# PaulMayer123/IMS-Toucan-Prosody-Variance

Hardware: AMD Instinct MI355X
Metric: mel-frames/sec + vocoder RTF @24kHz, batch=32, 1/2/4/8 MI355X (higher is better)
Workload: dtype bf16

## Files before the change

### ims-toucan-prosody-variance_amd/build.py

```python
import os
import shutil
import subprocess

PKG = os.path.dirname(os.path.abspath(__file__))
CSRC = os.path.join(PKG, "csrc")
LIB = os.path.join(PKG, "libtoucan_hip.so")
SOURCES = ["conv1d.hip", "resblock.hip", "rowops.hip", "attention_mfma.hip", "sequence_ops.hip", "capi.hip", "pipeline.hip", "style.hip", "wavenet.hip", "ffn.hip", "align.hip", "score.hip", "gan.hip", "pitch.hip", "train.hip", "resample.hip", "glow_forward.hip"]


def _hipcc():
    return shutil.which("hipcc") or "/opt/rocm/bin/hipcc"


def needs_build():
    if not os.path.exists(LIB):
        return True
    t = os.path.getmtime(LIB)
    deps = [os.path.join(CSRC, f) for f in os.listdir(CSRC)] + [os.path.join(PKG, "..", "include", h) for h in ("toucan_tts.h", "toucan_align.h", "toucan_score.h", "toucan_gan.h", "toucan_pitch.h", "toucan_train.h", "toucan_resample.h")]
    return any(os.path.getmtime(d) > t for d in deps)


def build(force=False, verbose=False):
    if not force and not needs_build():
        return LIB
    objs = []
    bdir = os.path.join(PKG, "build")
    os.makedirs(bdir, exist_ok=True)
    procs = []
    for src in SOURCES:
        obj = os.path.join(bdir, src.replace(".hip", ".o"))
        objs.append(obj)
        cmd = [_hipcc(), "--offload-arch=gfx950", "-O3", "-std=c++17", "-fPIC", "-c", os.path.join(CSRC, src), "-o", obj]
        if verbose:
            print(" ".join(cmd))
        procs.append((src, subprocess.Popen(cmd, stdout=subprocess.PIPE, stderr=subprocess.STDOUT, text=True)))
    for src, p in procs:
        out, _ = p.communicate()
        if p.returncode != 0:
            raise RuntimeError(f"hipcc failed on {src}:\n{out}")
        if verbose and out.strip():
            print(out)
    cmd = [_hipcc(), "--offload-arch=gfx950", "-shared", "-fPIC", "-o", LIB] + objs
    r = subprocess.run(cmd, stdout=subprocess.PIPE, stderr=subprocess.STDOUT, text=True)
    if r.returncode != 0:
        raise RuntimeError(f"link failed:\n{r.stdout}")
    return LIB


if __name__ == "__main__":
    print(build(force=True, verbose=True))
```

### ims-toucan-prosody-variance_amd/capi.py

```python
import ctypes as C
import os

_PKG = os.path.dirname(os.path.abspath(__file__))
LIB_PATH = os.environ.get("TOUCAN_HIP_LIB") or os.path.join(_PKG, "libtoucan_hip.so")

MODE_LINEAR, MODE_GLU, MODE_GATED, MODE_COUPLING = 0, 1, 2, 3
ACT_NONE, ACT_RELU, ACT_TANH = 0, 1, 2
PRE_NONE, PRE_LRELU, PRE_SNAKE = 0, 1, 2
COMPUTE_F32, COMPUTE_BF16, COMPUTE_F16 = 0, 1, 2
COMPUTE_F32X3 = 3

_p = C.c_void_p
_i = C.c_int32
_f = C.c_float


class TtsTile(C.Structure):
    _fields_ = [("row0", _i), ("seq_begin", _i), ("seq_end", _i), ("seq_id", _i)]


class TtsConvDesc(C.Structure):
    _fields_ = [
        ("x", _p), ("ldx", _i), ("cin", _i),
        ("w", _p), ("cin_pad", _i), ("wn", _i), ("half_pad", _i),
        ("bias", _p),
        ("y", _p), ("ldy", _i), ("cout", _i),
        ("taps", _i), ("dil", _i), ("pad_left", _i),
        ("pre_act", _i), ("pre_slope", _f),
        ("snake_alpha", _p), ("snake_beta", _p), ("snake_filt", _p),
        ("mode", _i), ("act", _i), ("alpha", _f),
        ("seqvec", _p), ("ld_seqvec", _i),
        ("preadd", _p), ("ld_preadd", _i),
        ("res", _p), ("ld_res", _i), ("res_scale", _f),
        ("aux", _p), ("ld_aux", _i),
        ("accumulate", _i),
        ("compute", _i),
        ("io_flags", _i),
        ("tiles", _p), ("n_tiles", _i), ("tile_rows", _i),
    ]


class TtsResblockDesc(C.Structure):
    _fields_ = [
        ("x", _p), ("ldx", _i),
        ("y", _p), ("ldy", _i),
        ("c", _i), ("taps", _i), ("dil", _i),
        ("w1", _p), ("b1", _p),
        ("w2", _p), ("b2", _p),
        ("act", _i), ("slope", _f),
        ("alpha1", _p), ("beta1", _p), ("alpha2", _p), ("beta2", _p), ("filt", _p),
        ("alpha", _f), ("res_scale", _f), ("accumulate", _i),
        ("io_bf16", _i),
        ("tiles", _p), ("n_tiles", _i), ("tile_rows", _i),
        ("compute", _i),
        ("fir_tab", _p),
    ]


class TtsWavenetDesc(C.Structure):
    _fields_ = [
        ("hs_in", _p), ("ld_in", _i),
        ("hs_out", _p), ("ld_out", _i),
        ("cond", _p), ("ld_cond", _i),
        ("w1", _p), ("b1", _p),
        ("w2", _p), ("b2", _p),
        ("cout2", _i),
        ("compute", _i),
        ("tiles", _p), ("n_tiles", _i), ("tile_rows", _i),
    ]


class TtsFfnDesc(C.Structure):
    _fields_ = [
        ("x", _p), ("ldx", _i),
        ("y", _p), ("ldy", _i),
        ("rows", _i), ("channels", _i),
        ("ln_g", _p), ("ln_b", _p),
        ("w", _p), ("b2", _p),
        ("post_g", _p), ("post_b", _p),
        ("hidden", _i), ("compute", _i),
        ("alpha", _f), ("eps", _f),
    ]


class TtsConfig(C.Structure):
    _fields_ = [("multilingual", _i), ("multispeaker", _i), ("vocoder", _i), ("precision", _i), ("small_tile_blocks", _i), ("post_bias", _f)]


IO_X_BF16, IO_Y_BF16, IO_RES_BF16, IO_F16 = 1, 2, 4, 8
IO_SPLIT_K = 16
IO_SPLIT_K_ALWAYS = 32
ATT_KEY_SPLIT, ATT_KEY_SPLIT_ALWAYS = 1, 2

PROTOTYPES = {
    "tts_last_error": (C.c_char_p, []),
    "tts_abi_version": (C.c_int, []),
    "tts_diag_queue_nonzero": (C.c_int, []),
    "tts_diag_queue_slots_used": (C.c_int, []),
    "tts_conv1d_tile_rows": (C.c_int, [_i, _i]),
    "tts_conv1d_n_tile": (C.c_int, [_i, _i]),
    "tts_conv1d_small_tile_rows": (C.c_int, [_i, _i, _i]),
    "tts_conv1d": (C.c_int, [C.POINTER(TtsConvDesc), _p]),
    "tts_resblock_step": (C.c_int, [C.POINTER(TtsResblockDesc), _p]),
    "tts_resblock_tile_rows": (C.c_int, [_i]),
    "tts_snake_fir_table": (C.c_int, [_p, _p]),
    "tts_wavenet_layer": (C.c_int, [C.POINTER(TtsWavenetDesc), _p]),
    "tts_ffn_fused": (C.c_int, [C.POINTER(TtsFfnDesc), _p]),
    "tts_layernorm": (C.c_int, [_p, _i, _p, _i, _p, _p, _i, _i, _f, _p]),
    "tts_cond_layernorm": (C.c_int, [_p, _i, _p, _i, _p, _p, _i, _p, _i, _i, _p]),
    "tts_cln_mlp_weight_floats": (C.c_int64, [_i, _i]),
    "tts_cln_mlp": (C.c_int, [_p, _i, _i, _i, _p, _i, _p, _p]),
    "tts_l2_normalize": (C.c_int, [_p, _p, _i, _i, _p]),
    "tts_groupnorm": (C.c_int, [_p, _i, _p, _i, _p, _p, _i, _i, _f, _i, _p, _i, _p, _p, _i, _i, _p, _p]),
    "tts_groupnorm_workspace_floats": (C.c_int64, [_i, _i, _i]),
    "tts_relpos_attention": (C.c_int, [_p, _i, _p, _i, _p, _p, _p, _i, _i, _i, _p, _i, _i, _i, _p]),
    "tts_relpos_attention_f16": (C.c_int, [_p, _i, _p, _i, _p, _p, _p, _i, _i, _i, _p, _i, _i, _p]),
    "tts_dwconv_swish": (C.c_int, [_p, _i, _p, _i, _p, _p, _i, _i, _p, _i, _i, _p]),
    "tts_duration_from_log": (C.c_int, [_p, _p, _i, _p]),
    "tts_prosody_control": (C.c_int, [_p, _i, _p, _p, _p, _p, _p, _i, _f, _f, _f, _f, _p]),
    "tts_length_regulate": (C.c_int, [_p, _i, _p, _p, _p, _p, _p, _p, _p, _p, _p, _p, _i, _i, _i, _i, _p, _i, _p, _i, _f, _p]),
    "tts_glow_invconv_actnorm": (C.c_int, [_p, _i, _i, _i, _p, _p, _p, _p]),
    "tts_snake_aa": (C.c_int, [_p, _i, _p, _i, _p, _p, _p, _i, _p, _i, _i, _i, _p]),
    "tts_conv_post": (C.c_int, [_p, _i, _i, _p, _f, _i, _f, _p, _p, _i, _i, _i, _p]),
    "tts_conv_post_snake_tile_rows": (C.c_int, []),
    "tts_conv_post_snake": (C.c_int, [_p, _i, _i, _p, _f, _p, _p, _p, _p, _p, _i, _i, _i, _p]),
    "tts_gather_rows": (C.c_int, [_p, _i, _p, _p, _i, _i, _i, _p]),
    "tts_gru_layer": (C.c_int, [_p, _i, _i, _i, _i, _i, _p, _p, _p, _p, _p, _i, _p]),
    "tts_style_tokens": (C.c_int, [_p, _p, _p, _i, _i, _i, _i, _p, _p]),
    "tts_complex_magnitude": (C.c_int, [_p, _i, _p, _i, _i, _i, _p]),
    "tts_log10_floor": (C.c_int, [_p, _i, _p, _i, _i, _i, _f, _p]),
    "tts_create": (C.c_int, [C.POINTER(TtsConfig), C.POINTER(_p)]),
    "tts_destroy": (C.c_int, [_p]),
    "tts_load_weights": (C.c_int, [_p, C.c_char_p, _p, C.POINTER(C.c_int64), _i, _i]),
    "tts_workspace_bytes": (C.c_int64, [_p, _i, _i, _i]),
    "tts_workspace_claimed": (C.c_int64, [_p]),
    "tts_table_stats": (C.c_int, [_p, C.POINTER(C.c_int64), C.POINTER(C.c_int64)]),
    "tts_encoder": (C.c_int, [_p, _p, _p, _p, _p, _i, _p]),
    "tts_variance_predictors": (C.c_int, [_p, _p, _p, _p, _p]),
    "tts_control_and_regulate": (C.c_int, [_p, _f, _f, _f, _f, _p, _p]),
    "tts_decoder": (C.c_int, [_p, _p]),
    "tts_postnet": (C.c_int, [_p, _p]),
    "tts_postflow": (C.c_int, [_p, _p, _p]),
    "tts_mel": (C.c_int, [_p, C.POINTER(_p), C.POINTER(_i), _p, _p]),
    "tts_prosody": (C.c_int, [_p, C.POINTER(_p), C.POINTER(_p), C.POINTER(_p)]),
    "tts_copy_mel": (C.c_int, [_p, _p, _i, _p]),
    "tts_copy_prosody": (C.c_int, [_p, _p, _p, _p, _p]),
    "tts_profile": (C.c_int, [_p, _i, C.c_char_p]),
    "tts_profile_count": (_i, [_p]),
    "tts_profile_read": (C.c_int, [_p, _i, C.c_char_p, _i, C.POINTER(C.c_double), C.POINTER(C.c_double), C.POINTER(C.c_double), C.POINTER(C.c_double)]),
    "tts_vocoder_bigvgan": (C.c_int, [_p, _p, _i, _p, _p, _i, _p, _p]),
    "tts_vocoder_hifigan": (C.c_int, [_p, _p, _i, _p, _p, _i, _p, _p]),
    "tts_synthesize_batch": (C.c_int, [_p, _p, _p, _p, _p, _i, _p, _p, _p, _f, _f, _f, _f, _p, _p, _p, _p, C.c_int64, C.POINTER(C.c_int64), _p]),
}

ALIGN_PROTOTYPES = {
    "tts_relu_affine": (C.c_int, [_p, _i, _p, _i, _i, _i, _p, _p, _p]),
    "tts_lstm_recurrence": (C.c_int, [_p, _i, _p, _p, _p, _p, _p, _p, _i, _p, _p, _i, _i, _i, _p]),
    "tts_mas_durations": (C.c_int, [_p, _i, _p, _p, _p, _p, _p, _p, _p, _p, _p, _p, _i, _i, _i, _p, _p]),
    "tts_frame_energy": (C.c_int, [_p, _i, _i, _p, _i, _p]),
    "tts_token_average": (C.c_int, [_p, _p, _p, _p, _p, _p, _p, _i, _i, _i, _p, _p]),
}

SCORE_PROTOTYPES = {
    "tts_ctc_loss": (C.c_int, [_p, _i, _i, _p, _p, _p, _p, _p, _i, _i, _i, _p, _p]),
    "tts_score_losses": (C.c_int, [_p, _i, _p, _i, _p, _i, _p, _p, _p, _p, _p, _p, _p, _p, _p, _p, _i, _p, _p]),
    "tts_teacher_forced": (C.c_int, [_p, _p, _p, _p, _p, _p, _p, C.POINTER(_i), _p]),
    "tts_copy_decoder_mel": (C.c_int, [_p, _p, _i, _p]),
    "tts_glow_forward_rows": (C.c_int, [_p, _i, _i, _p, _i, _p, _p, _p, _p, _p]),
    "tts_glow_nll_reduce": (C.c_int, [_p, _i, _p, _p, _p, _p, _i, C.c_double, _p, _p, _p]),
    "tts_postflow_nll": (C.c_int, [_p, _p, _i, _p, _p, _p, _p]),
}
CTC_MAX_TARGETS = 2048
GLOW_FORWARD_BLOCK_ROWS, GLOW_FORWARD_GRID_ROWS = 12, 24576


class TtsGanConvDesc(C.Structure):
    _fields_ = [
        ("x", _p), ("w", _p), ("scale", _p), ("shift", _p), ("res", _p), ("y", _p),
        ("n", _i), ("h", _i), ("cin", _i), ("cout", _i), ("taps", _i),
        ("flags", _i),
        ("pre_slope", _f), ("res_ratio", _f), ("slope", _f),
    ]


GAN_PROTOTYPES = {
    "tts_gan_conv2d": (C.c_int, [C.POINTER(TtsGanConvDesc), _p]),
}
GAN_KC, GAN_NC = 16, 64
GAN_UPSAMPLE, GAN_PRE_LRELU, GAN_RESIDUAL, GAN_RES_UPSAMPLE, GAN_LRELU = 1, 2, 4, 8, 16

PITCH_PROTOTYPES = {
    "tts_wave_stats": (C.c_int, [_p, _p, _p, _i, _p, _p]),
    "tts_pitch_candidates": (C.c_int, [_p, _p, _p, _p, _p, _p, _i, _i, _p, _p, _p, _p, _p, _p, _p]),
    "tts_pitch_path": (C.c_int, [_p, _p, _p, _p, _p, _p, _p, _i, _i, _p, _p]),
}
PITCH_CANDIDATES, PITCH_LAGS, PITCH_WINDOW = 15, 600, 1198
PITCH_MIN_SAMPLES, PITCH_PATH_LDS_FRAMES = 1200, 2048

_l = C.c_int64
TRAIN_PROTOTYPES = {
    "tts_gemm_f32": (C.c_int, [_i, _p, _i, _p, _i, _p, _i, _p, _i, _i, _i, _i, _p]),
    "tts_bn_train_forward": (C.c_int, [_p, _i, _p, _p, _p, _p, _p, _p, _i, _p, _p, _i, _i, _f, _f, _p]),
    "tts_bn_train_backward": (C.c_int, [_p, _i, _p, _i, _p, _p, _p, _p, _p, _i, _p, _p, _i, _i, _p]),
    "tts_bn_eval_affine": (C.c_int, [_p, _p, _p, _p, _p, _p, _i, _f, _p]),
    "tts_lstm_train_step": (C.c_int, [_p, _i, _p, _p, _p, _p, _i, _p, _p, _i, _i, _i, _p]),
    "tts_lstm_backward_step": (C.c_int, [_p, _i, _p, _p, _p, _p, _p, _i, _i, _i, _p]),
    "tts_ctc_grad": (C.c_int, [_p, _i, _i, _i, _p, _i, _i, _p, _p, _p, _p, _i, _p]),
    "tts_col_sum": (C.c_int, [_p, _i, _i, _i, _p, _p, _p]),
    "tts_sumsq": (C.c_int, [_p, _l, _p, _p, _p]),
    "tts_sgd_clip_update": (C.c_int, [_p, _p, _l, _p, _f, _f, _p]),
}
GEMM_NN, GEMM_NT, GEMM_TN = 0, 1, 2
CTC_GRAD_MAX_TARGETS, SUMSQ_PARTIALS = 768, 256


class TtsResampleSpan(C.Structure):
    _fields_ = [("in_begin", _l), ("n_held", _l), ("pos0", _l), ("out_first", _l), ("out_count", _l), ("out_begin", _l)]


RESAMPLE_PROTOTYPES = {
    "tts_resample_tile_outputs": (C.c_int, []),
    "tts_resample": (C.c_int, [_p, _p, _p, _i, _l, _i, _i, _i, _i, _p, _p]),
}
RESAMPLE_MAX_FACTOR, RESAMPLE_LDS_TABLE_BYTES = 1024, 65536

_LIB = None
ABI_VERSION = 15


class ToucanHipError(RuntimeError):
    pass


def lib():
    global _LIB
    if _LIB is not None:
        return _LIB
    if not os.path.exists(LIB_PATH):
        raise ToucanHipError(
            f"{LIB_PATH} not found: the HIP extension is mandatory (no CPU fallback). "
            f"Build it with `python -c 'import __graft_entry__ as g; g.build()'`.")
    import torch
    handle = C.CDLL(LIB_PATH)
    _assert_single_hip_runtime()
    for name, (res, args) in list(PROTOTYPES.items()) + list(ALIGN_PROTOTYPES.items()) + list(SCORE_PROTOTYPES.items()) + \
            list(GAN_PROTOTYPES.items()) + list(PITCH_PROTOTYPES.items()) + list(TRAIN_PROTOTYPES.items()) + list(RESAMPLE_PROTOTYPES.items()):
        try:
            fn = getattr(handle, name)
        except AttributeError as e:
            raise ToucanHipError(f"{LIB_PATH} does not export {name}") from e
        fn.restype = res
        fn.argtypes = args
    got = handle.tts_abi_version()
    if got != ABI_VERSION:
        raise ToucanHipError(f"{LIB_PATH} reports ABI version {got}, this binding was written for {ABI_VERSION}: rebuild the "
                             f"library (python -c 'import __graft_entry__ as g; g.build()')")
    _LIB = handle
    return handle


def _assert_single_hip_runtime():
    try:
        with open("/proc/self/maps") as f:
            paths = {line.split()[-1] for line in f if "libamdhip64" in line}
    except OSError:
        return
    if len(paths) > 1:
        raise ToucanHipError(f"two HIP runtimes are mapped ({sorted(paths)}); import torch before loading libtoucan_hip.so")


CALLS = 0


def check(rc, what=""):
    global CALLS
    CALLS += 1
    if rc != 0:
        msg = lib().tts_last_error().decode("utf-8", "replace")
        raise ToucanHipError(f"{what} failed with code {rc}: {msg}")
```

### ims-toucan-prosody-variance_amd/csrc/conv1d.hip

```cpp
#include <cstdlib>
#include <type_traits>

#include "common.h"
#include "snake.h"

namespace tts {

template <int TM, int TN, int WAVES_M, int WAVES_N, bool DUAL>
struct ConvCfg {
  static constexpr int BM = TM * WAVES_M * 32;
  static constexpr int BN = TN * WAVES_N * 32;
};

__device__ __forceinline__ float pre_activation(float v, int pre_act, float slope) {
  if (pre_act == TTS_PRE_LRELU) return v > 0.0f ? v : v * slope;
  return v;
}

__device__ __forceinline__ unsigned short f2bf(float f) { return f32_to_bf16(f); }

template <bool BF16, bool F16, class T>
__device__ __forceinline__ void store_group(T* dst, float a, float b, float c, float e) {
  if constexpr (BF16) {
    *reinterpret_cast<uint2*>(dst) = make_uint2(pack16<F16>(a, b), pack16<F16>(c, e));
  } else {
    dst[0] = a;
    dst[1] = b;
    dst[2] = c;
    dst[3] = e;
  }
}

__device__ __forceinline__ void split3(float v, float& hi, float& lo) {
  hi = (float)(_Float16)v;
  lo = (v - hi) * 2048.0f;
}
__device__ __forceinline__ void store_group_x3(unsigned short* dst, size_t plane_elems, float a, float b, float c, float e) {
  float h[4], l[4];
  split3(a, h[0], l[0]);
  split3(b, h[1], l[1]);
  split3(c, h[2], l[2]);
  split3(e, h[3], l[3]);
  *reinterpret_cast<uint2*>(dst) = make_uint2(pack16<true>(h[0], h[1]), pack16<true>(h[2], h[3]));
  *reinterpret_cast<uint2*>(dst + plane_elems) = make_uint2(pack16<true>(l[0], l[1]), pack16<true>(l[2], l[3]));
}

template <bool BF16, bool F16>
struct Elem {
  using T = unsigned short;
  static __device__ __forceinline__ unsigned short cvt(float v) { return to16<F16>(v); }
};
template <bool F16>
struct Elem<false, F16> {
  using T = float;
  static __device__ __forceinline__ float cvt(float v) { return v; }
};

template <int K, int N, class F>
__device__ __forceinline__ void static_for(F&& f) {
  if constexpr (K < N) {
    f(std::integral_constant<int, K>{});
    static_for<K + 1, N>(f);
  }
}

template <bool DUAL>
__device__ __forceinline__ float epilogue_value(const TtsConvDesc& d, float a, float g, float ba, float bg, float sv, float pa, float pg, float ax,
                                                float rv) {
  float v = a + ba + sv;
  if (d.preadd) v += pa;
  if (DUAL) {
    g += bg;
    if (d.preadd) g += pg;
    if (d.mode == TTS_MODE_GLU) {
      v = v * (1.0f / (1.0f + expf(-g)));
    } else if (d.mode == TTS_MODE_GATED) {
      v = tanhf(v) * (1.0f / (1.0f + expf(-g)));
    } else {
      v = (ax - v) * expf(-g);
    }
  } else {
    if (d.act == TTS_ACT_RELU) v = fmaxf(v, 0.0f);
    else if (d.act == TTS_ACT_TANH) v = tanhf(v);
  }
  v *= d.alpha;
  if (d.res) v += d.res_scale * rv;
  return v;
}

template <bool DUAL>
__device__ __forceinline__ void epilogue_element(const TtsConvDesc& d, int row, int n, float a, float g, float ba, float bg, float sv, bool io_f16) {
  const float pa = d.preadd ? d.preadd[(size_t)row * d.ld_preadd + n] : 0.0f;
  const float pg = (DUAL && d.preadd) ? d.preadd[(size_t)row * d.ld_preadd + d.cout + n] : 0.0f;
  const float ax = (DUAL && d.mode == TTS_MODE_COUPLING) ? d.aux[(size_t)row * d.ld_aux + n] : 0.0f;
  float rv = 0.0f;
  if (d.res)
    rv = (d.io_flags & TTS_IO_RES_BF16) ? load16(reinterpret_cast<const unsigned short*>(d.res)[(size_t)row * d.ld_res + n], io_f16)
                                        : d.res[(size_t)row * d.ld_res + n];
  float v = epilogue_value<DUAL>(d, a, g, ba, bg, sv, pa, pg, ax, rv);
  if (d.io_flags & TTS_IO_Y_BF16) {
    unsigned short* yp = reinterpret_cast<unsigned short*>(d.y) + (size_t)row * d.ldy + n;
    if (d.accumulate) v += load16(*yp, io_f16);
    *yp = store16(v, io_f16);
  } else {
    float* yp = d.y + (size_t)row * d.ldy + n;
    if (d.accumulate) v += *yp;
    *yp = v;
  }
}

__device__ __forceinline__ bool epilogue_vec_ok(const TtsConvDesc& d) {
  auto al = [](const void* p, unsigned m) { return (reinterpret_cast<uintptr_t>(p) & (m - 1)) == 0; };
  bool ok = (d.cout & 3) == 0 && (d.ldy & 3) == 0 && al(d.y, (d.io_flags & TTS_IO_Y_BF16) ? 8 : 16);
  if (d.bias) ok = ok && al(d.bias, 16);
  if (d.seqvec) ok = ok && (d.ld_seqvec & 3) == 0 && al(d.seqvec, 16);
  if (d.preadd) ok = ok && (d.ld_preadd & 3) == 0 && al(d.preadd, 16);
  if (d.res) ok = ok && (d.ld_res & 3) == 0 && al(d.res, (d.io_flags & TTS_IO_RES_BF16) ? 8 : 16);
  if (d.mode == TTS_MODE_COUPLING) ok = ok && (d.ld_aux & 3) == 0 && al(d.aux, 16);
  return ok;
}

template <int TM, int TN, int NH, bool DUAL>
__device__ __forceinline__ void conv_epilogue_t(const TtsConvDesc& d, const TtsTile& tile, int n0, int wm, int wn, int lrow, int lk,
                                                const f32x16 (&acc)[NH][TM][TN], const float* eb = nullptr, int eb_n = 0) {
  const bool io_f16 = d.io_flags & TTS_IO_F16;
  const bool vec = epilogue_vec_ok(d);
  const bool y16 = d.io_flags & TTS_IO_Y_BF16, r16 = d.io_flags & TTS_IO_RES_BF16;
  if constexpr (!DUAL) {
    if (vec && !d.preadd && eb) {
      auto col_of = [&](int j, int rq) { return n0 + (wn * TN + j) * 32 + 8 * rq + 4 * lk; };
#pragma unroll
      for (int i = 0; i < TM; ++i) {
        const int row = tile.row0 + (wm * TM + i) * 32 + lrow;
        const int rowc = row < tile.seq_end ? row : tile.seq_end - 1;
        constexpr int NG = TN * 4, CH = 8;
#pragma unroll
        for (int g0 = 0; g0 < NG; g0 += CH) {
        uint4 rv[CH], yv[CH];
#pragma unroll
          for (int g = 0; g < CH; ++g) {
            if (g0 + g >= NG) continue;
            const int j = (g0 + g) >> 2, rq = (g0 + g) & 3;
            int n = col_of(j, rq);
            n = n < d.cout ? n : d.cout - 4;
            rv[g] = make_uint4(0, 0, 0, 0);
            yv[g] = make_uint4(0, 0, 0, 0);
            if (d.res) {
              if (r16) {
                const uint2 u = *reinterpret_cast<const uint2*>(reinterpret_cast<const unsigned short*>(d.res) + (size_t)rowc * d.ld_res + n);
                rv[g].x = u.x; rv[g].y = u.y;
              } else {
                rv[g] = *reinterpret_cast<const uint4*>(d.res + (size_t)rowc * d.ld_res + n);
              }
            }
            if (d.accumulate) {
              if (y16) {
                const uint2 u = *reinterpret_cast<const uint2*>(reinterpret_cast<const unsigned short*>(d.y) + (size_t)rowc * d.ldy + n);
                yv[g].x = u.x; yv[g].y = u.y;
              } else {
                yv[g] = *reinterpret_cast<const uint4*>(d.y + (size_t)rowc * d.ldy + n);
              }
            }
          }
        __builtin_amdgcn_sched_barrier(0);
        if (row < tile.seq_end) {
#pragma unroll
          for (int g = 0; g < CH; ++g) {
            if (g0 + g >= NG) continue;
            const int j = (g0 + g) >> 2, rq = (g0 + g) & 3;
            const int n = col_of(j, rq);
            if (n >= d.cout) continue;
            const float4 ba = *reinterpret_cast<const float4*>(eb + (n - n0));
            const float4 sv = *reinterpret_cast<const float4*>(eb + eb_n + (n - n0));
            const uint4 ru = rv[g], yu = yv[g];
            float4 r4, y4;
            if (r16) r4 = make_float4(load16(ru.x & 0xFFFF, io_f16), load16(ru.x >> 16, io_f16), load16(ru.y & 0xFFFF, io_f16), load16(ru.y >> 16, io_f16));
            else r4 = make_float4(__builtin_bit_cast(float, ru.x), __builtin_bit_cast(float, ru.y), __builtin_bit_cast(float, ru.z), __builtin_bit_cast(float, ru.w));
            if (y16) y4 = make_float4(load16(yu.x & 0xFFFF, io_f16), load16(yu.x >> 16, io_f16), load16(yu.y & 0xFFFF, io_f16), load16(yu.y >> 16, io_f16));
            else y4 = make_float4(__builtin_bit_cast(float, yu.x), __builtin_bit_cast(float, yu.y), __builtin_bit_cast(float, yu.z), __builtin_bit_cast(float, yu.w));
            float v0 = epilogue_value<false>(d, acc[0][i][j][4 * rq + 0], 0.f, ba.x, 0.f, sv.x, 0.f, 0.f, 0.f, r4.x);
            float v1 = epilogue_value<false>(d, acc[0][i][j][4 * rq + 1], 0.f, ba.y, 0.f, sv.y, 0.f, 0.f, 0.f, r4.y);
            float v2 = epilogue_value<false>(d, acc[0][i][j][4 * rq + 2], 0.f, ba.z, 0.f, sv.z, 0.f, 0.f, 0.f, r4.z);
            float v3 = epilogue_value<false>(d, acc[0][i][j][4 * rq + 3], 0.f, ba.w, 0.f, sv.w, 0.f, 0.f, 0.f, r4.w);
            if (d.accumulate) { v0 += y4.x; v1 += y4.y; v2 += y4.z; v3 += y4.w; }
            if (y16) {
              uint2* yp = reinterpret_cast<uint2*>(reinterpret_cast<unsigned short*>(d.y) + (size_t)row * d.ldy + n);
              *yp = make_uint2((unsigned int)store16(v0, io_f16) | ((unsigned int)store16(v1, io_f16) << 16),
                               (unsigned int)store16(v2, io_f16) | ((unsigned int)store16(v3, io_f16) << 16));
            } else {
              *reinterpret_cast<float4*>(d.y + (size_t)row * d.ldy + n) = make_float4(v0, v1, v2, v3);
            }
          }
        }
        __builtin_amdgcn_sched_barrier(0);
        }
      }
      return;
    }
  }
#pragma unroll
  for (int i = 0; i < TM; ++i) {
    const int row = tile.row0 + (wm * TM + i) * 32 + lrow;
    if (row >= tile.seq_end) continue;
#pragma unroll
    for (int j = 0; j < TN; ++j) {
#pragma unroll
      for (int rq = 0; rq < 4; ++rq) {
        const int n = n0 + (wn * TN + j) * 32 + 8 * rq + 4 * lk;
        if (n >= d.cout) continue;
        if (!vec) {
          for (int q = 0; q < 4 && n + q < d.cout; ++q) {
            const float ba = d.bias ? d.bias[n + q] : 0.0f;
            const float bg = (DUAL && d.bias) ? d.bias[d.cout + n + q] : 0.0f;
            const float sv = d.seqvec ? d.seqvec[(size_t)tile.seq_id * d.ld_seqvec + n + q] : 0.0f;
            epilogue_element<DUAL>(d, row, n + q, acc[0][i][j][4 * rq + q], acc[NH - 1][i][j][4 * rq + q], ba, bg, sv, io_f16);
          }
          continue;
        }
        const float4 z4 = make_float4(0.f, 0.f, 0.f, 0.f);
        auto ld4 = [](const float* p) { return *reinterpret_cast<const float4*>(p); };
        const float4 ba = d.bias ? ld4(d.bias + n) : z4;
        const float4 bg = (DUAL && d.bias) ? ld4(d.bias + d.cout + n) : z4;
        const float4 sv = d.seqvec ? ld4(d.seqvec + (size_t)tile.seq_id * d.ld_seqvec + n) : z4;
        const float4 pa = d.preadd ? ld4(d.preadd + (size_t)row * d.ld_preadd + n) : z4;
        const float4 pg = (DUAL && d.preadd) ? ld4(d.preadd + (size_t)row * d.ld_preadd + d.cout + n) : z4;
        const float4 ax = (DUAL && d.mode == TTS_MODE_COUPLING) ? ld4(d.aux + (size_t)row * d.ld_aux + n) : z4;
        float4 rv = z4;
        if (d.res) {
          if (r16) {
            const uint2 u = *reinterpret_cast<const uint2*>(reinterpret_cast<const unsigned short*>(d.res) + (size_t)row * d.ld_res + n);
            rv = make_float4(load16(u.x & 0xFFFF, io_f16), load16(u.x >> 16, io_f16), load16(u.y & 0xFFFF, io_f16), load16(u.y >> 16, io_f16));
          } else {
            rv = ld4(d.res + (size_t)row * d.ld_res + n);
          }
        }
        float v[4];
        v[0] = epilogue_value<DUAL>(d, acc[0][i][j][4 * rq + 0], acc[NH - 1][i][j][4 * rq + 0], ba.x, bg.x, sv.x, pa.x, pg.x, ax.x, rv.x);
        v[1] = epilogue_value<DUAL>(d, acc[0][i][j][4 * rq + 1], acc[NH - 1][i][j][4 * rq + 1], ba.y, bg.y, sv.y, pa.y, pg.y, ax.y, rv.y);
        v[2] = epilogue_value<DUAL>(d, acc[0][i][j][4 * rq + 2], acc[NH - 1][i][j][4 * rq + 2], ba.z, bg.z, sv.z, pa.z, pg.z, ax.z, rv.z);
        v[3] = epilogue_value<DUAL>(d, acc[0][i][j][4 * rq + 3], acc[NH - 1][i][j][4 * rq + 3], ba.w, bg.w, sv.w, pa.w, pg.w, ax.w, rv.w);
        if (y16) {
          uint2* yp = reinterpret_cast<uint2*>(reinterpret_cast<unsigned short*>(d.y) + (size_t)row * d.ldy + n);
          if (d.accumulate) {
            const uint2 u = *yp;
            v[0] += load16(u.x & 0xFFFF, io_f16); v[1] += load16(u.x >> 16, io_f16);
            v[2] += load16(u.y & 0xFFFF, io_f16); v[3] += load16(u.y >> 16, io_f16);
          }
          *yp = make_uint2((unsigned int)store16(v[0], io_f16) | ((unsigned int)store16(v[1], io_f16) << 16),
                           (unsigned int)store16(v[2], io_f16) | ((unsigned int)store16(v[3], io_f16) << 16));
        } else {
          float4* yp = reinterpret_cast<float4*>(d.y + (size_t)row * d.ldy + n);
          if (d.accumulate) {
            const float4 u = *yp;
            v[0] += u.x; v[1] += u.y; v[2] += u.z; v[3] += u.w;
          }
          *yp = make_float4(v[0], v[1], v[2], v[3]);
        }
      }
    }
  }
}

template <int NH, bool DUAL>
__device__ __forceinline__ void conv_epilogue16_t(const TtsConvDesc& d, const TtsTile& tile, int n0, int row_base, int lane, const f32x4 (&acc)[NH]) {
  const bool io_f16 = d.io_flags & TTS_IO_F16;
  const int row = row_base + (lane & 15), n = n0 + 4 * (lane >> 4);
  if (row >= tile.seq_end || n >= d.cout) return;
  if (!epilogue_vec_ok(d)) {
    for (int q = 0; q < 4 && n + q < d.cout; ++q) {
      const float ba = d.bias ? d.bias[n + q] : 0.0f;
      const float bg = (DUAL && d.bias) ? d.bias[d.cout + n + q] : 0.0f;
      const float sv = d.seqvec ? d.seqvec[(size_t)tile.seq_id * d.ld_seqvec + n + q] : 0.0f;
      epilogue_element<DUAL>(d, row, n + q, acc[0][q], acc[NH - 1][q], ba, bg, sv, io_f16);
    }
    return;
  }
  const bool y16 = d.io_flags & TTS_IO_Y_BF16, r16 = d.io_flags & TTS_IO_RES_BF16;
  auto ld4 = [](const float* p) { return *reinterpret_cast<const float4*>(p); };
  auto ld16 = [&](const float* base, size_t off) {
    const uint2 u = *reinterpret_cast<const uint2*>(reinterpret_cast<const unsigned short*>(base) + off);
    return make_float4(load16(u.x & 0xFFFF, io_f16), load16(u.x >> 16, io_f16), load16(u.y & 0xFFFF, io_f16), load16(u.y >> 16, io_f16));
  };
  const float4 z4 = make_float4(0.f, 0.f, 0.f, 0.f);
  float4 ba = z4, bg = z4, sv = z4, pa = z4, pg = z4, ax = z4, rv = z4, yv = z4;
  if (d.bias) ba = ld4(d.bias + n);
  if (DUAL && d.bias) bg = ld4(d.bias + d.cout + n);
  if (d.seqvec) sv = ld4(d.seqvec + (size_t)tile.seq_id * d.ld_seqvec + n);
  if (d.preadd) pa = ld4(d.preadd + (size_t)row * d.ld_preadd + n);
  if (DUAL && d.preadd) pg = ld4(d.preadd + (size_t)row * d.ld_preadd + d.cout + n);
  if (DUAL && d.mode == TTS_MODE_COUPLING) ax = ld4(d.aux + (size_t)row * d.ld_aux + n);
  if (d.res) {
    if (r16) rv = ld16(d.res, (size_t)row * d.ld_res + n);
    else rv = ld4(d.res + (size_t)row * d.ld_res + n);
  }
  if (d.accumulate) {
    if (y16) yv = ld16(d.y, (size_t)row * d.ldy + n);
    else yv = ld4(d.y + (size_t)row * d.ldy + n);
  }
  float v0 = epilogue_value<DUAL>(d, acc[0][0], acc[NH - 1][0], ba.x, bg.x, sv.x, pa.x, pg.x, ax.x, rv.x);
  float v1 = epilogue_value<DUAL>(d, acc[0][1], acc[NH - 1][1], ba.y, bg.y, sv.y, pa.y, pg.y, ax.y, rv.y);
  float v2 = epilogue_value<DUAL>(d, acc[0][2], acc[NH - 1][2], ba.z, bg.z, sv.z, pa.z, pg.z, ax.z, rv.z);
  float v3 = epilogue_value<DUAL>(d, acc[0][3], acc[NH - 1][3], ba.w, bg.w, sv.w, pa.w, pg.w, ax.w, rv.w);
  if (d.accumulate) { v0 += yv.x; v1 += yv.y; v2 += yv.z; v3 += yv.w; }
  if (y16) {
    *reinterpret_cast<uint2*>(reinterpret_cast<unsigned short*>(d.y) + (size_t)row * d.ldy + n) =
        make_uint2((unsigned int)store16(v0, io_f16) | ((unsigned int)store16(v1, io_f16) << 16),
                   (unsigned int)store16(v2, io_f16) | ((unsigned int)store16(v3, io_f16) << 16));
  } else {
    *reinterpret_cast<float4*>(d.y + (size_t)row * d.ldy + n) = make_float4(v0, v1, v2, v3);
  }
}

constexpr int conv_min_waves(int tm, int tn, bool dual, bool bf16, bool snake, bool x3) {
  return (((tm == 2 && tn == 2) || (tm == 1 && tn == 3)) && !dual && !snake && !x3) ? 3 : 1;
}

template <int TM, int TN, int WAVES_M, int WAVES_N, bool DUAL, bool BF16, bool SNAKE, bool F16, bool X3 = false>
__global__ __launch_bounds__(256) __attribute__((amdgpu_waves_per_eu(conv_min_waves(TM, TN, DUAL, BF16, SNAKE, X3))))
void conv1d_kernel(const TtsConvDesc d) {
  static_assert(BF16 || !F16, "F16 selects the element format of the 16-bit MFMA path");
  static_assert(!X3 || (BF16 && F16 && !SNAKE), "the split fp32 product runs on the fp16 path");
  using C = ConvCfg<TM, TN, WAVES_M, WAVES_N, DUAL>;
  using ET = typename Elem<BF16, F16>::T;
  constexpr int BM = C::BM, BN = C::BN;
  constexpr int NH = DUAL ? 2 : 1;
  constexpr int BK = BF16 ? 64 : 32;
  const int XP = BF16 ? (d.cin_pad <= 32 ? 40 : BK + 8) : BK + 1;
  constexpr int EPU = BF16 ? 8 : 4;
  constexpr int UNITS = BK * BN / EPU;
  constexpr int UPT = UNITS / 256;
  static_assert(UNITS % 256 == 0, "slab must split evenly over the workgroup");
  extern __shared__ __attribute__((aligned(16))) unsigned char lds_raw[];

  const TtsTile tile = d.tiles[blockIdx.x];
  const int n0 = blockIdx.y * BN;
  const int halo = (d.taps - 1) * d.dil;
  const int win_rows = BM + halo;
  constexpr bool WIN2 = BM == 64 && !SNAKE && !X3;
  constexpr int NP = X3 ? 2 : 1;
  constexpr int GPR = BK / 4;
  constexpr int PF = BF16 ? 5 : 3;
  const size_t xs_elems = ((size_t)win_rows * XP + 7) & ~(size_t)7;
  ET* xs0 = reinterpret_cast<ET*>(lds_raw);
  ET* ws = xs0 + ((WIN2 || X3) ? 2 : 1) * xs_elems;
  constexpr int WBUF = NH * NP * BK * BN;
  float* eb = DUAL ? nullptr : reinterpret_cast<float*>(ws + (size_t)2 * WBUF);

  const int tid = threadIdx.x;
  const int lane = tid & 63;
  const int wave = tid >> 6;
  const int wm = wave / WAVES_N;
  const int wn = wave % WAVES_N;
  const int lrow = lane & 31;
  const int lk = lane >> 5;

  f32x16 acc[NH][TM][TN];
  f32x16 accx[X3 ? NH : 1][X3 ? TM : 1][X3 ? TN : 1];
#pragma unroll
  for (int h = 0; h < NH; ++h)
#pragma unroll
    for (int i = 0; i < TM; ++i)
#pragma unroll
      for (int j = 0; j < TN; ++j)
#pragma unroll
        for (int r = 0; r < 16; ++r) {
          acc[h][i][j][r] = 0.0f;
          if constexpr (X3) accx[h][i][j][r] = 0.0f;
        }

  if constexpr (!DUAL) {
    if (threadIdx.x < BN) {
      const int n = n0 + threadIdx.x;
      eb[threadIdx.x] = (d.bias && n < d.cout) ? d.bias[n] : 0.0f;
      eb[BN + threadIdx.x] = (d.seqvec && n < d.cout) ? d.seqvec[(size_t)tile.seq_id * d.ld_seqvec + n] : 0.0f;
    }
  }
  const int row_first = tile.row0 - d.pad_left;
  const bool x_bf16 = d.io_flags & TTS_IO_X_BF16;
  const bool x_f16 = BF16 ? F16 : (d.io_flags & TTS_IO_F16) != 0;
  const unsigned short* __restrict__ xh = reinterpret_cast<const unsigned short*>(d.x);
  const bool vec_ok = ((d.ldx & 3) == 0) && ((d.cin & 3) == 0) && ((reinterpret_cast<uintptr_t>(d.x) & (x_bf16 ? 7 : 15)) == 0);
  const bool win2 = WIN2 && vec_ok && win_rows * GPR <= PF * 256;
  const ET* __restrict__ W = reinterpret_cast<const ET*>(d.w);
  const int n_chunks = (d.cin_pad + BK - 1) / BK;
  const int total_steps = n_chunks * d.taps;

  uint4 wreg[NH][NP][UPT];
  const size_t w_plane = (size_t)d.taps * d.cin_pad * d.wn;
  auto load_slab = [&](int c0, int tap, int kchunk) __attribute__((always_inline)) {
#pragma unroll
    for (int h = 0; h < NH; ++h)
#pragma unroll
      for (int q = 0; q < UPT; ++q) {
        const int u = tid + q * 256;
        size_t goff;
        bool ok;
        if constexpr (BF16) {
          int kb = u / BN;
          const int n = u % BN;
          ok = kb * 8 < kchunk;
          kb = ok ? kb : 0;
          goff = (((size_t)tap * (d.cin_pad / 8) + c0 / 8 + kb) * d.wn + n0 + h * d.half_pad + n) * 8;
        } else {
          int k = u / (BN / 4);
          const int c4 = (u % (BN / 4)) * 4;
          ok = k < kchunk;
          k = ok ? k : 0;
          goff = ((size_t)tap * d.cin_pad + c0 + k) * d.wn + n0 + h * d.half_pad + c4;
        }
#pragma unroll
        for (int pl = 0; pl < NP; ++pl) {
          const uint4 v = *reinterpret_cast<const uint4*>(W + goff + pl * w_plane);
          wreg[h][pl][q] = ok ? v : make_uint4(0, 0, 0, 0);
        }
      }
  };
  auto store_slab = [&](int buf) __attribute__((always_inline)) {
#pragma unroll
    for (int h = 0; h < NH; ++h)
#pragma unroll
      for (int q = 0; q < UPT; ++q) {
        const int u = tid + q * 256;
#pragma unroll
        for (int pl = 0; pl < NP; ++pl)
          *reinterpret_cast<uint4*>(ws + (size_t)buf * WBUF + (h * NP + pl) * BK * BN + u * EPU) = wreg[h][pl][q];
      }
  };

  uint4 pre[WIN2 ? PF : 1];
  auto win_decode = [&](int e, int c0, int& wr, int& c4, bool& ok, size_t& goff) __attribute__((always_inline)) {
    wr = e / GPR;
    c4 = (e % GPR) * 4;
    const int gr = row_first + wr;
    ok = gr >= tile.seq_begin && gr < tile.seq_end && (c0 + c4) < d.cin;
    const int grc = gr < tile.seq_begin ? tile.seq_begin : (gr >= tile.seq_end ? tile.seq_end - 1 : gr);
    const int cc = (c0 + c4) < d.cin ? (c0 + c4) : d.cin - 4;
    goff = (size_t)grc * d.ldx + cc;
  };
  auto win_request = [&](int c0) __attribute__((always_inline)) {
    if constexpr (WIN2) {
      const int total = win_rows * GPR;
      size_t goff[PF];
#pragma unroll
      for (int q = 0; q < PF; ++q) {
        int e = tid + q * 256;
        e = e < total ? e : total - 1;
        int wr, c4;
        bool ok;
        win_decode(e, c0, wr, c4, ok, goff[q]);
      }
      if (x_bf16) {
#pragma unroll
        for (int q = 0; q < PF; ++q) {
          const uint2 raw = *reinterpret_cast<const uint2*>(xh + goff[q]);
          pre[q].x = raw.x;
          pre[q].y = raw.y;
        }
      } else {
#pragma unroll
        for (int q = 0; q < PF; ++q) pre[q] = *reinterpret_cast<const uint4*>(d.x + goff[q]);
      }
    }
  };
  auto win_commit = [&](int c0, ET* xs) __attribute__((always_inline)) {
    if constexpr (WIN2) {
      const int total = win_rows * GPR;
#pragma unroll
      for (int q = 0; q < PF; ++q) {
        const int e = tid + q * 256;
        if (e < total) {
          int wr, c4;
          bool ok;
          size_t goff;
          win_decode(e, c0, wr, c4, ok, goff);
          float4 v;
          if (x_bf16)
            v = make_float4(load16(pre[q].x & 0xFFFF, x_f16), load16(pre[q].x >> 16, x_f16), load16(pre[q].y & 0xFFFF, x_f16), load16(pre[q].y >> 16, x_f16));
          else
            v = make_float4(__builtin_bit_cast(float, pre[q].x), __builtin_bit_cast(float, pre[q].y), __builtin_bit_cast(float, pre[q].z),
                            __builtin_bit_cast(float, pre[q].w));
          if (!ok) v = make_float4(0.f, 0.f, 0.f, 0.f);
          ET* dst = xs + wr * XP + c4;
          store_group<BF16, F16>(dst, pre_activation(v.x, d.pre_act, d.pre_slope), pre_activation(v.y, d.pre_act, d.pre_slope),
                            pre_activation(v.z, d.pre_act, d.pre_slope), pre_activation(v.w, d.pre_act, d.pre_slope));
        }
      }
    }
  };
  if (win2) {
    win_request(0);
    win_commit(0, xs0);
  }

  {
    const int k0 = d.cin_pad < BK ? d.cin_pad : BK;
    load_slab(0, 0, k0);
    store_slab(0);
  }

  int step = 0;
  for (int ch = 0; ch < n_chunks; ++ch) {
    const int c0 = ch * BK;
    const int kchunk = (d.cin_pad - c0) < BK ? (d.cin_pad - c0) : BK;
    ET* xs = xs0 + ((win2 && (ch & 1)) ? xs_elems : 0);
    if (!win2 && ch > 0) __syncthreads();
    if (win2) {
      if (ch + 1 < n_chunks) win_request(c0 + BK);
    } else if (SNAKE) {
      float f[12];
#pragma unroll
      for (int k = 0; k < 12; ++k) f[k] = d.snake_filt[k];
      const int T = tile.seq_end - tile.seq_begin;
      const int items = ((win_rows + 7) >> 3) * kchunk;
      for (int it = tid; it < items; it += 256) {
        const int chl = it % kchunk, wr0 = (it / kchunk) * 8;
        const int cg = c0 + chl;
        const int t0 = row_first + wr0 - tile.seq_begin;
        float o[8];
        const bool live = cg < d.cin && t0 + 7 >= 0 && t0 < T;
        if constexpr (SNAKE)
          if (live) {
            const float ea = expf(d.snake_alpha[cg]), ib = 1.0f / (expf(d.snake_beta[cg]) + 1e-9f);
            if (x_bf16)
              snake_rows_fn<8>([&](int q) { return load16(xh[(size_t)(tile.seq_begin + q) * d.ldx + cg], x_f16); }, T, t0, f, ea, ib, o);
            else
              snake_rows<8>(d.x, d.ldx, cg, tile.seq_begin, T, t0, f, ea, ib, o);
          }
#pragma unroll
        for (int i = 0; i < 8; ++i)
          if (wr0 + i < win_rows) xs[(wr0 + i) * XP + chl] = Elem<BF16, F16>::cvt((live && t0 + i >= 0 && t0 + i < T) ? o[i] : 0.0f);
      }
    } else if (BF16 && BM != 64 && vec_ok && x_bf16 && (d.cin & 7) == 0 && (d.ldx & 7) == 0 && (reinterpret_cast<uintptr_t>(d.x) & 15) == 0) {
      if constexpr (BF16 && BM != 64) {
        constexpr int PER8 = 6;
        const int q8 = kchunk >> 3;
        const int total = win_rows * q8;
        for (int base = tid; base < total; base += 256 * PER8) {
          uint4 raw[PER8];
#pragma unroll
          for (int p = 0; p < PER8; ++p) {
            int e = base + p * 256;
            e = e < total ? e : total - 1;
            const int wr = e / q8, c8 = (e % q8) * 8;
            const int gr = row_first + wr;
            const int grc = gr < tile.seq_begin ? tile.seq_begin : (gr >= tile.seq_end ? tile.seq_end - 1 : gr);
            const int cc = (c0 + c8) < d.cin ? (c0 + c8) : d.cin - 8;
            raw[p] = *reinterpret_cast<const uint4*>(xh + (size_t)grc * d.ldx + cc);
          }
#pragma unroll
          for (int p = 0; p < PER8; ++p) {
            const int e = base + p * 256;
            if (e >= total) continue;
            const int wr = e / q8, c8 = (e % q8) * 8;
            const int gr = row_first + wr;
            const bool ok = gr >= tile.seq_begin && gr < tile.seq_end && (c0 + c8) < d.cin;
            uint4 o = raw[p];
            if (d.pre_act != TTS_PRE_NONE) {
              const unsigned int w4[4] = {o.x, o.y, o.z, o.w};
              unsigned int r4[4];
#pragma unroll
              for (int q = 0; q < 4; ++q)
                r4[q] = pack16<F16>(pre_activation(from16<F16>(w4[q] & 0xFFFF), d.pre_act, d.pre_slope),
// ... 248 lines not shown
#pragma unroll
        for (int j = 0; j < 4; ++j) TTS_GLOAD32(b[h][slot][j], wp + ((size_t)g * 8 + j) * wrow + h * whalf);
    };
    auto arrive = [&](int slot) __attribute__((always_inline)) {
      TTS_WAIT_VM((DEPTH - 1) * L);
      TTS_PIN(a[slot]);
#pragma unroll
      for (int h = 0; h < NH; ++h)
#pragma unroll
        for (int j = 0; j < 4; ++j) TTS_PIN(b[h][slot][j]);
    };
#pragma unroll
    for (int u = 0; u < DEPTH; ++u) request(u, u);
    for (int base = 0; base < n_groups; base += DEPTH) {
#pragma unroll
      for (int u = 0; u < DEPTH; ++u) {
        arrive(u);
        float av[4], bv[NH][4];
#pragma unroll
        for (int j = 0; j < 4; ++j) {
          av[j] = pre_activation(u2f(a[u][j]), d.pre_act, d.pre_slope);
#pragma unroll
          for (int h = 0; h < NH; ++h) bv[h][j] = u2f(b[h][u][j]);
        }
#pragma unroll
        for (int j = 0; j < 4; ++j)
#pragma unroll
          for (int h = 0; h < NH; ++h) acc[h][0][0] = __builtin_amdgcn_mfma_f32_32x32x2f32(bv[h][j], av[j], acc[h][0][0], 0, 0, 0);
        int nxt = base + u + DEPTH;
        nxt = nxt < n_groups ? nxt : n_groups - 1;
        request(u, nxt);
      }
    }
    TTS_WAIT_VM(0);
#pragma unroll
    for (int u = 0; u < DEPTH; ++u) {
      TTS_PIN(a[u]);
#pragma unroll
      for (int h = 0; h < NH; ++h)
#pragma unroll
        for (int j = 0; j < 4; ++j) TTS_PIN(b[h][u][j]);
    }
  }
  conv_epilogue_t<1, 1, NH, DUAL>(d, tile, n0, wm, wn, lrow, lk, acc);
}

template <bool DUAL, bool T16>
__global__ __launch_bounds__(256) void conv_splitk_f32_kernel(const TtsConvDesc d) {
  constexpr int NH = DUAL ? 2 : 1;
  constexpr int T = T16 ? 16 : 32;
  constexpr int GC = 16;
  constexpr int NA = T16 ? 1 : 2;
  constexpr int NB = 4 * NA;
  constexpr int AR = T16 ? 4 : 16;
  constexpr int DEPTH = T16 ? 4 : 2;
  constexpr int L = NA + NB * NH;
  static_assert((DEPTH - 1) * L <= 63, "vmcnt is a 6-bit count");
  using Acc = typename std::conditional<T16, f32x4, f32x16>::type;
  __shared__ float part[3][NH][AR][64];
  const int subs = d.tile_rows / T;
  const TtsTile tile = d.tiles[blockIdx.x / subs];
  const int sub = blockIdx.x % subs;
  if (tile.row0 + sub * T >= tile.seq_end) return;
  const int n0 = blockIdx.y * T;
  const int tid = threadIdx.x, lane = tid & 63, lrow = lane & (T - 1), kq = lane / T;
  const int wave = __builtin_amdgcn_readfirstlane(tid >> 6);
  const int orow = tile.row0 + sub * T + lrow;
  const int col = n0 + lrow;

  Acc acc[NH];
#pragma unroll
  for (int h = 0; h < NH; ++h)
#pragma unroll
    for (int r = 0; r < AR; ++r) acc[h][r] = 0.0f;

  typedef unsigned int u32x4 __attribute__((ext_vector_type(4)));
  auto u2f = [](unsigned int bits) __attribute__((always_inline)) { return __builtin_bit_cast(float, bits); };
  const int G = d.cin / GC;
  const int S = d.taps * G;
  const int n_w = S > wave ? (S - wave + 3) >> 2 : 0;
  int tap_r = wave / G, g_r = wave % G;
  const size_t wrow = (size_t)d.wn * 4, whalf = (size_t)d.half_pad * 4;
  u32x4 a[DEPTH][NA];
  unsigned int b[NH][DEPTH][NB];
  bool inside[DEPTH];
  auto request = [&](int slot) __attribute__((always_inline)) {
    const bool live = tap_r < d.taps;
    const int tp = live ? tap_r : d.taps - 1, gg = live ? g_r : G - 1;
    int r = orow + tp * d.dil - d.pad_left;
    inside[slot] = live && r >= tile.seq_begin && r < tile.seq_end;
    r = r < tile.seq_begin ? tile.seq_begin : (r >= tile.seq_end ? tile.seq_end - 1 : r);
    const char* xp = reinterpret_cast<const char*>(d.x) + ((size_t)r * d.ldx + gg * GC + kq * 4) * 4;
    const char* wp = reinterpret_cast<const char*>(d.w) + (((size_t)tp * d.cin_pad + gg * GC + kq * 4) * d.wn + col) * 4;
#pragma unroll
    for (int q = 0; q < NA; ++q) TTS_GLOAD128(a[slot][q], xp + q * 32);
#pragma unroll
    for (int h = 0; h < NH; ++h)
#pragma unroll
      for (int q = 0; q < NA; ++q)
#pragma unroll
        for (int j = 0; j < 4; ++j) TTS_GLOAD32(b[h][slot][4 * q + j], wp + (8 * q + j) * wrow + h * whalf);
    if (live) {
      g_r += 4;
      while (g_r >= G) { g_r -= G; ++tap_r; }
    }
  };
  auto arrive = [&](int slot) __attribute__((always_inline)) {
    TTS_WAIT_VM((DEPTH - 1) * L);
#pragma unroll
    for (int q = 0; q < NA; ++q) TTS_PIN(a[slot][q]);
#pragma unroll
    for (int h = 0; h < NH; ++h)
#pragma unroll
      for (int j = 0; j < NB; ++j) TTS_PIN(b[h][slot][j]);
  };
#pragma unroll
  for (int u = 0; u < DEPTH; ++u) request(u);
  for (int base = 0; base < n_w; base += DEPTH) {
#pragma unroll
    for (int u = 0; u < DEPTH; ++u) {
      arrive(u);
      float av[NA][4], bv[NH][NB];
#pragma unroll
      for (int q = 0; q < NA; ++q)
#pragma unroll
        for (int j = 0; j < 4; ++j) av[q][j] = inside[u] ? pre_activation(u2f(a[u][q][j]), d.pre_act, d.pre_slope) : 0.0f;
#pragma unroll
      for (int h = 0; h < NH; ++h)
#pragma unroll
        for (int j = 0; j < NB; ++j) bv[h][j] = u2f(b[h][u][j]);
#pragma unroll
      for (int j = 0; j < 4; ++j)
#pragma unroll
        for (int q = 0; q < NA; ++q)
#pragma unroll
          for (int h = 0; h < NH; ++h) {
            if constexpr (T16) acc[h] = __builtin_amdgcn_mfma_f32_16x16x4f32(bv[h][4 * q + j], av[q][j], acc[h], 0, 0, 0);
            else acc[h] = __builtin_amdgcn_mfma_f32_32x32x2f32(bv[h][4 * q + j], av[q][j], acc[h], 0, 0, 0);
          }
      request(u);
    }
  }
  TTS_WAIT_VM(0);
#pragma unroll
  for (int u = 0; u < DEPTH; ++u) {
#pragma unroll
    for (int q = 0; q < NA; ++q) TTS_PIN(a[u][q]);
#pragma unroll
    for (int h = 0; h < NH; ++h)
#pragma unroll
      for (int j = 0; j < NB; ++j) TTS_PIN(b[h][u][j]);
  }
  if (wave != 0) {
#pragma unroll
    for (int h = 0; h < NH; ++h)
#pragma unroll
      for (int r = 0; r < AR; ++r) part[wave - 1][h][r][lane] = acc[h][r];
  }
  __syncthreads();
  if (wave != 0) return;
#pragma unroll
  for (int h = 0; h < NH; ++h)
#pragma unroll
    for (int r = 0; r < AR; ++r) acc[h][r] = ((acc[h][r] + part[0][h][r][lane]) + part[1][h][r][lane]) + part[2][h][r][lane];
  if constexpr (T16) {
    conv_epilogue16_t<NH, DUAL>(d, tile, n0, tile.row0 + sub * 16, lane, acc);
  } else {
    f32x16 acc32[NH][1][1];
#pragma unroll
    for (int h = 0; h < NH; ++h) acc32[h][0][0] = acc[h];
    conv_epilogue_t<1, 1, NH, DUAL>(d, tile, n0, sub, 0, lrow, kq, acc32);
  }
}

enum ConvShape { S_128x128, S_128x96, S_128x64, S_256x32, S_D128x96, S_64x64, S_D64x64, S_64x128 };

static ConvShape pick_shape(int cout, int mode) {
  if (mode != TTS_MODE_LINEAR) return S_D128x96;
  if (cout <= 32) return S_256x32;
  if (cout <= 64) return S_128x64;
  const int pad96 = (cout + 95) / 96 * 96, pad128 = (cout + 127) / 128 * 128;
  return (pad96 < pad128) ? S_128x96 : S_128x128;
}

static void shape_dims(ConvShape s, int& bm, int& bn) {
  switch (s) {
    case S_128x128: bm = 128; bn = 128; break;
    case S_128x96: bm = 128; bn = 96; break;
    case S_128x64: bm = 128; bn = 64; break;
    case S_256x32: bm = 256; bn = 32; break;
    case S_D128x96: bm = 128; bn = 96; break;
    case S_64x64: bm = 64; bn = 64; break;
    case S_D64x64: bm = 64; bn = 64; break;
    case S_64x128: bm = 64; bn = 128; break;
  }
}

static bool small_form_ok(int cout, int mode, int cols) {
  if (cols % 64 != 0) return false;
  return mode != TTS_MODE_LINEAR || cout > 64;
}

template <int TM, int TN, int WAVES_M, int WAVES_N, bool DUAL, bool BF16, bool SNAKE, bool F16 = false, bool X3 = false>
static int launch_one(const TtsConvDesc& d, hipStream_t st) {
  using C = ConvCfg<TM, TN, WAVES_M, WAVES_N, DUAL>;
  constexpr int BK = BF16 ? 64 : 32, ESZ = BF16 ? 2 : 4, NH = DUAL ? 2 : 1;
  const int XP = BF16 ? (d.cin_pad <= 32 ? 40 : BK + 8) : BK + 1;
  const int halo = (d.taps - 1) * d.dil;
  const int win_rows = C::BM + halo;
  const int n_tiles_n = ((DUAL ? d.half_pad : d.wn) + C::BN - 1) / C::BN;
  dim3 grid(d.n_tiles, n_tiles_n), block(256);
  const size_t xs_elems = ((size_t)win_rows * XP + 7) & ~(size_t)7;
  const size_t lds = (((C::BM == 64 && !SNAKE) || X3 ? 2 : 1) * xs_elems + (size_t)2 * NH * (X3 ? 2 : 1) * BK * C::BN) * ESZ +
                     (DUAL ? 0 : 2 * C::BN * sizeof(float));
  TTS_CHECK_ARG(lds <= 160 * 1024, "conv1d: LDS %zu B exceeds 160 KiB (taps %d dil %d)", lds, d.taps, d.dil);
  auto k = conv1d_kernel<TM, TN, WAVES_M, WAVES_N, DUAL, BF16, SNAKE, F16, X3>;
  static unsigned long long lds_raised = 0;
  if (lds > 64 * 1024) {
    const hipError_t e = raise_lds_limit(reinterpret_cast<const void*>(k), lds_raised);
    if (e != hipSuccess) {
      set_error("conv1d: raising the dynamic LDS limit failed: %s", hipGetErrorString(e));
      return TTS_E_LAUNCH;
    }
  }
  hipLaunchKernelGGL(k, grid, block, lds, st, d);
  return launch_status("conv1d");
}

template <int TM, int TN, int WAVES_M, int WAVES_N, bool DUAL>
static int launch_cfg(const TtsConvDesc& d, hipStream_t st) {
  if constexpr (!DUAL) {
    TTS_CHECK_ARG(!(d.pre_act == TTS_PRE_SNAKE && d.compute == 3), "conv1d: the snake prologue is not available with the split fp32 product");
    if (d.pre_act == TTS_PRE_SNAKE) {
      if (d.compute == 0) return launch_one<TM, TN, WAVES_M, WAVES_N, DUAL, false, true>(d, st);
      if (d.compute == 2) return launch_one<TM, TN, WAVES_M, WAVES_N, DUAL, true, true, true>(d, st);
      return launch_one<TM, TN, WAVES_M, WAVES_N, DUAL, true, true>(d, st);
    }
  }
  TTS_CHECK_ARG(d.pre_act != TTS_PRE_SNAKE, "conv1d: the snake prologue is not available in the dual modes");
  if (d.compute == 3) return launch_one<TM, TN, WAVES_M, WAVES_N, DUAL, true, false, true, true>(d, st);
  if (d.compute == 0) return launch_one<TM, TN, WAVES_M, WAVES_N, DUAL, false, false>(d, st);
  if (d.compute == 2) return launch_one<TM, TN, WAVES_M, WAVES_N, DUAL, true, false, true>(d, st);
  return launch_one<TM, TN, WAVES_M, WAVES_N, DUAL, true, false>(d, st);
}

static bool gemm_rows_ok(const TtsConvDesc& d) {
  if (d.compute == 3) return false;
  if (d.taps != 1 || d.pad_left != 0 || d.pre_act == TTS_PRE_SNAKE || d.cin != d.cin_pad) return false;
  const bool xb = d.io_flags & TTS_IO_X_BF16;
  if (xb && d.compute == 0) return false;
  if (d.cin % (d.compute ? 64 : 32) != 0) return false;
  if (d.compute != 0 && std::getenv("TOUCAN_GEMM_ROWS_BF16") == nullptr) {
    const int cols = d.mode != TTS_MODE_LINEAR ? d.half_pad : d.wn;
    if ((long long)d.n_tiles * (cols / 64) > 256) return false;
  }
  if ((d.ldx & (xb ? 7 : 3)) != 0 || (reinterpret_cast<uintptr_t>(d.x) & 15) != 0) return false;
  return true;
}

static bool splitk_ok(const TtsConvDesc& d, int cols) {
  if (d.compute != 0 || !(d.io_flags & (TTS_IO_SPLIT_K | TTS_IO_SPLIT_K_ALWAYS)) || (d.io_flags & TTS_IO_X_BF16) || d.pre_act == TTS_PRE_SNAKE) return false;
  if ((d.cin & 15) != 0 || d.cin < 32 || (d.ldx & 3) != 0 || (reinterpret_cast<uintptr_t>(d.x) & 15) != 0 || (cols & 31) != 0) return false;
  constexpr int min_depth = 64, max_grid = 128;
  if ((long long)d.taps * d.cin < min_depth) return false;
  if (!(d.io_flags & TTS_IO_SPLIT_K_ALWAYS) && (long long)d.n_tiles * (d.tile_rows / 64) * ((cols + 63) / 64) > max_grid) return false;
  return std::getenv("TOUCAN_NO_SPLIT_K") == nullptr;
}

static int launch_splitk(const TtsConvDesc& d, int cols, hipStream_t st) {
  const bool dual = d.mode != TTS_MODE_LINEAR;
  if (d.cin >= 64 && (long long)d.n_tiles * (d.tile_rows / 32) * (cols / 32) <= 128 && std::getenv("TOUCAN_NO_SPLIT_K16") == nullptr) {
    dim3 grid(d.n_tiles * (d.tile_rows / 16), cols / 16), block(256);
    if (dual) hipLaunchKernelGGL((conv_splitk_f32_kernel<true, true>), grid, block, 0, st, d);
    else hipLaunchKernelGGL((conv_splitk_f32_kernel<false, true>), grid, block, 0, st, d);
    return launch_status("conv1d (split-K, 16 x 16)");
  }
  dim3 grid(d.n_tiles * (d.tile_rows / 32), cols / 32), block(256);
  if (dual) hipLaunchKernelGGL((conv_splitk_f32_kernel<true, false>), grid, block, 0, st, d);
  else hipLaunchKernelGGL((conv_splitk_f32_kernel<false, false>), grid, block, 0, st, d);
  return launch_status("conv1d (split-K)");
}

static int launch_gemm_rows(const TtsConvDesc& d, hipStream_t st) {
  const bool dual = d.mode != TTS_MODE_LINEAR, xb = d.io_flags & TTS_IO_X_BF16;
  const int cols = dual ? d.half_pad : d.wn;
  dim3 grid(d.n_tiles, cols / 64), block(256);
#define TTS_GEMM_ROWS(DUAL_, BF16_, XB_, F16_) hipLaunchKernelGGL((gemm_rows_kernel<DUAL_, BF16_, XB_, F16_>), grid, block, 0, st, d)
#define TTS_GEMM_ROWS2(DUAL_, XB_) do { if (d.compute == 2) TTS_GEMM_ROWS(DUAL_, true, XB_, true); else TTS_GEMM_ROWS(DUAL_, true, XB_, false); } while (0)
  if (d.compute == 0) {
    if (dual) TTS_GEMM_ROWS(true, false, false, false);
    else TTS_GEMM_ROWS(false, false, false, false);
  } else if (xb) {
    if (dual) TTS_GEMM_ROWS2(true, true);
    else TTS_GEMM_ROWS2(false, true);
  } else {
    if (dual) TTS_GEMM_ROWS2(true, false);
    else TTS_GEMM_ROWS2(false, false);
  }
#undef TTS_GEMM_ROWS2
#undef TTS_GEMM_ROWS
  return launch_status("conv1d (1-tap rows)");
}

int conv1d_dispatch(const TtsConvDesc& d, hipStream_t st) {
  TTS_CHECK_ARG(d.x && d.w && d.y && d.tiles, "conv1d: null pointer");
  TTS_CHECK_ARG(d.cin > 0 && d.cout > 0 && d.taps > 0 && d.dil > 0, "conv1d: bad dims");
  TTS_CHECK_ARG(d.cin_pad % 32 == 0 && d.cin_pad >= d.cin, "conv1d: cin_pad %d must be a multiple of 32 >= cin %d", d.cin_pad, d.cin);
  TTS_CHECK_ARG(d.mode >= 0 && d.mode <= 3, "conv1d: bad mode %d", d.mode);
  TTS_CHECK_ARG(d.compute >= 0 && d.compute <= 3, "conv1d: bad compute %d (0 fp32, 1 bf16, 2 fp16, 3 split fp32)", d.compute);
  TTS_CHECK_ARG(d.compute == 0 || d.compute == 3 || ((d.io_flags & TTS_IO_F16) != 0) == (d.compute == 2) || !(d.io_flags & 7),
                "conv1d: the 16-bit tensors of a bf16 / fp16 call must be in the call's own format");
  TTS_CHECK_ARG(d.compute != 3 || !(d.io_flags & 7), "conv1d: the split fp32 product takes and returns fp32 tensors");
  TTS_CHECK_ARG(d.mode != TTS_MODE_COUPLING || d.aux, "conv1d: coupling mode needs aux");
  TTS_CHECK_ARG(d.pre_act != TTS_PRE_SNAKE || (d.snake_alpha && d.snake_beta && d.snake_filt), "conv1d: PRE_SNAKE needs alpha/beta/filter");
  if (d.n_tiles == 0) return TTS_OK;
  const int cols = d.mode == TTS_MODE_LINEAR ? d.wn : d.half_pad;
  ConvShape s = pick_shape(d.cout, d.mode);
  if (d.tile_rows == 64 && small_form_ok(d.cout, d.mode, cols)) s = d.mode == TTS_MODE_LINEAR ? S_64x64 : S_D64x64;
  int bm, bn;
  shape_dims(s, bm, bn);
  TTS_CHECK_ARG(d.tile_rows == bm, "conv1d: tile table built for %d rows, kernel needs %d", d.tile_rows, bm);
  TTS_CHECK_ARG(cols % bn == 0 && cols >= d.cout, "conv1d: packed width %d not a multiple of the N tile %d (cout %d)", cols, bn, d.cout);
  TTS_CHECK_ARG(d.mode == TTS_MODE_LINEAR || d.wn == 2 * d.half_pad, "conv1d: dual mode needs wn == 2*half_pad");
  if (splitk_ok(d, cols)) return launch_splitk(d, cols, st);
  if ((s == S_64x64 || s == S_D64x64) && gemm_rows_ok(d)) return launch_gemm_rows(d, st);
  if (s == S_64x64 && cols % 128 == 0 && cols >= 256 && (long long)d.n_tiles * (cols / 64) >= 512) {
    s = S_64x128;
    bn = 128;
  }
  switch (s) {
    case S_128x128: return launch_cfg<2, 2, 2, 2, false>(d, st);
    case S_128x96: return launch_cfg<1, 3, 4, 1, false>(d, st);
    case S_128x64: return launch_cfg<2, 1, 2, 2, false>(d, st);
    case S_256x32: return launch_cfg<2, 1, 4, 1, false>(d, st);
    case S_D128x96: return launch_cfg<1, 3, 4, 1, true>(d, st);
    case S_64x64: return launch_cfg<1, 1, 2, 2, false>(d, st);
    case S_D64x64: return launch_cfg<1, 1, 2, 2, true>(d, st);
    case S_64x128: return launch_cfg<2, 1, 1, 4, false>(d, st);
  }
  return TTS_E_ARG;
}

int conv1d_tile_rows(int cout, int mode) {
  int bm, bn;
  shape_dims(pick_shape(cout, mode), bm, bn);
  return bm;
}

int conv1d_small_tile_rows(int cout, int mode, int packed_cols) { return small_form_ok(cout, mode, packed_cols) ? 64 : 0; }

int conv1d_n_tile(int cout, int mode) {
  int bm, bn;
  shape_dims(pick_shape(cout, mode), bm, bn);
  return bn;
}

}
```

### ims-toucan-prosody-variance_amd/csrc/pipeline.hip

```cpp
#include <algorithm>
#include <cmath>
#include <cstdlib>
#include <cstring>
#include <string>
#include <unordered_map>
#include <utility>
#include <vector>

#include "common.h"
#include "../../include/toucan_score.h"

namespace tts {

namespace {

constexpr int ATT = 192, HEADS = 4, DK = 48;

struct Dev {
  void* p = nullptr;
  int64_t shape[4] = {0, 0, 0, 0};
  int ndim = 0, dtype = 0;
  size_t bytes = 0;
};

struct ConvW {
  const float* w = nullptr;
  const void* w16 = nullptr;
  const float* bias = nullptr;
  int mode = 0, taps = 1, dil = 1, pad_left = 0, cin = 0, cin_pad = 0, cout = 0, wn = 0, half_pad = 0, tile_rows = 0, small_tile_rows = 0,
      small_only = 0, n_tile = 0, compute16 = 0, algo_taps = 1;
};

struct Block {
  const float *ln_g[5], *ln_b[5];
  ConvW ffm1, ffm2, qkv, out, pos, pw1, pw2, ff1, ff2;
  const float *u, *v, *dw_w, *dw_b;
  const Dev *ffm_fused = nullptr, *ff_fused = nullptr;
};

struct Predictor {
  int layers = 0, first_cln = 0;
  ConvW conv[7], lin;
  const float *g[7], *b[7];
};

struct Acoustic {
  bool resolved = false;
  ConvW embed0, embed2;
  const float* lang_table = nullptr;
  Block enc[6], dec[6];
  const float *out_norm_g, *out_norm_b;
  ConvW hs_h, hs_e;
  const float* cln_weights = nullptr;
  int n_mlp = 0;
  Predictor pitch, energy, duration;
  const float *pitch_w, *pitch_b, *energy_w, *energy_b;
  ConvW feat_out, g_proj;
  struct { ConvW conv; const float *g, *b; } postnet[5];
  struct { ConvW start, end, cond; const float *winv, *an_bias, *an_logs; } flow[18];
  bool scoring = false;
  struct { const float* wfwd; ConvW end_ml; } flow_fwd[18];
  double flow_logdet = 0.0;
  struct { ConvW inl[4], res_skip[4]; } flowgrp[5];
};

struct Vocoder {
  bool resolved = false;
  ConvW pre, ups[4];
  struct { ConvW c1, c2; const float *a1 = nullptr, *b1 = nullptr, *a2 = nullptr, *b2 = nullptr; } blk[4][3][3];
  const float *post_w, *post_a = nullptr, *post_b = nullptr, *filt = nullptr;
  const void* fir_tab = nullptr;
};

struct Layout {
  std::vector<int> begins, lengths;
  int total = 0, max_len = 0;
  static Layout make(const int* len, int n, int align) {
    Layout l;
    int off = 0;
    for (int i = 0; i < n; ++i) {
      l.begins.push_back(off);
      l.lengths.push_back(len[i]);
      off += (len[i] + align - 1) / align * align;
      l.max_len = std::max(l.max_len, len[i]);
    }
    l.total = off;
    return l;
  }
  Layout scaled(int f) const {
    Layout l;
    for (size_t i = 0; i < begins.size(); ++i) {
      l.begins.push_back(begins[i] * f);
      l.lengths.push_back(lengths[i] * f);
    }
    l.total = total * f;
    l.max_len = max_len * f;
    return l;
  }
  Layout halved() const {
    Layout l;
    for (size_t i = 0; i < begins.size(); ++i) {
      l.begins.push_back(begins[i] / 2);
      l.lengths.push_back(lengths[i] / 2);
      l.max_len = std::max(l.max_len, lengths[i] / 2);
    }
    l.total = total / 2;
    return l;
  }
  int n() const { return (int)lengths.size(); }
};

struct Arena {
  char* base = nullptr;
  size_t cap = 0, off = 0;
  void reset() { off = 0; }
};

struct TileTab {
  TtsTile* dev = nullptr;
  int n = 0;
};

constexpr size_t TABLE_FIRST_CHUNK = 64 << 10;
constexpr size_t TABLE_BUDGET = 16 << 20;

struct TableChunk {
  char* dev = nullptr;
  char* host = nullptr;
  size_t cap = 0, off = 0;
};

struct TableStore {
  std::vector<TableChunk> chunks;
  std::unordered_map<std::string, std::pair<void*, int>> index;
  hipEvent_t last_use = nullptr;
};

struct ProfRec {
  std::string name;
  double flops = 0, bytes = 0, elems = 0;
  hipEvent_t e0 = nullptr, e1 = nullptr;
};

}

struct Handle {
  TtsConfig cfg;
  std::unordered_map<std::string, Dev> weights;
  Acoustic acoustic;
  Vocoder vocoder;
  Arena phone, frame, voc[2];
  Arena nll;
  TableStore tabs[2][2];
  int tab_gen[2] = {0, 0};
  int tab_which = 0;
  long long n_tables_built = 0;
  int small_tile_blocks = 1536;
  int split_mode = 0;
  float* ptab[2] = {nullptr, nullptr};
  int pmax = 0;
  Layout lp, lf;
  int B = 0;
  const float* text = nullptr;
  float *e_norm = nullptr, *enc = nullptr, *pitch = nullptr, *energy = nullptr, *cln = nullptr;
  int* dur = nullptr;
  float *cat = nullptr, *dec = nullptr, *mel0 = nullptr, *mel = nullptr;
  std::vector<int> frames;
  bool have_flow = false;
  bool prof_on = false, prof_detail = false;
  std::string prof_select;
  std::vector<ProfRec> prof;
  std::vector<hipEvent_t> event_pool;
};

namespace {

#define TTS_TRY(expr)            \
  do {                           \
    const int rc_ = (expr);      \
    if (rc_ != TTS_OK) return rc_; \
  } while (0)

bool is16(const Handle* h);

#define TTS_CHECK_RESOLVED(h, entry) TTS_CHECK_ARG((h)->acoustic.resolved, entry ": weights were loaded since tts_encoder: run it again")

int hip_ok(hipError_t e, const char* what) {
  if (e == hipSuccess) return TTS_OK;
  set_error("%s: %s", what, hipGetErrorString(e));
  return TTS_E_LAUNCH;
}

int arena_reserve(Arena& a, size_t bytes, hipStream_t st) {
  a.reset();
  if (a.cap >= bytes) return TTS_OK;
  if (a.base) {
    TTS_TRY(hip_ok(hipStreamSynchronize(st), "workspace: stream sync before regrowth"));
    (void)hipFree(a.base);
    a.base = nullptr;
    a.cap = 0;
  }
  const size_t want = bytes + bytes / 8 + (1 << 20);
  TTS_TRY(hip_ok(hipMalloc(reinterpret_cast<void**>(&a.base), want), "workspace: hipMalloc"));
  a.cap = want;
  return TTS_OK;
}

template <class T>
T* arena_alloc(Arena& a, size_t count) {
  const size_t bytes = (count * sizeof(T) + 255) & ~(size_t)255;
  if (a.off + bytes > a.cap) return nullptr;
  T* p = reinterpret_cast<T*>(a.base + a.off);
  a.off += bytes;
  return p;
}

#define TTS_ALLOC(var, arena, T, count)                                                        \
  T* var = arena_alloc<T>(arena, (size_t)(count));                                             \
  if (!var) {                                                                                  \
    set_error("%s: workspace exhausted (%zu of %zu bytes used)", __func__, (arena).off, (arena).cap); \
    return TTS_E_ARG;                                                                          \
  }

std::string layout_key(const Layout& l, int tile_rows) {
  std::string k(reinterpret_cast<const char*>(l.begins.data()), l.begins.size() * sizeof(int));
  k.append(reinterpret_cast<const char*>(l.lengths.data()), l.lengths.size() * sizeof(int));
  k.append(reinterpret_cast<const char*>(&tile_rows), sizeof(int));
  return k;
}

int tables_begin(Handle* h, int which, hipStream_t st) {
  h->tab_which = which;
  h->tab_gen[which] ^= 1;
  TableStore& s = h->tabs[which][h->tab_gen[which]];
  if (!s.last_use) return TTS_OK;
  size_t held = 0;
  for (const TableChunk& c : s.chunks) held += c.off;
  if (held > TABLE_BUDGET) {
    TTS_TRY(hip_ok(hipEventSynchronize(s.last_use), "tile tables: last use before rewinding"));
    s.index.clear();
    for (TableChunk& c : s.chunks) c.off = 0;
    return TTS_OK;
  }
  const hipError_t q = hipEventQuery(s.last_use);
  if (q == hipSuccess) return TTS_OK;
  if (q != hipErrorNotReady) return hip_ok(q, "tile tables: last use");
  (void)hipGetLastError();
  return hip_ok(hipStreamWaitEvent(st, s.last_use, 0), "tile tables: wait for last use");
}

template <class Build>
int table_of(Handle* h, const std::string& key, hipStream_t st, Build build, void** dev, int* n) {
  TableStore& s = h->tabs[h->tab_which][h->tab_gen[h->tab_which]];
  auto it = s.index.find(key);
  if (it == s.index.end()) {
    auto host = build();
    const int count = (int)host.size();
    if (host.empty()) host.resize(1);
    const size_t bytes = host.size() * sizeof(host[0]), need = (bytes + 255) & ~(size_t)255;
    TableChunk* c = nullptr;
    for (TableChunk& k : s.chunks)
      if (k.off + need <= k.cap) {
        c = &k;
        break;
      }
    if (!c) {
      TableChunk k;
      k.cap = std::max(s.chunks.empty() ? TABLE_FIRST_CHUNK : 2 * s.chunks.back().cap, need);
      TTS_TRY(hip_ok(hipMalloc(reinterpret_cast<void**>(&k.dev), k.cap), "tile tables: hipMalloc"));
      const hipError_t e = hipHostMalloc(reinterpret_cast<void**>(&k.host), k.cap, hipHostMallocDefault);
      if (e != hipSuccess) (void)hipFree(k.dev);
      TTS_TRY(hip_ok(e, "tile tables: hipHostMalloc"));
      s.chunks.push_back(k);
      c = &s.chunks.back();
    }
    memcpy(c->host + c->off, host.data(), bytes);
    TTS_TRY(hip_ok(hipMemcpyAsync(c->dev + c->off, c->host + c->off, bytes, hipMemcpyHostToDevice, st), "tile tables: upload"));
    it = s.index.emplace(key, std::make_pair(static_cast<void*>(c->dev + c->off), count)).first;
    c->off += need;
    ++h->n_tables_built;
  }
  *dev = it->second.first;
  if (n) *n = it->second.second;
  return TTS_OK;
}

int tiles_of(Handle* h, const Layout& l, int tile_rows, hipStream_t st, TileTab* out) {
  void* dev;
  TTS_TRY(table_of(h, layout_key(l, tile_rows), st, [&] {
    std::vector<TtsTile> host;
    for (int u = 0; u < l.n(); ++u)
      for (int r = 0; r < l.lengths[u]; r += tile_rows) host.push_back(TtsTile{l.begins[u] + r, l.begins[u], l.begins[u] + l.lengths[u], u});
    return host;
  }, &dev, &out->n));
  out->dev = static_cast<TtsTile*>(dev);
  return TTS_OK;
}

int bounds_of(Handle* h, const Layout& l, hipStream_t st, const int** sb, const int** se) {
  void* dev;
  TTS_TRY(table_of(h, layout_key(l, -1), st, [&] {
    std::vector<int> host(2 * std::max(1, l.n()));
    for (int u = 0; u < l.n(); ++u) {
      host[u] = l.begins[u];
      host[l.n() + u] = l.begins[u] + l.lengths[u];
    }
    return host;
  }, &dev, nullptr));
  *sb = static_cast<const int*>(dev);
  *se = *sb + l.n();
  return TTS_OK;
}

const Dev* find(const Handle* h, const std::string& name) {
  auto it = h->weights.find(name);
  return it == h->weights.end() ? nullptr : &it->second;
}

int need(const Handle* h, const std::string& name, const Dev** out) {
  *out = find(h, name);
  if (!*out) {
    set_error("weight '%s' was not loaded (tts_load_weights)", name.c_str());
    return TTS_E_ARG;
  }
  return TTS_OK;
}

int fvec(const Handle* h, const std::string& name, const float** out) {
  const Dev* d;
  TTS_TRY(need(h, name, &d));
  *out = static_cast<const float*>(d->p);
  return TTS_OK;
}

int conv_of(const Handle* h, const std::string& name, ConvW* c) {
  const Dev *w, *m;
  TTS_TRY(need(h, name + ".w", &w));
  TTS_TRY(need(h, name + ".meta", &m));
  const int* mm = static_cast<const int*>(m->p);
  c->w = static_cast<const float*>(w->p);
  const Dev* w16 = find(h, name + ".w16");
  c->w16 = w16 ? w16->p : nullptr;
  const Dev* b = find(h, name + ".bias");
  c->bias = b ? static_cast<const float*>(b->p) : nullptr;
  c->mode = mm[0]; c->taps = mm[1]; c->dil = mm[2]; c->pad_left = mm[3]; c->cin = mm[4]; c->cin_pad = mm[5]; c->cout = mm[6];
  c->wn = mm[7]; c->half_pad = mm[8]; c->tile_rows = mm[9]; c->small_tile_rows = mm[10]; c->small_only = mm[11]; c->n_tile = mm[12];
  c->compute16 = mm[13];
  c->algo_taps = mm[14] > 0 ? mm[14] : c->taps;
  return TTS_OK;
}

hipEvent_t prof_event(Handle* h) {
  if (!h->event_pool.empty()) {
    hipEvent_t e = h->event_pool.back();
    h->event_pool.pop_back();
    return e;
  }
  hipEvent_t e = nullptr;
  (void)hipEventCreate(&e);
  return e;
}

template <class Launch>
int prof_launch(Handle* h, const char* name, double flops, double bytes, double elems, hipStream_t st, Launch launch) {
  if (!h->prof_on || !(h->prof_select.empty() || h->prof_select == name)) return launch();
  h->prof.emplace_back();
  ProfRec* r = &h->prof.back();
  r->name = name; r->flops = flops; r->bytes = bytes; r->elems = elems;
  r->e0 = prof_event(h);
  r->e1 = prof_event(h);
  (void)hipEventRecord(r->e0, st);
  const int rc = launch();
  (void)hipEventRecord(r->e1, st);
  return rc;
}

struct T2 {
  void* p;
  int ld;
  int bits;
  T2() : p(nullptr), ld(0), bits(32) {}
  T2(void* p_, int ld_, int bits_ = 32) : p(p_), ld(ld_), bits(bits_) {}
};

struct ConvOpt {
  int pre = TTS_PRE_NONE;
  float pre_slope = 0.f;
  int act = TTS_ACT_NONE;
  float alpha = 1.f;
  const float* seqvec = nullptr; int ld_seqvec = 0;
  const float* preadd = nullptr; int ld_preadd = 0;
  T2 res; float res_scale = 1.f;
  const float* aux = nullptr; int ld_aux = 0;
  bool accumulate = false;
  bool fp32_only = false;
  bool no_split_k = false;
  const float *snake_alpha = nullptr, *snake_beta = nullptr, *snake_filt = nullptr;
};

int conv(Handle* h, const ConvW& cw, T2 x, T2 y, const Layout& l, hipStream_t st, const ConvOpt& o = ConvOpt()) {
  int tile_rows = cw.tile_rows;
  if (h->small_tile_blocks && cw.small_tile_rows && !cw.small_only) {
    const int cols = cw.mode == TTS_MODE_LINEAR ? cw.wn : cw.half_pad;
    const long long grid = (long long)((l.total + cw.tile_rows - 1) / cw.tile_rows) * (cols / cw.n_tile);
    if (grid < h->small_tile_blocks) tile_rows = cw.small_tile_rows;
  }
  TileTab tt;
  TTS_TRY(tiles_of(h, l, tile_rows, st, &tt));
  TtsConvDesc d;
  memset(&d, 0, sizeof(d));
  bool use16 = !o.fp32_only && h->cfg.precision != TTS_COMPUTE_F32 && cw.w16 != nullptr;
  if (use16 && cw.compute16 == TTS_COMPUTE_F32X3) {
    const int cols = cw.mode == TTS_MODE_LINEAR ? cw.wn : cw.half_pad;
    const bool small = (long long)tt.n * (tile_rows / 64) * ((cols + 63) / 64) <= 128;
    if (h->split_mode == 2 || (h->split_mode == 1 && small)) use16 = false;
  }
  d.x = static_cast<const float*>(x.p); d.ldx = x.ld; d.cin = cw.cin;
  d.w = use16 ? cw.w16 : cw.w; d.cin_pad = cw.cin_pad; d.wn = cw.wn; d.half_pad = cw.half_pad;
  d.bias = cw.bias;
  d.y = static_cast<float*>(y.p); d.ldy = y.ld; d.cout = cw.cout;
  d.taps = cw.taps; d.dil = cw.dil; d.pad_left = cw.pad_left;
  d.pre_act = o.pre; d.pre_slope = o.pre_slope;
  d.snake_alpha = o.snake_alpha; d.snake_beta = o.snake_beta; d.snake_filt = o.snake_filt;
  d.mode = cw.mode; d.act = o.act; d.alpha = o.alpha;
  d.seqvec = o.seqvec; d.ld_seqvec = o.ld_seqvec;
  d.preadd = o.preadd; d.ld_preadd = o.ld_preadd;
  d.res = static_cast<const float*>(o.res.p); d.ld_res = o.res.ld; d.res_scale = o.res_scale;
  d.aux = o.aux; d.ld_aux = o.ld_aux;
  d.accumulate = o.accumulate ? 1 : 0;
  d.compute = use16 ? cw.compute16 : TTS_COMPUTE_F32;
  const bool any16 = x.bits == 16 || y.bits == 16 || (o.res.p && o.res.bits == 16);
  d.io_flags = (x.bits == 16 ? TTS_IO_X_BF16 : 0) | (y.bits == 16 ? TTS_IO_Y_BF16 : 0) | ((o.res.p && o.res.bits == 16) ? TTS_IO_RES_BF16 : 0) |
               ((any16 && h->cfg.precision == TTS_COMPUTE_F16) ? TTS_IO_F16 : 0);
  if (h->split_mode && !o.no_split_k && !is16(h) && d.compute == TTS_COMPUTE_F32)
    d.io_flags |= h->split_mode == 2 ? TTS_IO_SPLIT_K_ALWAYS : TTS_IO_SPLIT_K;
  d.tiles = tt.dev; d.n_tiles = tt.n; d.tile_rows = tile_rows;
  if (h->prof_on) {
    const bool dual = cw.mode != TTS_MODE_LINEAR;
    const int bm = tile_rows != cw.tile_rows ? tile_rows : cw.tile_rows, bn = tile_rows != cw.tile_rows ? 64 : cw.n_tile;
    char name[96];
    int nlen = snprintf(name, sizeof(name), "conv1d_%s<%dx%d%s>", d.compute == TTS_COMPUTE_F32 ? "f32" : (d.compute == TTS_COMPUTE_BF16 ? "bf16" : (d.compute == TTS_COMPUTE_F16 ? "f16" : "f32x3")),
                        bm, bn, dual ? ",dual" : "");
    if (h->prof_detail)
      snprintf(name + nlen, sizeof(name) - nlen, "[%dx%d k%d r%d]", cw.cin, cw.cout * (dual ? 2 : 1), cw.taps, l.total);
    double rows = 0;
    for (int n : l.lengths) rows += n;
    const double ctot = (double)cw.cout * (dual ? 2 : 1);
    return prof_launch(h, name, 2.0 * rows * cw.cin * ctot * cw.algo_taps,
                       rows * (cw.cin * (x.bits / 8.0) + cw.cout * (y.bits / 8.0)) + cw.taps * cw.cin * ctot * (d.compute == TTS_COMPUTE_F32 ? 4 : 2),
                       rows * cw.cout, st, [&] { return tts_conv1d(&d, st); });
  }
  return tts_conv1d(&d, st);
}

int block_of(const Handle* h, const std::string& p, Block* b) {
  static const char* ln[5] = {"norm_ff_macaron", "norm_mha", "norm_conv", "norm_ff", "norm_final"};
  for (int i = 0; i < 5; ++i) {
    TTS_TRY(fvec(h, p + ln[i] + ".g", &b->ln_g[i]));
    TTS_TRY(fvec(h, p + ln[i] + ".b", &b->ln_b[i]));
  }
  TTS_TRY(conv_of(h, p + "ffm.w1", &b->ffm1));
  TTS_TRY(conv_of(h, p + "ffm.w2", &b->ffm2));
  TTS_TRY(conv_of(h, p + "ff.w1", &b->ff1));
  TTS_TRY(conv_of(h, p + "ff.w2", &b->ff2));
  b->ffm_fused = find(h, p + "ffm.fused");
  b->ff_fused = find(h, p + "ff.fused");
  TTS_TRY(conv_of(h, p + "qkv", &b->qkv));
  TTS_TRY(conv_of(h, p + "out", &b->out));
  TTS_TRY(conv_of(h, p + "pos", &b->pos));
  TTS_TRY(conv_of(h, p + "pw1", &b->pw1));
  TTS_TRY(conv_of(h, p + "pw2", &b->pw2));
  TTS_TRY(fvec(h, p + "u", &b->u));
  TTS_TRY(fvec(h, p + "v", &b->v));
  TTS_TRY(fvec(h, p + "dw_w", &b->dw_w));
  TTS_TRY(fvec(h, p + "dw_b", &b->dw_b));
  return TTS_OK;
}

int predictor_of(const Handle* h, const std::string& p, int layers, int first_cln, Predictor* out) {
  out->layers = layers;
  out->first_cln = first_cln;
  for (int i = 0; i < layers; ++i) {
    TTS_TRY(conv_of(h, p + ".conv." + std::to_string(i), &out->conv[i]));
    if (h->cfg.multispeaker) continue;
    TTS_TRY(fvec(h, p + ".norm." + std::to_string(i) + ".g", &out->g[i]));
    TTS_TRY(fvec(h, p + ".norm." + std::to_string(i) + ".b", &out->b[i]));
  }
  return conv_of(h, p + ".lin", &out->lin);
}

int resolve_acoustic(Handle* h) {
  Acoustic& m = h->acoustic;
  if (m.resolved) return TTS_OK;
  TTS_TRY(conv_of(h, "embed0", &m.embed0));
  TTS_TRY(conv_of(h, "embed2", &m.embed2));
  const Dev* lang = find(h, "lang_table");
  m.lang_table = lang ? static_cast<const float*>(lang->p) : nullptr;
  for (int b = 0; b < 6; ++b) {
    TTS_TRY(block_of(h, "enc." + std::to_string(b) + ".", &m.enc[b]));
    TTS_TRY(block_of(h, "dec." + std::to_string(b) + ".", &m.dec[b]));
  }
  TTS_TRY(fvec(h, "out_norm.g", &m.out_norm_g));
  TTS_TRY(fvec(h, "out_norm.b", &m.out_norm_b));
  if (h->cfg.multispeaker) {
    TTS_TRY(conv_of(h, "hs_h", &m.hs_h));
    TTS_TRY(conv_of(h, "hs_e", &m.hs_e));
    const Dev* w;
    TTS_TRY(need(h, "cln_weights", &w));
    m.cln_weights = static_cast<const float*>(w->p);
    m.n_mlp = (int)(w->bytes / 4 / tts_cln_mlp_weight_floats(64, 256));
  }
  TTS_TRY(predictor_of(h, "pitch", 7, 0, &m.pitch));
  TTS_TRY(predictor_of(h, "energy", 2, 7, &m.energy));
  TTS_TRY(predictor_of(h, "duration", 3, 9, &m.duration));
  TTS_TRY(fvec(h, "pitch_w", &m.pitch_w));
  TTS_TRY(fvec(h, "pitch_b", &m.pitch_b));
  TTS_TRY(fvec(h, "energy_w", &m.energy_w));
  TTS_TRY(fvec(h, "energy_b", &m.energy_b));
  TTS_TRY(conv_of(h, "feat_out", &m.feat_out));
  for (int i = 0; i < 5; ++i) {
    const std::string p = "postnet." + std::to_string(i);
    TTS_TRY(conv_of(h, p + ".conv", &m.postnet[i].conv));
    TTS_TRY(fvec(h, p + ".g", &m.postnet[i].g));
    TTS_TRY(fvec(h, p + ".b", &m.postnet[i].b));
  }
  TTS_TRY(conv_of(h, "g_proj", &m.g_proj));
  for (int b = 0; b < 18; ++b) {
    const std::string p = "flow." + std::to_string(b) + ".";
    TTS_TRY(conv_of(h, p + "start", &m.flow[b].start));
    TTS_TRY(conv_of(h, p + "end", &m.flow[b].end));
    TTS_TRY(conv_of(h, p + "cond", &m.flow[b].cond));
    TTS_TRY(fvec(h, p + "winv", &m.flow[b].winv));
    TTS_TRY(fvec(h, p + "an_bias", &m.flow[b].an_bias));
    TTS_TRY(fvec(h, p + "an_logs", &m.flow[b].an_logs));
  }
  for (int g = 0; g < 5; ++g)
    for (int i = 0; i < 4; ++i) {
      const std::string p = "flowgrp." + std::to_string(g) + ".";
      TTS_TRY(conv_of(h, p + "inl." + std::to_string(i), &m.flowgrp[g].inl[i]));
      TTS_TRY(conv_of(h, p + "res_skip." + std::to_string(i), &m.flowgrp[g].res_skip[i]));
    }
  const Dev* logdet = find(h, "flow.logdet");
  m.scoring = logdet != nullptr;
  if (m.scoring) {
    TTS_CHECK_ARG(logdet->dtype == 3 && logdet->bytes == sizeof(double), "weight 'flow.logdet' is not one float64 as two int32 words of host metadata");
    memcpy(&m.flow_logdet, logdet->p, sizeof(double));
    for (int b = 0; b < 18; ++b) {
      const std::string p = "flow." + std::to_string(b) + ".";
      TTS_TRY(fvec(h, p + "wfwd", &m.flow_fwd[b].wfwd));
      TTS_TRY(conv_of(h, p + "end_ml", &m.flow_fwd[b].end_ml));
      const ConvW& e = m.flow_fwd[b].end_ml;
      TTS_CHECK_ARG(e.mode == TTS_MODE_LINEAR && e.cin == ATT && e.cout == 160 && e.taps == 1, "weight '%send_ml' is not a plain 1-tap 192 -> 160 conv", p.c_str());
    }
  }
  m.resolved = true;
  return TTS_OK;
}

int resolve_vocoder(Handle* h) {
  Vocoder& m = h->vocoder;
  if (m.resolved) return TTS_OK;
  const bool big = h->cfg.vocoder == 2;
  TTS_TRY(conv_of(h, "voc.pre", &m.pre));
  for (int i = 0; i < 4; ++i) {
    TTS_TRY(conv_of(h, "voc.ups." + std::to_string(i), &m.ups[i]));
    for (int j = 0; j < 3; ++j)
      for (int dd = 0; dd < 3; ++dd) {
        const std::string p = "voc.blk." + std::to_string(i) + "." + std::to_string(j) + "." + std::to_string(dd);
        auto& k = m.blk[i][j][dd];
        TTS_TRY(conv_of(h, p + ".c1", &k.c1));
        TTS_TRY(conv_of(h, p + ".c2", &k.c2));
        if (!big) continue;
        TTS_TRY(fvec(h, p + ".a1", &k.a1));
        TTS_TRY(fvec(h, p + ".b1", &k.b1));
        TTS_TRY(fvec(h, p + ".a2", &k.a2));
        TTS_TRY(fvec(h, p + ".b2", &k.b2));
      }
  }
  TTS_TRY(fvec(h, "voc.post_w", &m.post_w));
  if (big) {
    TTS_TRY(fvec(h, "voc.post_a", &m.post_a));
    TTS_TRY(fvec(h, "voc.post_b", &m.post_b));
    TTS_TRY(fvec(h, "voc.filt", &m.filt));
    const Dev* ft;
    TTS_TRY(need(h, "voc.fir_tab", &ft));
    m.fir_tab = ft->p;
  }
  m.resolved = true;
  return TTS_OK;
}

bool is16(const Handle* h) { return h->cfg.precision == TTS_COMPUTE_BF16 || h->cfg.precision == TTS_COMPUTE_F16; }
int bits16(const Handle* h) { return is16(h) ? 16 : 32; }
bool postflow_cond_buffer(const Handle* h) { return !is16(h); }

int ensure_ptabs(Handle* h, hipStream_t st) {
  const Dev* pe;
  TTS_TRY(need(h, "pe", &pe));
  const int rows = (int)pe->shape[0], pmax = (rows + 1) / 2;
  if (h->pmax == pmax && h->ptab[0]) return TTS_OK;
  TTS_TRY(hip_ok(hipStreamSynchronize(st), "position tables: sync"));
  for (int s = 0; s < 2; ++s) {
    if (h->ptab[s]) (void)hipFree(h->ptab[s]);
    TTS_TRY(hip_ok(hipMalloc(reinterpret_cast<void**>(&h->ptab[s]), (size_t)6 * rows * ATT * sizeof(float)), "position tables: hipMalloc"));
  }
  int one = rows;
  const Layout l = Layout::make(&one, 1, 1);
  for (int s = 0; s < 2; ++s)
    for (int b = 0; b < 6; ++b) {
      ConvOpt o;
      o.fp32_only = true;
      o.no_split_k = true;
      TTS_TRY(conv(h, (s ? h->acoustic.dec : h->acoustic.enc)[b].pos, T2(pe->p, ATT), T2(h->ptab[s] + (size_t)b * rows * ATT, ATT), l, st, o));
    }
  h->pmax = pmax;
  return TTS_OK;
}

int ffn_fused(Handle* h, const Dev* fused, const ConvW& w1, const ConvW& w2, const float* g, const float* b, const float* post_g, const float* post_b,
              float* x, int R, hipStream_t st) {
  TtsFfnDesc d;
  memset(&d, 0, sizeof(d));
  d.x = x; d.ldx = ATT; d.y = x; d.ldy = ATT; d.rows = R; d.channels = ATT;
  d.ln_g = g; d.ln_b = b;
  d.w = fused->p; d.b2 = w2.bias;
  d.post_g = post_g; d.post_b = post_b;
  d.hidden = (int)(fused->bytes / (28 * 1024)) * 32;
  d.compute = w1.compute16; d.alpha = 0.5f; d.eps = 1e-12f;
  return prof_launch(h, d.compute == TTS_COMPUTE_F16 ? "ffn_fused_f16" : "ffn_fused_bf16", 4.0 * R * ATT * d.hidden,
                     (double)R * ATT * 8 + (double)fused->bytes, (double)R * ATT, st, [&] { return tts_ffn_fused(&d, st); });
}

int conformer(Handle* h, int stack, float* x, const Layout& l, Arena& a, hipStream_t st) {
  const int R = l.total, kernel = stack ? 31 : 7;
  if (l.max_len > h->pmax) {
    set_error("conformer: %d positions exceed the uploaded position table (pmax %d): upload a larger 'pe'", l.max_len, h->pmax);
    return TTS_E_ARG;
  }
  const int b16 = bits16(h);
  TTS_ALLOC(ln, a, float, (size_t)R * ATT);
  TTS_ALLOC(hid, a, char, (size_t)R * 1536 * (b16 / 8));
  TTS_ALLOC(qkv, a, float, (size_t)R * 3 * ATT);
  TTS_ALLOC(ctx, a, float, (size_t)R * ATT);
  TTS_ALLOC(glu, a, float, (size_t)R * ATT);
  TTS_ALLOC(dwo, a, float, (size_t)R * ATT);
  TileTab t128, t64;
  TTS_TRY(tiles_of(h, l, 128, st, &t128));
  TTS_TRY(tiles_of(h, l, 64, st, &t64));
  const size_t prow = (size_t)(2 * h->pmax - 1) * ATT;
  for (int bi = 0; bi < 6; ++bi) {
    const Block& b = (stack ? h->acoustic.dec : h->acoustic.enc)[bi];
    ConvOpt relu, half, res1;
    relu.act = TTS_ACT_RELU;
    half.alpha = 0.5f; half.res = T2(x, ATT);
    res1.res = T2(x, ATT);
    const bool fuse_ffn = b16 == 16;
    if (fuse_ffn && b.ffm_fused) {
      TTS_TRY(ffn_fused(h, b.ffm_fused, b.ffm1, b.ffm2, b.ln_g[0], b.ln_b[0], nullptr, nullptr, x, R, st));
    } else {
      TTS_TRY(tts_layernorm(x, ATT, ln, ATT, b.ln_g[0], b.ln_b[0], R, ATT, 1e-12f, st));
      TTS_TRY(conv(h, b.ffm1, T2(ln, ATT), T2(hid, 1536, b16), l, st, relu));
      TTS_TRY(conv(h, b.ffm2, T2(hid, 1536, b16), T2(x, ATT), l, st, half));
    }
    TTS_TRY(tts_layernorm(x, ATT, ln, ATT, b.ln_g[1], b.ln_b[1], R, ATT, 1e-12f, st));
    TTS_TRY(conv(h, b.qkv, T2(ln, ATT), T2(qkv, 3 * ATT), l, st));
    if (b16 == 16)
      TTS_TRY(tts_relpos_attention_f16(qkv, 3 * ATT, h->ptab[stack] + bi * prow, h->pmax, b.u, b.v, ctx, ATT, HEADS, DK, t128.dev, t128.n, 128, st));
    else
      TTS_TRY(tts_relpos_attention(qkv, 3 * ATT, h->ptab[stack] + bi * prow, h->pmax, b.u, b.v, ctx, ATT, HEADS, DK, t128.dev, t128.n, 128,
                                   h->split_mode == 2 ? TTS_ATT_KEY_SPLIT_ALWAYS : (h->split_mode == 1 ? TTS_ATT_KEY_SPLIT : 0), st));
    TTS_TRY(conv(h, b.out, T2(ctx, ATT), T2(x, ATT), l, st, res1));
    TTS_TRY(tts_layernorm(x, ATT, ln, ATT, b.ln_g[2], b.ln_b[2], R, ATT, 1e-12f, st));
    TTS_TRY(conv(h, b.pw1, T2(ln, ATT), T2(glu, ATT), l, st));
    TTS_TRY(tts_dwconv_swish(glu, ATT, dwo, ATT, b.dw_w, b.dw_b, ATT, kernel, t64.dev, t64.n, 64, st));
    TTS_TRY(conv(h, b.pw2, T2(dwo, ATT), T2(x, ATT), l, st, res1));
    if (fuse_ffn && b.ff_fused) {
      TTS_TRY(ffn_fused(h, b.ff_fused, b.ff1, b.ff2, b.ln_g[3], b.ln_b[3], b.ln_g[4], b.ln_b[4], x, R, st));
    } else {
      TTS_TRY(tts_layernorm(x, ATT, ln, ATT, b.ln_g[3], b.ln_b[3], R, ATT, 1e-12f, st));
      TTS_TRY(conv(h, b.ff1, T2(ln, ATT), T2(hid, 1536, b16), l, st, relu));
      TTS_TRY(conv(h, b.ff2, T2(hid, 1536, b16), T2(x, ATT), l, st, half));
      TTS_TRY(tts_layernorm(x, ATT, x, ATT, b.ln_g[4], b.ln_b[4], R, ATT, 1e-12f, st));
    }
  }
  return TTS_OK;
}

size_t conformer_bytes(size_t R) { return R * (ATT * 4 * 4 + 1536 * 4 + 3 * ATT * 4) + 8 * 256; }

size_t phone_arena_bytes(size_t R, size_t B) {
  return conformer_bytes(R) + R * (100 + 3 * ATT + 6 * 256 + 16) * 4 + B * (64 + 2 * ATT + 24 * 256 + 8) * 4 + (1 << 16);
}
size_t frame_arena_bytes(size_t RF, bool cond_buffer) {
  return conformer_bytes(RF) + RF * ((80 + ATT) + 2 * ATT + 3 * 80 + 2 * 256 + ATT + 160 + 4 * ATT + ATT + (cond_buffer ? 8 * ATT : 0) + 64) * 4 + (64 << 20);
}
size_t vocoder_stage_bytes(size_t R, int stage, bool fused_mode, bool big) {
  static const int UPS[4] = {8, 48, 192, 384};
  const size_t ch = 256 >> stage, rows = R * UPS[stage], se = fused_mode ? 2 : 4;
  const bool fused = fused_mode && ch <= 128;
  const size_t tensors = 4 + (fused ? 0 : (big ? 3 : 1));
  return tensors * (((rows * ch * se) + 255) & ~(size_t)255) + (1 << 20);
}
size_t vocoder_arena_bytes(size_t R, int arena, bool fused_mode, bool big) {
  size_t m = arena == 1 ? R * 512 * 4 + (1 << 20) : 0;
  for (int i = arena; i < 4; i += 2) m = std::max(m, vocoder_stage_bytes(R, i, fused_mode, big));
  return m;
}
size_t with_growth_slack(size_t bytes) { return bytes + bytes / 8 + (1 << 20); }

int predictor(Handle* h, const Predictor& p, float* out, hipStream_t st) {
  const Layout& l = h->lp;
  const int R = l.total;
  TTS_ALLOC(a, h->phone, float, (size_t)R * 256);
  TTS_ALLOC(bb, h->phone, float, (size_t)R * 256);
  TileTab t64;
  TTS_TRY(tiles_of(h, l, 64, st, &t64));
  const float* cur = h->enc;
  int ld = ATT;
  for (int i = 0; i < p.layers; ++i) {
    ConvOpt o;
    o.act = TTS_ACT_RELU;
    o.fp32_only = true;
    TTS_TRY(conv(h, p.conv[i], T2(const_cast<float*>(cur), ld), T2(a, 256), l, st, o));
    if (h->cfg.multispeaker) {
      const float* sc = h->cln + (size_t)(2 * (p.first_cln + i)) * h->B * 256;
      TTS_TRY(tts_cond_layernorm(a, 256, bb, 256, sc, sc + (size_t)h->B * 256, 256, t64.dev, t64.n, 64, st));
    } else {
      TTS_TRY(tts_layernorm(a, 256, bb, 256, p.g[i], p.b[i], R, 256, 1e-12f, st));
    }
    cur = bb;
    ld = 256;
  }
  ConvOpt o;
  o.fp32_only = true;
  return conv(h, p.lin, T2(const_cast<float*>(cur), ld), T2(out, 1), l, st, o);
}

}

int pipeline_create(const TtsConfig* cfg, Handle** out) {
  TTS_CHECK_ARG(cfg && out, "tts_create: null pointer");
  TTS_CHECK_ARG(cfg->precision >= 0 && cfg->precision <= 3, "tts_create: precision %d (0 fp32, 1 bf16, 2 fp16, 3 split fp32)", cfg->precision);
// ... 790 lines not shown
```

### ims-toucan-prosody-variance_amd/engine.py

```python
import ctypes as C
import math

import numpy as np
import torch

from . import capi, packing
from .capi import (ACT_NONE, ACT_RELU, ACT_TANH, COMPUTE_BF16, COMPUTE_F16, COMPUTE_F32, COMPUTE_F32X3, MODE_COUPLING, MODE_GATED, MODE_GLU,
                   MODE_LINEAR, PRE_LRELU, PRE_NONE, PRE_SNAKE)
from .ragged import Ragged

ATT, HEADS, DK = 192, 4, 48


def _ptr(t):
    return 0 if t is None else t.data_ptr()


def _is_bf16(t):
    return t is not None and t.dtype in (torch.bfloat16, torch.float16)


def _f16_flag(*ts):
    return capi.IO_F16 if any(t is not None and t.dtype == torch.float16 for t in ts) else 0


def precision_of(bf16, precision):
    name = precision if precision is not None else ("bf16" if bf16 else "f32")
    if name in ("fp32", "f32"):
        return "f32", False, COMPUTE_F32, torch.float32
    if name in ("f32x3", "fp32x3"):
        return "f32x3", "x3", COMPUTE_F32X3, torch.float32
    if name == "bf16":
        return "bf16", "bf16", COMPUTE_BF16, torch.bfloat16
    if name in ("fp16", "f16"):
        return "f16", "f16", COMPUTE_F16, torch.float16
    raise ValueError(f"precision {name!r}: expected f32, bf16 or f16")


def _ld(t):
    if t is None:
        return 0
    if t.dim() == 1:
        return 1
    assert t.stride(-1) == 1, "kernels need unit channel stride"
    return t.stride(0)


class Ops:

    def __init__(self, device, lib=None):
        self.lib = capi.lib() if lib is None else lib
        self.device = torch.device(device)
        if self.device.type == "cuda" and self.device.index is None:
            self.device = torch.device("cuda", torch.cuda.current_device())
        if isinstance(self.lib, C.CDLL) and self.device.type != "cuda":
            raise capi.ToucanHipError(f"device {str(self.device)!r}: libtoucan_hip.so has no CPU path - construct the engines / the "
                                      f"interface with device='cuda' (the reference's default 'cpu' cannot be served)")
        self.timer = None
        self.split_k = 0
        self.small_tile_blocks = 1536
        self._fir_tabs = {}
        self.default_compute = COMPUTE_F32

    def stream(self):
        if self.device.type == "cuda":
            return torch.cuda.current_stream(self.device).cuda_stream
        return 0

    def empty(self, *shape, dtype=torch.float32):
        return torch.empty(*shape, dtype=dtype, device=self.device)

    def conv(self, cw, x, y, rag, pre=PRE_NONE, pre_slope=0.0, act=ACT_NONE, alpha=1.0, seqvec=None, preadd=None, res=None,
             res_scale=1.0, aux=None, accumulate=False, compute=None, snake=None, split_k=True):
        if compute is None:
            compute = self.default_compute
        tile_rows = cw.tile_rows
        if self.small_tile_blocks and cw.small_tile_rows and not cw.small_only:
            cols = cw.wn if cw.mode == MODE_LINEAR else cw.half_pad
            if -(-rag.total_rows // cw.tile_rows) * (cols // cw.n_tile) < self.small_tile_blocks:
                tile_rows = cw.small_tile_rows
        tiles, n_tiles = rag.tiles(tile_rows)
        d = capi.TtsConvDesc()
        d.x, d.ldx, d.cin = x.data_ptr(), _ld(x), cw.cin
        use_bf16 = compute != COMPUTE_F32 and cw.w16 is not None
        if use_bf16 and cw.compute16 == COMPUTE_F32X3:
            cols = cw.wn if cw.mode == MODE_LINEAR else cw.half_pad
            small = n_tiles * (tile_rows // 64) * (-(-cols // 64)) <= 128
            if self.split_k == 2 or (self.split_k == 1 and small):
                use_bf16 = False
        d.w = cw.w16.data_ptr() if use_bf16 else cw.w.data_ptr()
        d.cin_pad, d.wn, d.half_pad = cw.cin_pad, cw.wn, cw.half_pad
        d.bias = _ptr(cw.bias)
        d.y, d.ldy, d.cout = y.data_ptr(), _ld(y), cw.cout
        d.taps, d.dil, d.pad_left = cw.taps, cw.dil, cw.pad_left
        d.pre_act, d.pre_slope = pre, pre_slope
        if snake is not None:
            d.snake_alpha, d.snake_beta, d.snake_filt = snake[0].data_ptr(), snake[1].data_ptr(), snake[2].data_ptr()
        d.mode, d.act, d.alpha = cw.mode, act, alpha
        d.seqvec, d.ld_seqvec = _ptr(seqvec), _ld(seqvec)
        d.preadd, d.ld_preadd = _ptr(preadd), _ld(preadd)
        d.res, d.ld_res, d.res_scale = _ptr(res), _ld(res), res_scale
        d.aux, d.ld_aux = _ptr(aux), _ld(aux)
        d.accumulate = 1 if accumulate else 0
        d.compute = cw.compute16 if use_bf16 else COMPUTE_F32
        d.io_flags = (capi.IO_X_BF16 if _is_bf16(x) else 0) | (capi.IO_Y_BF16 if _is_bf16(y) else 0) | (capi.IO_RES_BF16 if _is_bf16(res) else 0) \
            | _f16_flag(x, y, res)
        if split_k and self.split_k and self.default_compute in (COMPUTE_F32, COMPUTE_F32X3) and d.compute == COMPUTE_F32:
            d.io_flags |= capi.IO_SPLIT_K_ALWAYS if self.split_k == 2 else capi.IO_SPLIT_K
        d.tiles, d.n_tiles, d.tile_rows = tiles.data_ptr(), n_tiles, tile_rows
        tm = self.timer
        if tm is not None and tm.wants(cw, d.compute, tile_rows):
            ev0, ev1 = tm.events()
            ev0.record()
            capi.check(self.lib.tts_conv1d(C.byref(d), self.stream()), "tts_conv1d")
            ev1.record()
            tm.add(cw, d.compute, sum(rag.lengths), ev0, ev1, tile_rows, x.element_size(), y.element_size())
        else:
            capi.check(self.lib.tts_conv1d(C.byref(d), self.stream()), "tts_conv1d")
        return y

    def resblock_step(self, c1, c2, x, y, rag, act, slope=0.1, snake1=None, snake2=None, filt=None, alpha=1.0, res_scale=1.0,
                      accumulate=False, fir_tab=None):
        tile_rows = self.lib.tts_resblock_tile_rows(c1.cin)
        tiles, n_tiles = rag.tiles(tile_rows)
        d = capi.TtsResblockDesc()
        d.x, d.ldx, d.y, d.ldy = x.data_ptr(), _ld(x), y.data_ptr(), _ld(y)
        d.c, d.taps, d.dil = c1.cin, c1.taps, c1.dil
        d.w1, d.b1, d.w2, d.b2 = c1.w16.data_ptr(), c1.bias.data_ptr(), c2.w16.data_ptr(), c2.bias.data_ptr()
        assert c1.compute16 == c2.compute16 != COMPUTE_F32
        d.compute = c1.compute16
        d.act, d.slope = act, slope
        if snake1 is not None:
            d.alpha1, d.beta1 = snake1[0].data_ptr(), snake1[1].data_ptr()
            d.alpha2, d.beta2 = snake2[0].data_ptr(), snake2[1].data_ptr()
            d.filt = filt.data_ptr()
            if fir_tab is None:
                key = (filt.data_ptr(), str(filt.device))
                if key not in self._fir_tabs:
                    self._fir_tabs[key] = (packing.snake_fir_table(filt.detach().cpu().numpy(), filt.device), filt)
                fir_tab = self._fir_tabs[key][0]
            d.fir_tab = fir_tab.data_ptr()
        d.alpha, d.res_scale, d.accumulate = alpha, res_scale, 1 if accumulate else 0
        assert x.dtype == y.dtype and (not _is_bf16(x) or (x.dtype == torch.float16) == (c1.compute16 == COMPUTE_F16))
        d.io_bf16 = 1 if _is_bf16(x) else 0
        d.tiles, d.n_tiles, d.tile_rows = tiles.data_ptr(), n_tiles, tile_rows
        tm = self.timer
        if tm is not None and tm.wants_name("resblock_step<%d>" % c1.cin):
            ev0, ev1 = tm.events()
            ev0.record()
            capi.check(self.lib.tts_resblock_step(C.byref(d), self.stream()), "tts_resblock_step")
            ev1.record()
            rows = sum(rag.lengths)
            nbytes = 2.0 * rows * c1.cin * x.element_size() + 2.0 * c1.taps * c1.cin * c1.cin * 2
            tm.add_named("resblock_step<%d>" % c1.cin, 2.0 * rows * c1.cin * c1.cin * c1.taps * 2, ev0, ev1, nbytes, float(rows) * c1.cin)
        else:
            capi.check(self.lib.tts_resblock_step(C.byref(d), self.stream()), "tts_resblock_step")
        return y

    def wavenet_layer(self, inl, res_skip, hs_in, hs_out, cond, rag):
        tiles, n = rag.tiles(64)
        d = capi.TtsWavenetDesc()
        d.hs_in, d.ld_in, d.hs_out, d.ld_out = hs_in.data_ptr(), _ld(hs_in), hs_out.data_ptr(), _ld(hs_out)
        d.cond, d.ld_cond = cond.data_ptr(), _ld(cond)
        d.w1, d.b1, d.w2, d.b2 = inl.w16.data_ptr(), inl.bias.data_ptr(), res_skip.w16.data_ptr(), res_skip.bias.data_ptr()
        assert inl.compute16 == res_skip.compute16 != COMPUTE_F32 and inl.wn == 384 and inl.taps == 5 and res_skip.wn == res_skip.cout
        d.cout2, d.compute = res_skip.cout, inl.compute16
        d.tiles, d.n_tiles, d.tile_rows = tiles.data_ptr(), n, 64
        capi.check(self.lib.tts_wavenet_layer(C.byref(d), self.stream()), "tts_wavenet_layer")
        return hs_out

    def ffn_fused(self, x, y, norm, fused, b2, rows, compute, post=None, alpha=0.5, eps=1e-12):
        d = capi.TtsFfnDesc()
        d.x, d.ldx, d.y, d.ldy, d.rows, d.channels = x.data_ptr(), _ld(x), y.data_ptr(), _ld(y), rows, x.shape[1]
        d.ln_g, d.ln_b = norm[0].data_ptr(), norm[1].data_ptr()
        d.w, d.b2 = fused.data_ptr(), b2.data_ptr()
        d.post_g, d.post_b = (post[0].data_ptr(), post[1].data_ptr()) if post is not None else (None, None)
        d.hidden, d.compute, d.alpha, d.eps = 32 * (fused.numel() // (14 * 1024)), compute, alpha, eps
        capi.check(self.lib.tts_ffn_fused(C.byref(d), self.stream()), "tts_ffn_fused")
        return y

    def layernorm(self, x, y, gamma, beta, rows, c, eps=1e-12):
        capi.check(self.lib.tts_layernorm(x.data_ptr(), _ld(x), y.data_ptr(), _ld(y), gamma.data_ptr(), beta.data_ptr(), rows, c, eps,
                                          self.stream()), "tts_layernorm")
        return y

    def cond_layernorm(self, x, y, scale, shift, c, rag):
        tiles, n = rag.tiles(64)
        capi.check(self.lib.tts_cond_layernorm(x.data_ptr(), _ld(x), y.data_ptr(), _ld(y), scale.data_ptr(), shift.data_ptr(), c,
                                               tiles.data_ptr(), n, 64, self.stream()), "tts_cond_layernorm")
        return y

    def cln_mlp(self, e_norm, weights, n_mlp, d_in, d_out):
        out = self.empty(n_mlp, e_norm.shape[0], d_out)
        capi.check(self.lib.tts_cln_mlp(e_norm.data_ptr(), e_norm.shape[0], d_in, d_out, weights.data_ptr(), n_mlp, out.data_ptr(),
                                        self.stream()), "tts_cln_mlp")
        return out

    def l2_normalize(self, x, y):
        capi.check(self.lib.tts_l2_normalize(x.data_ptr(), y.data_ptr(), x.shape[0], x.shape[1], self.stream()), "tts_l2_normalize")
        return y

    def groupnorm(self, x, y, gamma, beta, c, groups, rag, tanh, res=None, eps=1e-5):
        sb, se = rag.bounds()
        ws = self.empty(max(1, int(self.lib.tts_groupnorm_workspace_floats(rag.n_seq, rag.max_len, groups))))
        capi.check(self.lib.tts_groupnorm(x.data_ptr(), _ld(x), y.data_ptr(), _ld(y), gamma.data_ptr(), beta.data_ptr(), c, groups, eps,
                                          1 if tanh else 0, _ptr(res), _ld(res), sb.data_ptr(), se.data_ptr(), rag.n_seq, rag.max_len,
                                          ws.data_ptr(), self.stream()), "tts_groupnorm")
        return y

    def attention(self, qkv, ptab, pmax, bias_u, bias_v, ctx, rag, tile_rows=128, f16=False, flags=None):
        tiles, n = rag.tiles(tile_rows)
        args = (qkv.data_ptr(), _ld(qkv), ptab.data_ptr(), pmax, bias_u.data_ptr(), bias_v.data_ptr(), ctx.data_ptr(), _ld(ctx), HEADS, DK,
                tiles.data_ptr(), n, tile_rows)
        if f16:
            capi.check(self.lib.tts_relpos_attention_f16(*args, self.stream()), "tts_relpos_attention_f16")
            return ctx
        if flags is None:
            flags = 0 if self.default_compute not in (COMPUTE_F32, COMPUTE_F32X3) else {0: 0, 1: capi.ATT_KEY_SPLIT, 2: capi.ATT_KEY_SPLIT_ALWAYS}[self.split_k]
        capi.check(self.lib.tts_relpos_attention(*args, flags, self.stream()), "tts_relpos_attention")
        return ctx

    def dwconv_swish(self, x, y, w, b, c, k, rag):
        tiles, n = rag.tiles(64)
        capi.check(self.lib.tts_dwconv_swish(x.data_ptr(), _ld(x), y.data_ptr(), _ld(y), w.data_ptr(), b.data_ptr(), c, k,
                                             tiles.data_ptr(), n, 64, self.stream()), "tts_dwconv_swish")
        return y

    def duration_from_log(self, logd, dur):
        capi.check(self.lib.tts_duration_from_log(logd.data_ptr(), dur.data_ptr(), logd.numel(), self.stream()), "tts_duration_from_log")

    def prosody_control(self, text, pitch, energy, dur, rag, duration_scale, pitch_scale, energy_scale, pause_scale):
        sb, se = rag.bounds()
        capi.check(self.lib.tts_prosody_control(text.data_ptr(), _ld(text), pitch.data_ptr(), energy.data_ptr(), dur.data_ptr(),
                                                sb.data_ptr(), se.data_ptr(), rag.n_seq, duration_scale, pitch_scale, energy_scale,
                                                pause_scale, self.stream()), "tts_prosody_control")

    def length_regulate(self, enc, pitch, energy, wp, bp, we, be, dur, rag_phone, rag_frame, up, dec_in, dec_scale):
        pb, pe = rag_phone.bounds()
        fb, _ = rag_frame.bounds()
        capi.check(self.lib.tts_length_regulate(enc.data_ptr(), _ld(enc), pitch.data_ptr(), energy.data_ptr(), wp.data_ptr(),
                                                bp.data_ptr(), we.data_ptr(), be.data_ptr(), dur.data_ptr(), pb.data_ptr(), pe.data_ptr(),
                                                fb.data_ptr(), rag_phone.n_seq, rag_frame.max_len, rag_phone.max_len, enc.shape[1],
                                                up.data_ptr(), _ld(up), _ptr(dec_in), _ld(dec_in), dec_scale, self.stream()),
                   "tts_length_regulate")

    def glow_invconv_actnorm(self, x, rows, c, winv, an_bias, an_logs):
        capi.check(self.lib.tts_glow_invconv_actnorm(x.data_ptr(), _ld(x), rows, c, winv.data_ptr(), an_bias.data_ptr(), an_logs.data_ptr(),
                                                     self.stream()), "tts_glow_invconv_actnorm")

    def snake_aa(self, x, y, alpha, beta, filt, c, rag):
        tiles, n = rag.tiles(256)
        flags = (capi.IO_X_BF16 if _is_bf16(x) else 0) | (capi.IO_Y_BF16 if _is_bf16(y) else 0) | _f16_flag(x, y)
        capi.check(self.lib.tts_snake_aa(x.data_ptr(), _ld(x), y.data_ptr(), _ld(y), alpha.data_ptr(), beta.data_ptr(), filt.data_ptr(), c,
                                         tiles.data_ptr(), n, 256, flags, self.stream()), "tts_snake_aa")
        return y

    def conv_post(self, x, cin, w, bias, pre, slope, wav, rag):
        tiles, n = rag.tiles(256)
        capi.check(self.lib.tts_conv_post(x.data_ptr(), _ld(x), cin, w.data_ptr(), bias, pre, slope, wav.data_ptr(), tiles.data_ptr(), n,
                                          256, (capi.IO_X_BF16 if _is_bf16(x) else 0) | _f16_flag(x), self.stream()), "tts_conv_post")
        return wav

    def conv_post_snake(self, x, cin, w, bias, alpha, beta, filt, wav, rag):
        tr = self.lib.tts_conv_post_snake_tile_rows()
        tiles, n = rag.tiles(tr)
        capi.check(self.lib.tts_conv_post_snake(x.data_ptr(), _ld(x), cin, w.data_ptr(), bias, alpha.data_ptr(), beta.data_ptr(), filt.data_ptr(),
                                                wav.data_ptr(), tiles.data_ptr(), n, tr, (capi.IO_X_BF16 if _is_bf16(x) else 0) | _f16_flag(x), self.stream()),
                   "tts_conv_post_snake")
        return wav

    def gather_rows(self, src, idx, dst):
        capi.check(self.lib.tts_gather_rows(src.data_ptr(), _ld(src), idx.data_ptr(), dst.data_ptr(), _ld(dst), idx.numel(), src.shape[1],
                                            self.stream()), "tts_gather_rows")
        return dst


def _dev(a, device):
    return torch.from_numpy(np.ascontiguousarray(a, dtype=np.float32)).to(device)


class GraphCache:

    def __init__(self, device, max_entries=16):
        self.device = torch.device(device)
        self.entries = {}
        self.max_entries = max_entries

    def run(self, key, inputs, fn):
        entry = self.entries.get(key)
        if entry is None:
            if len(self.entries) >= self.max_entries:
                self.entries.clear()
            static = {k: (None if v is None else v.clone()) for k, v in inputs.items()}
            side = torch.cuda.Stream(self.device)
            side.wait_stream(torch.cuda.current_stream(self.device))
            with torch.cuda.stream(side):
                fn(**static)
            torch.cuda.current_stream(self.device).wait_stream(side)
            torch.cuda.synchronize(self.device)
            graph = torch.cuda.CUDAGraph()
            with torch.cuda.graph(graph):
                outs = fn(**static)
            entry = self.entries[key] = (graph, static, outs, fn)
            graph.replay()
            return outs
        graph, static, outs, _keep = entry
        for k, v in inputs.items():
            if v is not None:
                static[k].copy_(v)
        graph.replay()
        return outs


class ConformerWeights:

    def __init__(self, sd, prefix, kernel, device, bf16=False):
        self.kernel = kernel
        self.blocks = []
        pack = lambda *a, **k: packing.pack_conv(*a, bf16=bf16, **k)
        for b in range(6):
            p = f"{prefix}.encoders.{b}."
            blk = {}
            for ln in ("norm_ff_macaron", "norm_mha", "norm_conv", "norm_ff", "norm_final"):
                blk[ln] = (_dev(sd[p + ln + ".weight"], device), _dev(sd[p + ln + ".bias"], device))
            for ff in ("feed_forward_macaron", "feed_forward"):
                blk[ff + ".w1"] = pack(sd[p + ff + ".w_1.weight"], sd[p + ff + ".w_1.bias"], device)
                blk[ff + ".w2"] = pack(sd[p + ff + ".w_2.weight"], sd[p + ff + ".w_2.bias"], device)
                w1 = np.asarray(sd[p + ff + ".w_1.weight"])
                if bf16 in ("bf16", "f16", True) and (w1.ndim == 2 or w1.shape[2] == 1) and w1.shape[1] == ATT and w1.shape[0] % 32 == 0:
                    blk[ff + ".fused"] = packing.pack_ffn(w1, sd[p + ff + ".w_1.bias"], sd[p + ff + ".w_2.weight"], device, "f16" if bf16 == "f16" else "bf16")
            a = p + "self_attn."
            wqkv = np.concatenate([sd[a + f"linear_{n}.weight"] for n in "qkv"], axis=0)
            bqkv = np.concatenate([sd[a + f"linear_{n}.bias"] for n in "qkv"], axis=0)
            blk["qkv"] = pack(wqkv, bqkv, device)
            blk["out"] = pack(sd[a + "linear_out.weight"], sd[a + "linear_out.bias"], device)
            blk["pos"] = packing.pack_conv(sd[a + "linear_pos.weight"], None, device)
            blk["u"] = _dev(sd[a + "pos_bias_u"].reshape(-1), device)
            blk["v"] = _dev(sd[a + "pos_bias_v"].reshape(-1), device)
            c = p + "conv_module."
            blk["pw1"] = pack(sd[c + "pointwise_conv1.weight"], sd[c + "pointwise_conv1.bias"], device, mode=MODE_GLU)
            g = sd[c + "norm.weight"].astype(np.float64) / np.sqrt(sd[c + "norm.running_var"].astype(np.float64) + 1e-5)
            dw = sd[c + "depthwise_conv.weight"][:, 0, :].astype(np.float64) * g[:, None]
            db = (sd[c + "depthwise_conv.bias"].astype(np.float64) - sd[c + "norm.running_mean"].astype(np.float64)) * g \
                + sd[c + "norm.bias"].astype(np.float64)
            blk["dw_w"] = _dev(dw.T, device)
            blk["dw_b"] = _dev(db, device)
            blk["pw2"] = pack(sd[c + "pointwise_conv2.weight"], sd[c + "pointwise_conv2.bias"], device)
            self.blocks.append(blk)
        self.pmax = 0
        self.ptabs = None


class AcousticEngine:

    def __init__(self, state_dict, device, bf16=False, use_graphs=False, precision=None, pack_only=False):
        self.ops = None if pack_only else Ops(device)
        self.device = torch.device(device) if pack_only else self.ops.device
        self.precision, bf16, compute16, self.dt16 = precision_of(bf16, precision)
        self.bf16 = bf16 in ("bf16", "f16", True)
        self.use_graphs = use_graphs
        self._graphs = GraphCache(self.device)
        if bf16 and self.ops is not None:
            self.ops.default_compute = compute16
        dev = self.device
        sd = packing.fold_weight_norm(state_dict)
        self.multilingual = "encoder.language_embedding.weight" in sd
        self.multispeaker = "encoder.hs_emb_projection.weight" in sd
        pc = packing.pack_conv
        pcb = lambda *a, **k: packing.pack_conv(*a, bf16=bf16, **k)
        self.embed0 = pc(sd["encoder.embed.0.weight"], sd["encoder.embed.0.bias"], dev)
        self.embed2 = pc(sd["encoder.embed.2.weight"], sd["encoder.embed.2.bias"], dev)
        self.lang_table = _dev(sd["encoder.language_embedding.weight"], dev) if self.multilingual else None
        self.enc = ConformerWeights(sd, "encoder", 7, dev, bf16)
        self.dec = ConformerWeights(sd, "decoder", 31, dev, bf16)
        self.out_norm = (_dev(sd["encoder.output_norm.weight"], dev), _dev(sd["encoder.output_norm.bias"], dev))
        if self.multispeaker:
            hs = sd["encoder.hs_emb_projection.weight"]
            self.hs_h = pcb(hs[:, :ATT], None, dev)
            self.hs_e = pc(hs[:, ATT:], sd["encoder.hs_emb_projection.bias"], dev)
        self.pred = {}
        cln_blocks = []
        for name, layers, k in (("pitch_predictor", 7, 5), ("energy_predictor", 2, 3), ("duration_predictor", 3, 3)):
            convs = [pc(sd[f"{name}.conv.{i}.0.weight"], sd[f"{name}.conv.{i}.0.bias"], dev) for i in range(layers)]
            first = len(cln_blocks) // 2
            if not self.multispeaker:
                norms = [(_dev(sd[f"{name}.norms.{i}.weight"], dev), _dev(sd[f"{name}.norms.{i}.bias"], dev)) for i in range(layers)]
                self.pred[name] = (convs, norms, pc(sd[name + ".linear.weight"], sd[name + ".linear.bias"], dev))
                continue
            for i in range(layers):
                for which in ("W_scale", "W_bias"):
                    q = f"{name}.norms.{i}.{which}."
                    parts = []
                    for j in (0, 2, 4):
                        parts += [np.ascontiguousarray(np.asarray(sd[q + f"{j}.weight"], dtype=np.float32).T).reshape(-1),
                                  np.asarray(sd[q + f"{j}.bias"], dtype=np.float32).reshape(-1)]
                    cln_blocks.append(np.concatenate(parts))
            lin = pc(sd[name + ".linear.weight"], sd[name + ".linear.bias"], dev)
            self.pred[name] = (convs, first, lin)
        self.n_cln_mlp = len(cln_blocks)
        if cln_blocks:
            self.cln_weights = _dev(np.concatenate(cln_blocks), dev)
            assert cln_blocks[0].size == capi.lib().tts_cln_mlp_weight_floats(64, 256)
        self.pitch_w = _dev(sd["pitch_embed.0.weight"].reshape(-1), dev)
        self.pitch_b = _dev(sd["pitch_embed.0.bias"], dev)
        self.energy_w = _dev(sd["energy_embed.0.weight"].reshape(-1), dev)
        self.energy_b = _dev(sd["energy_embed.0.bias"], dev)
        self.feat_out = pcb(sd["feat_out.weight"], sd["feat_out.bias"], dev)
        self.postnet = [(pcb(sd[f"conv_postnet.postnet.{i}.0.weight"], None, dev), _dev(sd[f"conv_postnet.postnet.{i}.1.weight"], dev),
                         _dev(sd[f"conv_postnet.postnet.{i}.1.bias"], dev)) for i in range(5)]
        self.g_proj = pcb(sd["post_flow.g_proj.weight"], sd["post_flow.g_proj.bias"], dev)
        self.flow = []
# ... 409 lines not shown
```

### ims-toucan-prosody-variance_amd/profiling.py

```python
import torch

from . import capi


def kernel_class(cw, compute, tile_rows=None):
    dual = cw.mode != capi.MODE_LINEAR
    bm, bn = cw.tile_rows, cw.n_tile
    if tile_rows is not None and tile_rows != cw.tile_rows:
        bm, bn = tile_rows, 64
    prec = {capi.COMPUTE_F32: "f32", capi.COMPUTE_BF16: "bf16", capi.COMPUTE_F16: "f16", capi.COMPUTE_F32X3: "f32x3"}[compute]
    return "conv1d_%s<%dx%d%s>" % (prec, bm, bn, ",dual" if dual else "")


class ConvTimer:
    def __init__(self, select=None):
        self.select = select
        self.records = []
        self.enabled = True

    def wants(self, cw, compute, tile_rows=None):
        return self.enabled and (self.select is None or kernel_class(cw, compute, tile_rows) in self.select)

    def wants_name(self, name):
        return self.enabled and (self.select is None or name in self.select)

    def add_named(self, name, flops, ev0, ev1, nbytes=0.0, elems=0.0):
        self.records.append((name, flops, ev0, ev1, nbytes, elems))

    def events(self):
        return torch.cuda.Event(enable_timing=True), torch.cuda.Event(enable_timing=True)

    def add(self, cw, compute, rows, ev0, ev1, tile_rows=None, x_bytes=4, y_bytes=4):
        ctot = cw.cout * (2 if cw.mode != capi.MODE_LINEAR else 1)
        flops = 2.0 * rows * cw.cin * ctot * cw.algo_taps
        wbytes = cw.taps * cw.cin * ctot * (4 if compute == capi.COMPUTE_F32 else 2)
        nbytes = float(rows) * (cw.cin * x_bytes + cw.cout * y_bytes) + wbytes
        self.records.append((kernel_class(cw, compute, tile_rows), flops, ev0, ev1, nbytes, float(rows) * cw.cout))

    def summary(self):
        out = {}
        for name, flops, e0, e1, nbytes, elems in self.records:
            ms = e0.elapsed_time(e1)
            s = out.setdefault(name, dict(launches=0, total_ms=0.0, flops=0.0, bytes=0.0, elems=0.0))
            s["launches"] += 1
            s["total_ms"] += ms
            s["flops"] += flops
            s["bytes"] += nbytes
            s["elems"] += elems
        for s in out.values():
            s["avg_us"] = 1e3 * s["total_ms"] / s["launches"]
            s["flops_per_launch"] = s["flops"] / s["launches"]
            s["bytes_per_launch"] = s["bytes"] / s["launches"]
            s["elems_per_launch"] = s["elems"] / s["launches"]
            s["tflops"] = s["flops"] / (s["total_ms"] * 1e-3) / 1e12 if s["total_ms"] > 0 else 0.0
        return out

    def reset(self):
        self.records = []
```

### include/toucan_tts.h

```cpp
#ifndef TOUCAN_TTS_H
#define TOUCAN_TTS_H

#include <stdint.h>

#ifdef __cplusplus
extern "C" {
#endif

typedef void* tts_stream_t;

#define TTS_OK 0
#define TTS_E_ARG (-1)
#define TTS_E_LAUNCH (-2)

typedef struct {
  int32_t row0;
  int32_t seq_begin;
  int32_t seq_end;
  int32_t seq_id;
} TtsTile;

#define TTS_MODE_LINEAR 0
#define TTS_MODE_GLU 1
#define TTS_MODE_GATED 2
#define TTS_MODE_COUPLING 3
#define TTS_ACT_NONE 0
#define TTS_ACT_RELU 1
#define TTS_ACT_TANH 2
#define TTS_IO_X_BF16 1
#define TTS_IO_Y_BF16 2
#define TTS_IO_RES_BF16 4
#define TTS_IO_F16 8
#define TTS_IO_SPLIT_K 16
#define TTS_IO_SPLIT_K_ALWAYS 32
#define TTS_ATT_KEY_SPLIT 1
#define TTS_ATT_KEY_SPLIT_ALWAYS 2
#define TTS_COMPUTE_F32 0
#define TTS_COMPUTE_BF16 1
#define TTS_COMPUTE_F16 2
#define TTS_COMPUTE_F32X3 3
#define TTS_PRE_NONE 0
#define TTS_PRE_LRELU 1
#define TTS_PRE_SNAKE 2

typedef struct {
  const float* x;      int32_t ldx;  int32_t cin;
  const void*  w;      int32_t cin_pad; int32_t wn; int32_t half_pad;
  const float* bias;
  float* y;            int32_t ldy;  int32_t cout;
  int32_t taps, dil, pad_left;
  int32_t pre_act;     float pre_slope;
  const float* snake_alpha; const float* snake_beta; const float* snake_filt;
  int32_t mode, act;   float alpha;
  const float* seqvec; int32_t ld_seqvec;
  const float* preadd; int32_t ld_preadd;
  const float* res;    int32_t ld_res; float res_scale;
  const float* aux;    int32_t ld_aux;
  int32_t accumulate;
  int32_t compute;
  int32_t io_flags;
  const TtsTile* tiles; int32_t n_tiles; int32_t tile_rows;
} TtsConvDesc;

int tts_conv1d_tile_rows(int32_t cout, int32_t mode);
int tts_conv1d_n_tile(int32_t cout, int32_t mode);
int tts_conv1d_small_tile_rows(int32_t cout, int32_t mode, int32_t packed_cols);
int tts_conv1d(const TtsConvDesc* d, tts_stream_t stream);

typedef struct {
  const float* x; int32_t ldx;
  float* y;       int32_t ldy;
  int32_t c, taps, dil;
  const void* w1; const float* b1;
  const void* w2; const float* b2;
  int32_t act; float slope;
  const float* alpha1; const float* beta1; const float* alpha2; const float* beta2; const float* filt;
  float alpha, res_scale; int32_t accumulate;
  int32_t io_bf16;
  const TtsTile* tiles; int32_t n_tiles; int32_t tile_rows;
  int32_t compute;
  const void* fir_tab;
} TtsResblockDesc;

#define TTS_SNAKE_FIR_TABLE_BYTES 4096
int tts_snake_fir_table(const float* filt , void* table );

int tts_resblock_tile_rows(int32_t c);
int tts_resblock_step(const TtsResblockDesc* d, tts_stream_t stream);

typedef struct {
  const float* hs_in;  int32_t ld_in;
  float* hs_out;       int32_t ld_out;
  const float* cond;   int32_t ld_cond;
  const void* w1;      const float* b1;
  const void* w2;      const float* b2;
  int32_t cout2;
  int32_t compute;
  const TtsTile* tiles; int32_t n_tiles; int32_t tile_rows;
} TtsWavenetDesc;
int tts_wavenet_layer(const TtsWavenetDesc* d, tts_stream_t stream);

typedef struct {
  const float* x;      int32_t ldx;
  float* y;            int32_t ldy;
  int32_t rows;        int32_t channels;
  const float* ln_g;   const float* ln_b;
  const void* w;       const float* b2;
  const float* post_g; const float* post_b;
  int32_t hidden;      int32_t compute;
  float alpha;         float eps;
} TtsFfnDesc;
int tts_ffn_fused(const TtsFfnDesc* d, tts_stream_t stream);

int tts_layernorm(const float* x, int32_t ldx, float* y, int32_t ldy, const float* gamma, const float* beta,
                  int32_t rows, int32_t c, float eps, tts_stream_t stream);

int tts_cond_layernorm(const float* x, int32_t ldx, float* y, int32_t ldy, const float* scale, const float* shift,
                       int32_t c, const TtsTile* tiles, int32_t n_tiles, int32_t tile_rows, tts_stream_t stream);

int64_t tts_cln_mlp_weight_floats(int32_t d_in, int32_t d_out);
int tts_cln_mlp(const float* e, int32_t n_seq, int32_t d_in, int32_t d_out, const float* weights, int32_t n_mlp, float* out,
                tts_stream_t stream);

int tts_l2_normalize(const float* x, float* y, int32_t rows, int32_t c, tts_stream_t stream);

int tts_groupnorm(const float* x, int32_t ldx, float* y, int32_t ldy, const float* gamma, const float* beta,
                  int32_t c, int32_t groups, float eps, int32_t apply_tanh, const float* res, int32_t ld_res,
                  const int32_t* seq_begin, const int32_t* seq_end, int32_t n_seq, int32_t max_len, float* workspace,
                  tts_stream_t stream);
int64_t tts_groupnorm_workspace_floats(int32_t n_seq, int32_t max_len, int32_t groups);

int tts_relpos_attention(const float* qkv, int32_t ld_qkv, const float* ptab, int32_t pmax, const float* bias_u,
                         const float* bias_v, float* ctx, int32_t ld_ctx, int32_t heads, int32_t dk,
                         const TtsTile* tiles, int32_t n_tiles, int32_t tile_rows, int32_t flags, tts_stream_t stream);
int tts_relpos_attention_f16(const float* qkv, int32_t ld_qkv, const float* ptab, int32_t pmax, const float* bias_u,
                             const float* bias_v, float* ctx, int32_t ld_ctx, int32_t heads, int32_t dk,
                             const TtsTile* tiles, int32_t n_tiles, int32_t tile_rows, tts_stream_t stream);

int tts_dwconv_swish(const float* x, int32_t ldx, float* y, int32_t ldy, const float* w, const float* b, int32_t c,
                     int32_t k, const TtsTile* tiles, int32_t n_tiles, int32_t tile_rows, tts_stream_t stream);

int tts_duration_from_log(const float* logd, int32_t* dur, int32_t n, tts_stream_t stream);

int tts_prosody_control(const float* text, int32_t ld_text, float* pitch, float* energy, int32_t* dur,
                        const int32_t* seq_begin, const int32_t* seq_end, int32_t n_seq, float duration_scale,
                        float pitch_scale, float energy_scale, float pause_scale, tts_stream_t stream);

int tts_length_regulate(const float* enc, int32_t ld_enc, const float* pitch, const float* energy,
                        const float* wp, const float* bp, const float* we, const float* be, const int32_t* dur,
                        const int32_t* phone_begin, const int32_t* phone_end, const int32_t* frame_begin,
                        int32_t n_seq, int32_t max_frames, int32_t max_phones, int32_t c, float* up, int32_t ld_up,
                        float* dec_in, int32_t ld_dec, float dec_scale, tts_stream_t stream);

int tts_glow_invconv_actnorm(float* x, int32_t ldx, int32_t rows, int32_t c, const float* winv ,
                             const float* an_bias, const float* an_logs, tts_stream_t stream);

int tts_snake_aa(const float* x, int32_t ldx, float* y, int32_t ldy, const float* alpha, const float* beta,
                 const float* filt , int32_t c, const TtsTile* tiles, int32_t n_tiles, int32_t tile_rows,
                 int32_t io_flags , tts_stream_t stream);

int tts_conv_post(const float* x, int32_t ldx, int32_t cin, const float* w , float bias, int32_t pre_act,
                  float pre_slope, float* wav, const TtsTile* tiles, int32_t n_tiles, int32_t tile_rows,
                  int32_t io_flags , tts_stream_t stream);

int tts_conv_post_snake_tile_rows(void);
int tts_conv_post_snake(const float* x, int32_t ldx, int32_t cin, const float* w , float bias, const float* alpha,
                        const float* beta, const float* filt , float* wav, const TtsTile* tiles, int32_t n_tiles,
                        int32_t tile_rows, int32_t io_flags , tts_stream_t stream);

int tts_gather_rows(const float* src, int32_t ld_src, const int32_t* idx, float* dst, int32_t ld_dst, int32_t n,
                    int32_t c, tts_stream_t stream);


int tts_gru_layer(const float* x, int32_t ldx, int32_t batch, int32_t steps, int32_t in_dim, int32_t hidden, const float* w_ih_t,
                  const float* w_hh_t, const float* b_ih, const float* b_hh, float* y, int32_t ldy, tts_stream_t stream);
int tts_style_tokens(const float* q, const float* k, const float* v, int32_t batch, int32_t n_tokens, int32_t heads, int32_t dk, float* ctx,
                     tts_stream_t stream);
int tts_complex_magnitude(const float* x, int32_t ldx, float* y, int32_t ldy, int32_t rows, int32_t bins, tts_stream_t stream);
int tts_log10_floor(const float* x, int32_t ldx, float* y, int32_t ldy, int32_t rows, int32_t c, float eps, tts_stream_t stream);

typedef struct TtsHandle TtsHandle;

typedef struct {
  int32_t multilingual;
  int32_t multispeaker;
  int32_t vocoder;
  int32_t precision;
  int32_t small_tile_blocks;
  float post_bias;
} TtsConfig;

int tts_create(const TtsConfig* cfg, TtsHandle** out);
int tts_destroy(TtsHandle* h);

int tts_load_weights(TtsHandle* h, const char* name, const void* host_ptr, const int64_t* shape, int32_t ndim, int32_t dtype);

int64_t tts_workspace_bytes(const TtsHandle* h, int32_t B, int32_t Lmax, int32_t Tmax);
int64_t tts_workspace_claimed(const TtsHandle* h);
int tts_table_stats(const TtsHandle* h, int64_t* tables_built, int64_t* table_chunks);

int tts_encoder(TtsHandle* h, const float* text, const float* utt_emb, const int32_t* lang_ids, const int32_t* phone_lengths ,
                int32_t B, tts_stream_t stream);
int tts_variance_predictors(TtsHandle* h, const float* gold_pitch, const float* gold_energy, const int32_t* gold_durations,
                            tts_stream_t stream);
int tts_control_and_regulate(TtsHandle* h, float duration_scale, float pitch_scale, float energy_scale, float pause_scale,
                             int32_t* frame_counts , tts_stream_t stream);
int tts_decoder(TtsHandle* h, tts_stream_t stream);
int tts_postnet(TtsHandle* h, tts_stream_t stream);
int tts_postflow(TtsHandle* h, const float* z_noise, tts_stream_t stream);
int tts_mel(TtsHandle* h, const float** mel, int32_t* ld, int32_t* frame_begins , int32_t* frame_counts );
int tts_copy_mel(TtsHandle* h, float* dst, int32_t ld_dst, tts_stream_t stream);
int tts_prosody(TtsHandle* h, const int32_t** durations, const float** pitch, const float** energy);
int tts_copy_prosody(TtsHandle* h, int32_t* durations, float* pitch, float* energy, tts_stream_t stream);
int tts_profile(TtsHandle* h, int32_t enable, const char* select);
int32_t tts_profile_count(TtsHandle* h);
int tts_profile_read(TtsHandle* h, int32_t index, char* name, int32_t name_cap, double* ms, double* flops, double* bytes, double* elems);
int tts_vocoder_bigvgan(TtsHandle* h, const float* mel, int32_t ld_mel, const int32_t* frame_begins ,
                        const int32_t* frame_counts , int32_t B, float* wav, tts_stream_t stream);
int tts_vocoder_hifigan(TtsHandle* h, const float* mel, int32_t ld_mel, const int32_t* frame_begins ,
                        const int32_t* frame_counts , int32_t B, float* wav, tts_stream_t stream);
int tts_synthesize_batch(TtsHandle* h, const float* text, const float* utt_emb, const int32_t* lang_ids, const int32_t* phone_lengths ,
                         int32_t B, const float* gold_pitch, const float* gold_energy, const int32_t* gold_durations, float duration_scale,
                         float pitch_scale, float energy_scale, float pause_scale, const float* z_noise, int32_t* frame_begins ,
                         int32_t* frame_counts , float* wav, int64_t wav_capacity, int64_t* wav_needed , tts_stream_t stream);

const char* tts_last_error(void);
int tts_diag_queue_nonzero(void);
int tts_diag_queue_slots_used(void);
#define TTS_ABI_VERSION 15
int tts_abi_version(void);

#ifdef __cplusplus
}
#endif
#endif
```

Baseline: 578,900.

## Add wide 256x256 bf16 conv1d kernel with LDS DMA and polyphase tap skipping

Adds a new 256x256-tile conv1d kernel for linear bf16/f16 convolutions. It stages input windows and weight slabs into LDS via global_load_lds DMA with double buffering, and skips taps that are structurally zero for polyphase (2-of-3 tap) upsampling weights. The host routes eligible convs to it when the channel and tap count is large enough and the 256-row tile count fills the device's CUs. The shared epilogue moves to a header. The aim is better weight/input reuse and less wasted MFMA work on large convs, at the cost of extra LDS pressure, fewer blocks and a new code path.

```diff
diff --git a/ims-toucan-prosody-variance_amd/build.py b/ims-toucan-prosody-variance_amd/build.py
--- a/ims-toucan-prosody-variance_amd/build.py
+++ b/ims-toucan-prosody-variance_amd/build.py
@@ -5,7 +5,7 @@
 PKG = os.path.dirname(os.path.abspath(__file__))
 CSRC = os.path.join(PKG, "csrc")
 LIB = os.path.join(PKG, "libtoucan_hip.so")
-SOURCES = ["conv1d.hip", "resblock.hip", "rowops.hip", "attention_mfma.hip", "sequence_ops.hip", "capi.hip", "pipeline.hip", "style.hip", "wavenet.hip", "ffn.hip", "align.hip", "score.hip", "gan.hip", "pitch.hip", "train.hip", "resample.hip", "glow_forward.hip"]
+SOURCES = ["conv1d.hip", "conv1d_wide.hip", "resblock.hip", "rowops.hip", "attention_mfma.hip", "sequence_ops.hip", "capi.hip", "pipeline.hip", "style.hip", "wavenet.hip", "ffn.hip", "align.hip", "score.hip", "gan.hip", "pitch.hip", "train.hip", "resample.hip", "glow_forward.hip"]
 
 
 def _hipcc():
diff --git a/ims-toucan-prosody-variance_amd/capi.py b/ims-toucan-prosody-variance_amd/capi.py
--- a/ims-toucan-prosody-variance_amd/capi.py
+++ b/ims-toucan-prosody-variance_amd/capi.py
@@ -90,6 +90,7 @@
 IO_X_BF16, IO_Y_BF16, IO_RES_BF16, IO_F16 = 1, 2, 4, 8
 IO_SPLIT_K = 16
 IO_SPLIT_K_ALWAYS = 32
+IO_POLYPHASE = 64
 ATT_KEY_SPLIT, ATT_KEY_SPLIT_ALWAYS = 1, 2
 
 PROTOTYPES = {
diff --git a/ims-toucan-prosody-variance_amd/csrc/conv1d.hip b/ims-toucan-prosody-variance_amd/csrc/conv1d.hip
--- a/ims-toucan-prosody-variance_amd/csrc/conv1d.hip
+++ b/ims-toucan-prosody-variance_amd/csrc/conv1d.hip
@@ -2,6 +2,7 @@
 #include <type_traits>
 
 #include "common.h"
+#include "conv_epilogue.h"
 #include "snake.h"
 
 namespace tts {
@@ -61,203 +62,6 @@
   if constexpr (K < N) {
     f(std::integral_constant<int, K>{});
     static_for<K + 1, N>(f);
-  }
-}
-
-template <bool DUAL>
-__device__ __forceinline__ float epilogue_value(const TtsConvDesc& d, float a, float g, float ba, float bg, float sv, float pa, float pg, float ax,
-                                                float rv) {
-  float v = a + ba + sv;
-  if (d.preadd) v += pa;
-  if (DUAL) {
-    g += bg;
-    if (d.preadd) g += pg;
-    if (d.mode == TTS_MODE_GLU) {
-      v = v * (1.0f / (1.0f + expf(-g)));
-    } else if (d.mode == TTS_MODE_GATED) {
-      v = tanhf(v) * (1.0f / (1.0f + expf(-g)));
-    } else {
-      v = (ax - v) * expf(-g);
-    }
-  } else {
-    if (d.act == TTS_ACT_RELU) v = fmaxf(v, 0.0f);
-    else if (d.act == TTS_ACT_TANH) v = tanhf(v);
-  }
-  v *= d.alpha;
-  if (d.res) v += d.res_scale * rv;
-  return v;
-}
-
-template <bool DUAL>
-__device__ __forceinline__ void epilogue_element(const TtsConvDesc& d, int row, int n, float a, float g, float ba, float bg, float sv, bool io_f16) {
-  const float pa = d.preadd ? d.preadd[(size_t)row * d.ld_preadd + n] : 0.0f;
-  const float pg = (DUAL && d.preadd) ? d.preadd[(size_t)row * d.ld_preadd + d.cout + n] : 0.0f;
-  const float ax = (DUAL && d.mode == TTS_MODE_COUPLING) ? d.aux[(size_t)row * d.ld_aux + n] : 0.0f;
-  float rv = 0.0f;
-  if (d.res)
-    rv = (d.io_flags & TTS_IO_RES_BF16) ? load16(reinterpret_cast<const unsigned short*>(d.res)[(size_t)row * d.ld_res + n], io_f16)
-                                        : d.res[(size_t)row * d.ld_res + n];
-  float v = epilogue_value<DUAL>(d, a, g, ba, bg, sv, pa, pg, ax, rv);
-  if (d.io_flags & TTS_IO_Y_BF16) {
-    unsigned short* yp = reinterpret_cast<unsigned short*>(d.y) + (size_t)row * d.ldy + n;
-    if (d.accumulate) v += load16(*yp, io_f16);
-    *yp = store16(v, io_f16);
-  } else {
-    float* yp = d.y + (size_t)row * d.ldy + n;
-    if (d.accumulate) v += *yp;
-    *yp = v;
-  }
-}
-
-__device__ __forceinline__ bool epilogue_vec_ok(const TtsConvDesc& d) {
-  auto al = [](const void* p, unsigned m) { return (reinterpret_cast<uintptr_t>(p) & (m - 1)) == 0; };
-  bool ok = (d.cout & 3) == 0 && (d.ldy & 3) == 0 && al(d.y, (d.io_flags & TTS_IO_Y_BF16) ? 8 : 16);
-  if (d.bias) ok = ok && al(d.bias, 16);
-  if (d.seqvec) ok = ok && (d.ld_seqvec & 3) == 0 && al(d.seqvec, 16);
-  if (d.preadd) ok = ok && (d.ld_preadd & 3) == 0 && al(d.preadd, 16);
-  if (d.res) ok = ok && (d.ld_res & 3) == 0 && al(d.res, (d.io_flags & TTS_IO_RES_BF16) ? 8 : 16);
-  if (d.mode == TTS_MODE_COUPLING) ok = ok && (d.ld_aux & 3) == 0 && al(d.aux, 16);
-  return ok;
-}
-
-template <int TM, int TN, int NH, bool DUAL>
-__device__ __forceinline__ void conv_epilogue_t(const TtsConvDesc& d, const TtsTile& tile, int n0, int wm, int wn, int lrow, int lk,
-                                                const f32x16 (&acc)[NH][TM][TN], const float* eb = nullptr, int eb_n = 0) {
-  const bool io_f16 = d.io_flags & TTS_IO_F16;
-  const bool vec = epilogue_vec_ok(d);
-  const bool y16 = d.io_flags & TTS_IO_Y_BF16, r16 = d.io_flags & TTS_IO_RES_BF16;
-  if constexpr (!DUAL) {
-    if (vec && !d.preadd && eb) {
-      auto col_of = [&](int j, int rq) { return n0 + (wn * TN + j) * 32 + 8 * rq + 4 * lk; };
-#pragma unroll
-      for (int i = 0; i < TM; ++i) {
-        const int row = tile.row0 + (wm * TM + i) * 32 + lrow;
-        const int rowc = row < tile.seq_end ? row : tile.seq_end - 1;
-        constexpr int NG = TN * 4, CH = 8;
-#pragma unroll
-        for (int g0 = 0; g0 < NG; g0 += CH) {
-        uint4 rv[CH], yv[CH];
-#pragma unroll
-          for (int g = 0; g < CH; ++g) {
-            if (g0 + g >= NG) continue;
-            const int j = (g0 + g) >> 2, rq = (g0 + g) & 3;
-            int n = col_of(j, rq);
-            n = n < d.cout ? n : d.cout - 4;
-            rv[g] = make_uint4(0, 0, 0, 0);
-            yv[g] = make_uint4(0, 0, 0, 0);
-            if (d.res) {
-              if (r16) {
-                const uint2 u = *reinterpret_cast<const uint2*>(reinterpret_cast<const unsigned short*>(d.res) + (size_t)rowc * d.ld_res + n);
-                rv[g].x = u.x; rv[g].y = u.y;
-              } else {
-                rv[g] = *reinterpret_cast<const uint4*>(d.res + (size_t)rowc * d.ld_res + n);
-              }
-            }
-            if (d.accumulate) {
-              if (y16) {
-                const uint2 u = *reinterpret_cast<const uint2*>(reinterpret_cast<const unsigned short*>(d.y) + (size_t)rowc * d.ldy + n);
-                yv[g].x = u.x; yv[g].y = u.y;
-              } else {
-                yv[g] = *reinterpret_cast<const uint4*>(d.y + (size_t)rowc * d.ldy + n);
-              }
-            }
-          }
-        __builtin_amdgcn_sched_barrier(0);
-        if (row < tile.seq_end) {
-#pragma unroll
-          for (int g = 0; g < CH; ++g) {
-            if (g0 + g >= NG) continue;
-            const int j = (g0 + g) >> 2, rq = (g0 + g) & 3;
-            const int n = col_of(j, rq);
-            if (n >= d.cout) continue;
-            const float4 ba = *reinterpret_cast<const float4*>(eb + (n - n0));
-            const float4 sv = *reinterpret_cast<const float4*>(eb + eb_n + (n - n0));
-            const uint4 ru = rv[g], yu = yv[g];
-            float4 r4, y4;
-            if (r16) r4 = make_float4(load16(ru.x & 0xFFFF, io_f16), load16(ru.x >> 16, io_f16), load16(ru.y & 0xFFFF, io_f16), load16(ru.y >> 16, io_f16));
-            else r4 = make_float4(__builtin_bit_cast(float, ru.x), __builtin_bit_cast(float, ru.y), __builtin_bit_cast(float, ru.z), __builtin_bit_cast(float, ru.w));
-            if (y16) y4 = make_float4(load16(yu.x & 0xFFFF, io_f16), load16(yu.x >> 16, io_f16), load16(yu.y & 0xFFFF, io_f16), load16(yu.y >> 16, io_f16));
-            else y4 = make_float4(__builtin_bit_cast(float, yu.x), __builtin_bit_cast(float, yu.y), __builtin_bit_cast(float, yu.z), __builtin_bit_cast(float, yu.w));
-            float v0 = epilogue_value<false>(d, acc[0][i][j][4 * rq + 0], 0.f, ba.x, 0.f, sv.x, 0.f, 0.f, 0.f, r4.x);
-            float v1 = epilogue_value<false>(d, acc[0][i][j][4 * rq + 1], 0.f, ba.y, 0.f, sv.y, 0.f, 0.f, 0.f, r4.y);
-            float v2 = epilogue_value<false>(d, acc[0][i][j][4 * rq + 2], 0.f, ba.z, 0.f, sv.z, 0.f, 0.f, 0.f, r4.z);
-            float v3 = epilogue_value<false>(d, acc[0][i][j][4 * rq + 3], 0.f, ba.w, 0.f, sv.w, 0.f, 0.f, 0.f, r4.w);
-            if (d.accumulate) { v0 += y4.x; v1 += y4.y; v2 += y4.z; v3 += y4.w; }
-            if (y16) {
-              uint2* yp = reinterpret_cast<uint2*>(reinterpret_cast<unsigned short*>(d.y) + (size_t)row * d.ldy + n);
-              *yp = make_uint2((unsigned int)store16(v0, io_f16) | ((unsigned int)store16(v1, io_f16) << 16),
-                               (unsigned int)store16(v2, io_f16) | ((unsigned int)store16(v3, io_f16) << 16));
-            } else {
-              *reinterpret_cast<float4*>(d.y + (size_t)row * d.ldy + n) = make_float4(v0, v1, v2, v3);
-            }
-          }
-        }
-        __builtin_amdgcn_sched_barrier(0);
-        }
-      }
-      return;
-    }
-  }
-#pragma unroll
-  for (int i = 0; i < TM; ++i) {
-    const int row = tile.row0 + (wm * TM + i) * 32 + lrow;
-    if (row >= tile.seq_end) continue;
-#pragma unroll
-    for (int j = 0; j < TN; ++j) {
-#pragma unroll
-      for (int rq = 0; rq < 4; ++rq) {
-        const int n = n0 + (wn * TN + j) * 32 + 8 * rq + 4 * lk;
-        if (n >= d.cout) continue;
-        if (!vec) {
-          for (int q = 0; q < 4 && n + q < d.cout; ++q) {
-            const float ba = d.bias ? d.bias[n + q] : 0.0f;
-            const float bg = (DUAL && d.bias) ? d.bias[d.cout + n + q] : 0.0f;
-            const float sv = d.seqvec ? d.seqvec[(size_t)tile.seq_id * d.ld_seqvec + n + q] : 0.0f;
-            epilogue_element<DUAL>(d, row, n + q, acc[0][i][j][4 * rq + q], acc[NH - 1][i][j][4 * rq + q], ba, bg, sv, io_f16);
-          }
-          continue;
-        }
-        const float4 z4 = make_float4(0.f, 0.f, 0.f, 0.f);
-        auto ld4 = [](const float* p) { return *reinterpret_cast<const float4*>(p); };
-        const float4 ba = d.bias ? ld4(d.bias + n) : z4;
-        const float4 bg = (DUAL && d.bias) ? ld4(d.bias + d.cout + n) : z4;
-        const float4 sv = d.seqvec ? ld4(d.seqvec + (size_t)tile.seq_id * d.ld_seqvec + n) : z4;
-        const float4 pa = d.preadd ? ld4(d.preadd + (size_t)row * d.ld_preadd + n) : z4;
-        const float4 pg = (DUAL && d.preadd) ? ld4(d.preadd + (size_t)row * d.ld_preadd + d.cout + n) : z4;
-        const float4 ax = (DUAL && d.mode == TTS_MODE_COUPLING) ? ld4(d.aux + (size_t)row * d.ld_aux + n) : z4;
-        float4 rv = z4;
-        if (d.res) {
-          if (r16) {
-            const uint2 u = *reinterpret_cast<const uint2*>(reinterpret_cast<const unsigned short*>(d.res) + (size_t)row * d.ld_res + n);
-            rv = make_float4(load16(u.x & 0xFFFF, io_f16), load16(u.x >> 16, io_f16), load16(u.y & 0xFFFF, io_f16), load16(u.y >> 16, io_f16));
-          } else {
-            rv = ld4(d.res + (size_t)row * d.ld_res + n);
-          }
-        }
-        float v[4];
-        v[0] = epilogue_value<DUAL>(d, acc[0][i][j][4 * rq + 0], acc[NH - 1][i][j][4 * rq + 0], ba.x, bg.x, sv.x, pa.x, pg.x, ax.x, rv.x);
-        v[1] = epilogue_value<DUAL>(d, acc[0][i][j][4 * rq + 1], acc[NH - 1][i][j][4 * rq + 1], ba.y, bg.y, sv.y, pa.y, pg.y, ax.y, rv.y);
-        v[2] = epilogue_value<DUAL>(d, acc[0][i][j][4 * rq + 2], acc[NH - 1][i][j][4 * rq + 2], ba.z, bg.z, sv.z, pa.z, pg.z, ax.z, rv.z);
-        v[3] = epilogue_value<DUAL>(d, acc[0][i][j][4 * rq + 3], acc[NH - 1][i][j][4 * rq + 3], ba.w, bg.w, sv.w, pa.w, pg.w, ax.w, rv.w);
-        if (y16) {
-          uint2* yp = reinterpret_cast<uint2*>(reinterpret_cast<unsigned short*>(d.y) + (size_t)row * d.ldy + n);
-          if (d.accumulate) {
-            const uint2 u = *yp;
-            v[0] += load16(u.x & 0xFFFF, io_f16); v[1] += load16(u.x >> 16, io_f16);
-            v[2] += load16(u.y & 0xFFFF, io_f16); v[3] += load16(u.y >> 16, io_f16);
-          }
-          *yp = make_uint2((unsigned int)store16(v[0], io_f16) | ((unsigned int)store16(v[1], io_f16) << 16),
-                           (unsigned int)store16(v[2], io_f16) | ((unsigned int)store16(v[3], io_f16) << 16));
-        } else {
-          float4* yp = reinterpret_cast<float4*>(d.y + (size_t)row * d.ldy + n);
-          if (d.accumulate) {
-            const float4 u = *yp;
-            v[0] += u.x; v[1] += u.y; v[2] += u.z; v[3] += u.w;
-          }
-          *yp = make_float4(v[0], v[1], v[2], v[3]);
-        }
-      }
-    }
   }
 }
 
@@ -1112,6 +916,8 @@
   return launch_status("conv1d (1-tap rows)");
 }
 
+int conv1d_wide_launch(const TtsConvDesc& d, hipStream_t st);
+
 int conv1d_dispatch(const TtsConvDesc& d, hipStream_t st) {
   TTS_CHECK_ARG(d.x && d.w && d.y && d.tiles, "conv1d: null pointer");
   TTS_CHECK_ARG(d.cin > 0 && d.cout > 0 && d.taps > 0 && d.dil > 0, "conv1d: bad dims");
@@ -1127,6 +933,7 @@
   const int cols = d.mode == TTS_MODE_LINEAR ? d.wn : d.half_pad;
   ConvShape s = pick_shape(d.cout, d.mode);
   if (d.tile_rows == 64 && small_form_ok(d.cout, d.mode, cols)) s = d.mode == TTS_MODE_LINEAR ? S_64x64 : S_D64x64;
+  if (d.tile_rows == 256 && s != S_256x32) return conv1d_wide_launch(d, st);
   int bm, bn;
   shape_dims(s, bm, bn);
   TTS_CHECK_ARG(d.tile_rows == bm, "conv1d: tile table built for %d rows, kernel needs %d", d.tile_rows, bm);
diff --git a/ims-toucan-prosody-variance_amd/csrc/conv1d_wide.hip b/ims-toucan-prosody-variance_amd/csrc/conv1d_wide.hip
--- /dev/null
+++ b/ims-toucan-prosody-variance_amd/csrc/conv1d_wide.hip
@@ -0,0 +1,185 @@
+#include "common.h"
+#include "conv_epilogue.h"
+
+namespace tts {
+
+namespace {
+
+constexpr int WIDE_BM = 256, WIDE_BN = 256, WIDE_BK = 64, WIDE_THREADS = 512;
+constexpr int WIDE_ROW_BYTES = WIDE_BK * 2;
+constexpr int WIDE_SLAB_BYTES = WIDE_BK * WIDE_BN * 2;
+
+__host__ __device__ inline int wide_win_rows(int taps, int dil) { return (WIDE_BM + (taps - 1) * dil + 7) & ~7; }
+inline size_t wide_lds_bytes(int taps, int dil) {
+  return (size_t)2 * wide_win_rows(taps, dil) * WIDE_ROW_BYTES + 2 * WIDE_SLAB_BYTES + 2 * WIDE_BN * sizeof(float);
+}
+
+__device__ __forceinline__ void wide_dma16(const void* src, void* lds_wave_base) {
+  __builtin_amdgcn_global_load_lds((const void __attribute__((address_space(1)))*)src, (void __attribute__((address_space(3)))*)lds_wave_base, 16, 0, 0);
+}
+
+template <bool F16>
+__global__ __launch_bounds__(WIDE_THREADS) void conv1d_wide_kernel(const TtsConvDesc d) {
+  constexpr int TM = 4, TN = 2;
+  extern __shared__ __attribute__((aligned(16))) unsigned char lds_raw[];
+
+  const TtsTile tile = d.tiles[blockIdx.x];
+  const int n0 = blockIdx.y * WIDE_BN;
+  const int win_rows = wide_win_rows(d.taps, d.dil);
+  const int win_bytes = win_rows * WIDE_ROW_BYTES;
+  unsigned char* const xs0 = lds_raw;
+  unsigned char* const ws0 = lds_raw + 2 * win_bytes;
+  float* const eb = reinterpret_cast<float*>(ws0 + 2 * WIDE_SLAB_BYTES);
+
+  const int tid = threadIdx.x;
+  const int lane = tid & 63;
+  const int wave = __builtin_amdgcn_readfirstlane(tid >> 6);
+  const int wm = wave >> 2, wn = wave & 3;
+  const int lrow = lane & 31, lk = lane >> 5;
+
+  f32x16 acc[1][TM][TN];
+#pragma unroll
+  for (int i = 0; i < TM; ++i)
+#pragma unroll
+    for (int j = 0; j < TN; ++j)
+#pragma unroll
+      for (int r = 0; r < 16; ++r) acc[0][i][j][r] = 0.0f;
+
+  if (tid < WIDE_BN) {
+    const int n = n0 + tid;
+    eb[tid] = (d.bias && n < d.cout) ? d.bias[n] : 0.0f;
+    eb[WIDE_BN + tid] = 0.0f;
+  }
+
+  const bool poly = d.io_flags & TTS_IO_POLYPHASE;
+  const int half = d.wn >> 1;
+  const int tap_lo = (poly && n0 >= half) ? 1 : 0;
+  const int tap_hi = (poly && n0 + WIDE_BN <= half) ? 2 : d.taps;
+  const int wc0 = n0 + wn * 64;
+  const int skip_tap = !poly ? -1 : (wc0 >= half ? 0 : (wc0 + 64 <= half ? 2 : -1));
+
+  const int row_first = tile.row0 - d.pad_left;
+  const bool edge = row_first < tile.seq_begin || row_first + win_rows > tile.seq_end;
+  const unsigned short* __restrict__ xh = reinterpret_cast<const unsigned short*>(d.x);
+  const unsigned short* __restrict__ W = reinterpret_cast<const unsigned short*>(d.w);
+  const int n_chunks = d.cin / WIDE_BK;
+  const int n_win_inst = win_rows >> 3;
+
+  auto request_window = [&](int ch) __attribute__((always_inline)) {
+    unsigned char* xb = xs0 + (ch & 1) * win_bytes;
+    for (int i = wave; i < n_win_inst; i += 8) {
+      const int wr = i * 8 + (lane >> 3);
+      const int g = (lane & 7) ^ ((wr >> 1) & 7);
+      const int gr = row_first + wr;
+      const int grc = gr < tile.seq_begin ? tile.seq_begin : (gr >= tile.seq_end ? tile.seq_end - 1 : gr);
+      wide_dma16(xh + (size_t)grc * d.ldx + ch * WIDE_BK + g * 8, xb + i * 1024);
+    }
+  };
+  auto zero_window_edges = [&](int ch) __attribute__((always_inline)) {
+    unsigned char* xb = xs0 + (ch & 1) * win_bytes;
+    for (int i = wave; i < n_win_inst; i += 8) {
+      const int gr = row_first + i * 8 + (lane >> 3);
+      if (gr < tile.seq_begin || gr >= tile.seq_end) *reinterpret_cast<uint4*>(xb + i * 1024 + lane * 16) = make_uint4(0, 0, 0, 0);
+    }
+  };
+  auto request_weights = [&](int ch, int tap, int buf) __attribute__((always_inline)) {
+    unsigned char* wb = ws0 + buf * WIDE_SLAB_BYTES;
+#pragma unroll
+    for (int q = 0; q < 4; ++q) {
+      const int idx = q * 8 + wave;
+      const int kb = idx >> 2, part = idx & 3;
+      const size_t goff = (((size_t)tap * (d.cin_pad >> 3) + ch * 8 + kb) * d.wn + n0 + part * 64 + lane) * 8;
+      wide_dma16(W + goff, wb + idx * 1024);
+    }
+  };
+
+  request_window(0);
+  request_weights(0, tap_lo, 0);
+  bool zero_pending = edge;
+  int zero_ch = 0;
+
+  int step = 0;
+  for (int ch = 0; ch < n_chunks; ++ch) {
+    const unsigned char* xb = xs0 + (ch & 1) * win_bytes;
+    for (int tap = tap_lo; tap < tap_hi; ++tap, ++step) {
+      asm volatile("s_waitcnt vmcnt(0)" ::: "memory");
+      if (zero_pending) {
+        zero_window_edges(zero_ch);
+        zero_pending = false;
+      }
+      asm volatile("s_waitcnt lgkmcnt(0)\n\ts_barrier" ::: "memory");
+      {
+        const bool last_tap = tap + 1 == tap_hi;
+        const int nch = last_tap ? ch + 1 : ch, ntap = last_tap ? tap_lo : tap + 1;
+        if (nch < n_chunks) request_weights(nch, ntap, (step + 1) & 1);
+      }
+      if (tap == tap_lo && ch + 1 < n_chunks) {
+        request_window(ch + 1);
+        zero_pending = edge;
+        zero_ch = ch + 1;
+      }
+      if (tap == skip_tap) continue;
+      const unsigned char* wb = ws0 + (step & 1) * WIDE_SLAB_BYTES;
+      const int r0 = wm * 128 + lrow + tap * d.dil;
+#pragma unroll
+      for (int ks = 0; ks < 4; ++ks) {
+        const int g = ks * 2 + lk;
+        bf16x8 a[TM], b[TN];
+#pragma unroll
+        for (int j = 0; j < TN; ++j) b[j] = *reinterpret_cast<const bf16x8*>(wb + (size_t)(g * WIDE_BN + wn * 64 + j * 32 + lrow) * 16);
+#pragma unroll
+        for (int i = 0; i < TM; ++i) {
+          const int r = r0 + i * 32;
+          a[i] = *reinterpret_cast<const bf16x8*>(xb + r * WIDE_ROW_BYTES + ((g ^ ((r >> 1) & 7)) << 4));
+        }
+#pragma unroll
+        for (int i = 0; i < TM; ++i)
+#pragma unroll
+          for (int j = 0; j < TN; ++j) acc[0][i][j] = mfma16<F16>(b[j], a[i], acc[0][i][j]);
+      }
+    }
+  }
+  conv_epilogue_t<TM, TN, 1, false, true>(d, tile, n0, wm, wn, lrow, lk, acc, eb, WIDE_BN);
+}
+
+}
+
+const char* conv1d_wide_reject(const TtsConvDesc& d) {
+  auto al16 = [](const void* p) { return (reinterpret_cast<uintptr_t>(p) & 15) == 0; };
+  if (d.compute != TTS_COMPUTE_BF16 && d.compute != TTS_COMPUTE_F16) return "compute must be bf16 or fp16";
+  if (d.mode != TTS_MODE_LINEAR) return "mode must be LINEAR";
+  if (!(d.io_flags & TTS_IO_X_BF16) || !(d.io_flags & TTS_IO_Y_BF16) || (d.res && !(d.io_flags & TTS_IO_RES_BF16))) return "x, y and res must be 16-bit tensors";
+  if (((d.io_flags & TTS_IO_F16) != 0) != (d.compute == TTS_COMPUTE_F16)) return "the 16-bit tensors must be in the call's own format";
+  if (d.pre_act != TTS_PRE_NONE) return "no pre-activation";
+  if (d.seqvec || d.preadd || d.aux) return "no seqvec, preadd or aux";
+  if (d.cin != d.cin_pad || d.cin % WIDE_BK != 0) return "cin must be unpadded and a multiple of 64";
+  if (d.wn % WIDE_BN != 0 || d.cout > d.wn) return "wn must be a multiple of 256";
+  if ((d.cout & 3) || (d.bias && !al16(d.bias))) return "cout must be a multiple of 4 and the bias 16-byte aligned";
+  if ((d.ldx & 7) || (d.ldy & 7) || (d.res && (d.ld_res & 7)) || !al16(d.x) || !al16(d.y) || !al16(d.w) || (d.res && !al16(d.res))) return "rows and pointers must be 16-byte aligned";
+  if ((d.io_flags & TTS_IO_POLYPHASE) && d.taps != 3) return "TTS_IO_POLYPHASE needs taps == 3";
+  if (wide_lds_bytes(d.taps, d.dil) > 160 * 1024) return "the window does not fit in 160 KiB of LDS";
+  return nullptr;
+}
+
+int conv1d_wide_launch(const TtsConvDesc& d, hipStream_t st) {
+  const char* why = conv1d_wide_reject(d);
+  TTS_CHECK_ARG(why == nullptr, "conv1d: a 256-row tile table asks for the wide tile, which this call cannot take: %s", why);
+  const size_t lds = wide_lds_bytes(d.taps, d.dil);
+  dim3 grid(d.n_tiles, d.wn / WIDE_BN), block(WIDE_THREADS);
+  auto launch = [&](auto k, unsigned long long& raised) {
+    if (lds > 64 * 1024) {
+      const hipError_t e = raise_lds_limit(reinterpret_cast<const void*>(k), raised);
+      if (e != hipSuccess) {
+        set_error("conv1d (wide): raising the dynamic LDS limit failed: %s", hipGetErrorString(e));
+        return (int)TTS_E_LAUNCH;
+      }
+    }
+    hipLaunchKernelGGL(k, grid, block, lds, st, d);
+    return launch_status("conv1d (wide)");
+  };
+  static unsigned long long raised_bf16 = 0, raised_f16 = 0;
+  if (d.compute == TTS_COMPUTE_F16) return launch(conv1d_wide_kernel<true>, raised_f16);
+  return launch(conv1d_wide_kernel<false>, raised_bf16);
+}
+
+}
diff --git a/ims-toucan-prosody-variance_amd/csrc/conv_epilogue.h b/ims-toucan-prosody-variance_amd/csrc/conv_epilogue.h
--- /dev/null
+++ b/ims-toucan-prosody-variance_amd/csrc/conv_epilogue.h
@@ -0,0 +1,203 @@
+#pragma once
+#include "common.h"
+
+namespace tts {
+
+template <bool DUAL>
+__device__ __forceinline__ float epilogue_value(const TtsConvDesc& d, float a, float g, float ba, float bg, float sv, float pa, float pg, float ax,
+                                                float rv) {
+  float v = a + ba + sv;
+  if (d.preadd) v += pa;
+  if (DUAL) {
+    g += bg;
+    if (d.preadd) g += pg;
+    if (d.mode == TTS_MODE_GLU) {
+      v = v * (1.0f / (1.0f + expf(-g)));
+    } else if (d.mode == TTS_MODE_GATED) {
+      v = tanhf(v) * (1.0f / (1.0f + expf(-g)));
+    } else {
+      v = (ax - v) * expf(-g);
+    }
+  } else {
+    if (d.act == TTS_ACT_RELU) v = fmaxf(v, 0.0f);
+    else if (d.act == TTS_ACT_TANH) v = tanhf(v);
+  }
+  v *= d.alpha;
+  if (d.res) v += d.res_scale * rv;
+  return v;
+}
+
+template <bool DUAL>
+__device__ __forceinline__ void epilogue_element(const TtsConvDesc& d, int row, int n, float a, float g, float ba, float bg, float sv, bool io_f16) {
+  const float pa = d.preadd ? d.preadd[(size_t)row * d.ld_preadd + n] : 0.0f;
+  const float pg = (DUAL && d.preadd) ? d.preadd[(size_t)row * d.ld_preadd + d.cout + n] : 0.0f;
+  const float ax = (DUAL && d.mode == TTS_MODE_COUPLING) ? d.aux[(size_t)row * d.ld_aux + n] : 0.0f;
+  float rv = 0.0f;
+  if (d.res)
+    rv = (d.io_flags & TTS_IO_RES_BF16) ? load16(reinterpret_cast<const unsigned short*>(d.res)[(size_t)row * d.ld_res + n], io_f16)
+                                        : d.res[(size_t)row * d.ld_res + n];
+  float v = epilogue_value<DUAL>(d, a, g, ba, bg, sv, pa, pg, ax, rv);
+  if (d.io_flags & TTS_IO_Y_BF16) {
+    unsigned short* yp = reinterpret_cast<unsigned short*>(d.y) + (size_t)row * d.ldy + n;
+    if (d.accumulate) v += load16(*yp, io_f16);
+    *yp = store16(v, io_f16);
+  } else {
+    float* yp = d.y + (size_t)row * d.ldy + n;
+    if (d.accumulate) v += *yp;
+    *yp = v;
+  }
+}
+
+__device__ __forceinline__ bool epilogue_vec_ok(const TtsConvDesc& d) {
+  auto al = [](const void* p, unsigned m) { return (reinterpret_cast<uintptr_t>(p) & (m - 1)) == 0; };
+  bool ok = (d.cout & 3) == 0 && (d.ldy & 3) == 0 && al(d.y, (d.io_flags & TTS_IO_Y_BF16) ? 8 : 16);
+  if (d.bias) ok = ok && al(d.bias, 16);
+  if (d.seqvec) ok = ok && (d.ld_seqvec & 3) == 0 && al(d.seqvec, 16);
+  if (d.preadd) ok = ok && (d.ld_preadd & 3) == 0 && al(d.preadd, 16);
+  if (d.res) ok = ok && (d.ld_res & 3) == 0 && al(d.res, (d.io_flags & TTS_IO_RES_BF16) ? 8 : 16);
+  if (d.mode == TTS_MODE_COUPLING) ok = ok && (d.ld_aux & 3) == 0 && al(d.aux, 16);
+  return ok;
+}
+
+template <int TM, int TN, int NH, bool DUAL, bool FAST_ONLY = false>
+__device__ __forceinline__ void conv_epilogue_t(const TtsConvDesc& d, const TtsTile& tile, int n0, int wm, int wn, int lrow, int lk,
+                                                const f32x16 (&acc)[NH][TM][TN], const float* eb = nullptr, int eb_n = 0) {
+  const bool io_f16 = d.io_flags & TTS_IO_F16;
+  const bool vec = epilogue_vec_ok(d);
+  const bool y16 = d.io_flags & TTS_IO_Y_BF16, r16 = d.io_flags & TTS_IO_RES_BF16;
+  if constexpr (!DUAL) {
+    if (FAST_ONLY || (vec && !d.preadd && eb)) {
+      auto col_of = [&](int j, int rq) { return n0 + (wn * TN + j) * 32 + 8 * rq + 4 * lk; };
+#pragma unroll
+      for (int i = 0; i < TM; ++i) {
+        const int row = tile.row0 + (wm * TM + i) * 32 + lrow;
+        const int rowc = row < tile.seq_end ? row : tile.seq_end - 1;
+        constexpr int NG = TN * 4, CH = 8;
+#pragma unroll
+        for (int g0 = 0; g0 < NG; g0 += CH) {
+        uint4 rv[CH], yv[CH];
+#pragma unroll
+          for (int g = 0; g < CH; ++g) {
+            if (g0 + g >= NG) continue;
+            const int j = (g0 + g) >> 2, rq = (g0 + g) & 3;
+            int n = col_of(j, rq);
+            n = n < d.cout ? n : d.cout - 4;
+            rv[g] = make_uint4(0, 0, 0, 0);
+            yv[g] = make_uint4(0, 0, 0, 0);
+            if (d.res) {
+              if (r16) {
+                const uint2 u = *reinterpret_cast<const uint2*>(reinterpret_cast<const unsigned short*>(d.res) + (size_t)rowc * d.ld_res + n);
+                rv[g].x = u.x; rv[g].y = u.y;
+              } else {
+                rv[g] = *reinterpret_cast<const uint4*>(d.res + (size_t)rowc * d.ld_res + n);
+              }
+            }
+            if (d.accumulate) {
+              if (y16) {
+                const uint2 u = *reinterpret_cast<const uint2*>(reinterpret_cast<const unsigned short*>(d.y) + (size_t)rowc * d.ldy + n);
+                yv[g].x = u.x; yv[g].y = u.y;
+              } else {
+                yv[g] = *reinterpret_cast<const uint4*>(d.y + (size_t)rowc * d.ldy + n);
+              }
+            }
+          }
+        __builtin_amdgcn_sched_barrier(0);
+        if (row < tile.seq_end) {
+#pragma unroll
+          for (int g = 0; g < CH; ++g) {
+            if (g0 + g >= NG) continue;
+            const int j = (g0 + g) >> 2, rq = (g0 + g) & 3;
+            const int n = col_of(j, rq);
+            if (n >= d.cout) continue;
+            const float4 ba = *reinterpret_cast<const float4*>(eb + (n - n0));
+            const float4 sv = *reinterpret_cast<const float4*>(eb + eb_n + (n - n0));
+            const uint4 ru = rv[g], yu = yv[g];
+            float4 r4, y4;
+            if (r16) r4 = make_float4(load16(ru.x & 0xFFFF, io_f16), load16(ru.x >> 16, io_f16), load16(ru.y & 0xFFFF, io_f16), load16(ru.y >> 16, io_f16));
+            else r4 = make_float4(__builtin_bit_cast(float, ru.x), __builtin_bit_cast(float, ru.y), __builtin_bit_cast(float, ru.z), __builtin_bit_cast(float, ru.w));
+            if (y16) y4 = make_float4(load16(yu.x & 0xFFFF, io_f16), load16(yu.x >> 16, io_f16), load16(yu.y & 0xFFFF, io_f16), load16(yu.y >> 16, io_f16));
+            else y4 = make_float4(__builtin_bit_cast(float, yu.x), __builtin_bit_cast(float, yu.y), __builtin_bit_cast(float, yu.z), __builtin_bit_cast(float, yu.w));
+            float v0 = epilogue_value<false>(d, acc[0][i][j][4 * rq + 0], 0.f, ba.x, 0.f, sv.x, 0.f, 0.f, 0.f, r4.x);
+            float v1 = epilogue_value<false>(d, acc[0][i][j][4 * rq + 1], 0.f, ba.y, 0.f, sv.y, 0.f, 0.f, 0.f, r4.y);
+            float v2 = epilogue_value<false>(d, acc[0][i][j][4 * rq + 2], 0.f, ba.z, 0.f, sv.z, 0.f, 0.f, 0.f, r4.z);
+            float v3 = epilogue_value<false>(d, acc[0][i][j][4 * rq + 3], 0.f, ba.w, 0.f, sv.w, 0.f, 0.f, 0.f, r4.w);
+            if (d.accumulate) { v0 += y4.x; v1 += y4.y; v2 += y4.z; v3 += y4.w; }
+            if (y16) {
+              uint2* yp = reinterpret_cast<uint2*>(reinterpret_cast<unsigned short*>(d.y) + (size_t)row * d.ldy + n);
+              *yp = make_uint2((unsigned int)store16(v0, io_f16) | ((unsigned int)store16(v1, io_f16) << 16),
+                               (unsigned int)store16(v2, io_f16) | ((unsigned int)store16(v3, io_f16) << 16));
+            } else {
+              *reinterpret_cast<float4*>(d.y + (size_t)row * d.ldy + n) = make_float4(v0, v1, v2, v3);
+            }
+          }
+        }
+        __builtin_amdgcn_sched_barrier(0);
+        }
+      }
+      return;
+    }
+  }
+#pragma unroll
+  for (int i = 0; i < TM; ++i) {
+    const int row = tile.row0 + (wm * TM + i) * 32 + lrow;
+    if (row >= tile.seq_end) continue;
+#pragma unroll
+    for (int j = 0; j < TN; ++j) {
+#pragma unroll
+      for (int rq = 0; rq < 4; ++rq) {
+        const int n = n0 + (wn * TN + j) * 32 + 8 * rq + 4 * lk;
+        if (n >= d.cout) continue;
+        if (!vec) {
+          for (int q = 0; q < 4 && n + q < d.cout; ++q) {
+            const float ba = d.bias ? d.bias[n + q] : 0.0f;
+            const float bg = (DUAL && d.bias) ? d.bias[d.cout + n + q] : 0.0f;
+            const float sv = d.seqvec ? d.seqvec[(size_t)tile.seq_id * d.ld_seqvec + n + q] : 0.0f;
+            epilogue_element<DUAL>(d, row, n + q, acc[0][i][j][4 * rq + q], acc[NH - 1][i][j][4 * rq + q], ba, bg, sv, io_f16);
+          }
+          continue;
+        }
+        const float4 z4 = make_float4(0.f, 0.f, 0.f, 0.f);
+        auto ld4 = [](const float* p) { return *reinterpret_cast<const float4*>(p); };
+        const float4 ba = d.bias ? ld4(d.bias + n) : z4;
+        const float4 bg = (DUAL && d.bias) ? ld4(d.bias + d.cout + n) : z4;
+        const float4 sv = d.seqvec ? ld4(d.seqvec + (size_t)tile.seq_id * d.ld_seqvec + n) : z4;
+        const float4 pa = d.preadd ? ld4(d.preadd + (size_t)row * d.ld_preadd + n) : z4;
+        const float4 pg = (DUAL && d.preadd) ? ld4(d.preadd + (size_t)row * d.ld_preadd + d.cout + n) : z4;
+        const float4 ax = (DUAL && d.mode == TTS_MODE_COUPLING) ? ld4(d.aux + (size_t)row * d.ld_aux + n) : z4;
+        float4 rv = z4;
+        if (d.res) {
+          if (r16) {
+            const uint2 u = *reinterpret_cast<const uint2*>(reinterpret_cast<const unsigned short*>(d.res) + (size_t)row * d.ld_res + n);
+            rv = make_float4(load16(u.x & 0xFFFF, io_f16), load16(u.x >> 16, io_f16), load16(u.y & 0xFFFF, io_f16), load16(u.y >> 16, io_f16));
+          } else {
+            rv = ld4(d.res + (size_t)row * d.ld_res + n);
+          }
+        }
+        float v[4];
+        v[0] = epilogue_value<DUAL>(d, acc[0][i][j][4 * rq + 0], acc[NH - 1][i][j][4 * rq + 0], ba.x, bg.x, sv.x, pa.x, pg.x, ax.x, rv.x);
+        v[1] = epilogue_value<DUAL>(d, acc[0][i][j][4 * rq + 1], acc[NH - 1][i][j][4 * rq + 1], ba.y, bg.y, sv.y, pa.y, pg.y, ax.y, rv.y);
+        v[2] = epilogue_value<DUAL>(d, acc[0][i][j][4 * rq + 2], acc[NH - 1][i][j][4 * rq + 2], ba.z, bg.z, sv.z, pa.z, pg.z, ax.z, rv.z);
+        v[3] = epilogue_value<DUAL>(d, acc[0][i][j][4 * rq + 3], acc[NH - 1][i][j][4 * rq + 3], ba.w, bg.w, sv.w, pa.w, pg.w, ax.w, rv.w);
+        if (y16) {
+          uint2* yp = reinterpret_cast<uint2*>(reinterpret_cast<unsigned short*>(d.y) + (size_t)row * d.ldy + n);
+          if (d.accumulate) {
+            const uint2 u = *yp;
+            v[0] += load16(u.x & 0xFFFF, io_f16); v[1] += load16(u.x >> 16, io_f16);
+            v[2] += load16(u.y & 0xFFFF, io_f16); v[3] += load16(u.y >> 16, io_f16);
+          }
+          *yp = make_uint2((unsigned int)store16(v[0], io_f16) | ((unsigned int)store16(v[1], io_f16) << 16),
+                           (unsigned int)store16(v[2], io_f16) | ((unsigned int)store16(v[3], io_f16) << 16));
+        } else {
+          float4* yp = reinterpret_cast<float4*>(d.y + (size_t)row * d.ldy + n);
+          if (d.accumulate) {
+            const float4 u = *yp;
+            v[0] += u.x; v[1] += u.y; v[2] += u.z; v[3] += u.w;
+          }
+          *yp = make_float4(v[0], v[1], v[2], v[3]);
+        }
+      }
+    }
+  }
+}
+
+}
diff --git a/ims-toucan-prosody-variance_amd/csrc/pipeline.hip b/ims-toucan-prosody-variance_amd/csrc/pipeline.hip
--- a/ims-toucan-prosody-variance_amd/csrc/pipeline.hip
+++ b/ims-toucan-prosody-variance_amd/csrc/pipeline.hip
@@ -11,6 +11,8 @@
 #include "../../include/toucan_score.h"
 
 namespace tts {
+
+const char* conv1d_wide_reject(const TtsConvDesc& d);
 
 namespace {
 
@@ -398,6 +400,18 @@
   const float *snake_alpha = nullptr, *snake_beta = nullptr, *snake_filt = nullptr;
 };
 
+int device_cus() {
+  static int cus[64] = {0};
+  int dev = 0;
+  (void)hipGetDevice(&dev);
+  int& c = cus[dev & 63];
+  if (c == 0 && (hipDeviceGetAttribute(&c, hipDeviceAttributeMultiprocessorCount, dev) != hipSuccess || c < 1)) {
+    (void)hipGetLastError();
+    c = 256;
+  }
+  return c;
+}
+
 int conv(Handle* h, const ConvW& cw, T2 x, T2 y, const Layout& l, hipStream_t st, const ConvOpt& o = ConvOpt()) {
   int tile_rows = cw.tile_rows;
   if (h->small_tile_blocks && cw.small_tile_rows && !cw.small_only) {
@@ -434,10 +448,21 @@
                ((any16 && h->cfg.precision == TTS_COMPUTE_F16) ? TTS_IO_F16 : 0);
   if (h->split_mode && !o.no_split_k && !is16(h) && d.compute == TTS_COMPUTE_F32)
     d.io_flags |= h->split_mode == 2 ? TTS_IO_SPLIT_K_ALWAYS : TTS_IO_SPLIT_K;
+  if (cw.algo_taps == 2 && cw.taps == 3) d.io_flags |= TTS_IO_POLYPHASE;
+  const bool wide_pays = (cw.cin / 64) * cw.taps >= 28 || ((d.io_flags & TTS_IO_POLYPHASE) && cw.wn >= 512);
+  if (cw.tile_rows != 256 && wide_pays && conv1d_wide_reject(d) == nullptr) {
+    long long t256 = 0;
+    for (int n : l.lengths) t256 += (n + 255) / 256;
+    if (t256 * (cw.wn / 256) >= device_cus()) {
+      tile_rows = 256;
+      TTS_TRY(tiles_of(h, l, tile_rows, st, &tt));
+    }
+  }
   d.tiles = tt.dev; d.n_tiles = tt.n; d.tile_rows = tile_rows;
   if (h->prof_on) {
     const bool dual = cw.mode != TTS_MODE_LINEAR;
-    const int bm = tile_rows != cw.tile_rows ? tile_rows : cw.tile_rows, bn = tile_rows != cw.tile_rows ? 64 : cw.n_tile;
+    const bool wide = tile_rows == 256 && cw.tile_rows != 256;
+    const int bm = tile_rows != cw.tile_rows ? tile_rows : cw.tile_rows, bn = wide ? 256 : (tile_rows != cw.tile_rows ? 64 : cw.n_tile);
     char name[96];
     int nlen = snprintf(name, sizeof(name), "conv1d_%s<%dx%d%s>", d.compute == TTS_COMPUTE_F32 ? "f32" : (d.compute == TTS_COMPUTE_BF16 ? "bf16" : (d.compute == TTS_COMPUTE_F16 ? "f16" : "f32x3")),
                         bm, bn, dual ? ",dual" : "");
diff --git a/ims-toucan-prosody-variance_amd/engine.py b/ims-toucan-prosody-variance_amd/engine.py
--- a/ims-toucan-prosody-variance_amd/engine.py
+++ b/ims-toucan-prosody-variance_amd/engine.py
@@ -22,6 +22,16 @@
 
 def _f16_flag(*ts):
     return capi.IO_F16 if any(t is not None and t.dtype == torch.float16 for t in ts) else 0
+
+
+def _wide_ok(d, cw, x, y, res):
+    ts = [t for t in (x, y, res) if t is not None]
+    dt = torch.float16 if d.compute == COMPUTE_F16 else torch.bfloat16
+    return (d.compute in (COMPUTE_BF16, COMPUTE_F16) and cw.mode == MODE_LINEAR and all(t.dtype == dt for t in ts)
+            and d.pre_act == PRE_NONE and not (d.seqvec or d.preadd or d.aux)
+            and cw.cin == cw.cin_pad and cw.cin % 64 == 0 and cw.wn % 256 == 0 and cw.cout % 4 == 0
+            and all(_ld(t) % 8 == 0 and t.data_ptr() % 16 == 0 for t in ts)
+            and 2 * ((256 + (cw.taps - 1) * cw.dil + 7) // 8 * 8) * 128 + 66 * 1024 <= 160 * 1024)
 
 
 def precision_of(bf16, precision):
@@ -58,6 +68,7 @@
                                       f"interface with device='cuda' (the reference's default 'cpu' cannot be served)")
         self.timer = None
         self.split_k = 0
+        self.n_cus = torch.cuda.get_device_properties(self.device).multi_processor_count if isinstance(self.lib, C.CDLL) else 0
         self.small_tile_blocks = 1536
         self._fir_tabs = {}
         self.default_compute = COMPUTE_F32
@@ -71,11 +82,13 @@
         return torch.empty(*shape, dtype=dtype, device=self.device)
 
     def conv(self, cw, x, y, rag, pre=PRE_NONE, pre_slope=0.0, act=ACT_NONE, alpha=1.0, seqvec=None, preadd=None, res=None,
-             res_scale=1.0, aux=None, accumulate=False, compute=None, snake=None, split_k=True):
+             res_scale=1.0, aux=None, accumulate=False, compute=None, snake=None, split_k=True, tile_rows=None):
         if compute is None:
             compute = self.default_compute
-        tile_rows = cw.tile_rows
-        if self.small_tile_blocks and cw.small_tile_rows and not cw.small_only:
+        forced = tile_rows is not None
+        if not forced:
+            tile_rows = cw.tile_rows
+        if not forced and self.small_tile_blocks and cw.small_tile_rows and not cw.small_only:
             cols = cw.wn if cw.mode == MODE_LINEAR else cw.half_pad
             if -(-rag.total_rows // cw.tile_rows) * (cols // cw.n_tile) < self.small_tile_blocks:
                 tile_rows = cw.small_tile_rows
@@ -107,6 +120,13 @@
             | _f16_flag(x, y, res)
         if split_k and self.split_k and self.default_compute in (COMPUTE_F32, COMPUTE_F32X3) and d.compute == COMPUTE_F32:
             d.io_flags |= capi.IO_SPLIT_K_ALWAYS if self.split_k == 2 else capi.IO_SPLIT_K
+        if cw.algo_taps == 2 and cw.taps == 3:
+            d.io_flags |= capi.IO_POLYPHASE
+        wide_pays = (cw.cin // 64) * cw.taps >= 28 or (bool(d.io_flags & capi.IO_POLYPHASE) and cw.wn >= 512)
+        if not forced and self.n_cus and cw.tile_rows != 256 and wide_pays and _wide_ok(d, cw, x, y, res):
+            if sum(-(-n // 256) for n in rag.lengths) * (cw.wn // 256) >= self.n_cus:
+                tile_rows = 256
+                tiles, n_tiles = rag.tiles(tile_rows)
         d.tiles, d.n_tiles, d.tile_rows = tiles.data_ptr(), n_tiles, tile_rows
         tm = self.timer
         if tm is not None and tm.wants(cw, d.compute, tile_rows):
diff --git a/ims-toucan-prosody-variance_amd/profiling.py b/ims-toucan-prosody-variance_amd/profiling.py
--- a/ims-toucan-prosody-variance_amd/profiling.py
+++ b/ims-toucan-prosody-variance_amd/profiling.py
@@ -7,7 +7,7 @@
     dual = cw.mode != capi.MODE_LINEAR
     bm, bn = cw.tile_rows, cw.n_tile
     if tile_rows is not None and tile_rows != cw.tile_rows:
-        bm, bn = tile_rows, 64
+        bm, bn = tile_rows, (256 if tile_rows == 256 else 64)
     prec = {capi.COMPUTE_F32: "f32", capi.COMPUTE_BF16: "bf16", capi.COMPUTE_F16: "f16", capi.COMPUTE_F32X3: "f32x3"}[compute]
     return "conv1d_%s<%dx%d%s>" % (prec, bm, bn, ",dual" if dual else "")
 
diff --git a/include/toucan_tts.h b/include/toucan_tts.h
--- a/include/toucan_tts.h
+++ b/include/toucan_tts.h
@@ -33,6 +33,7 @@
 #define TTS_IO_F16 8
 #define TTS_IO_SPLIT_K 16
 #define TTS_IO_SPLIT_K_ALWAYS 32
+#define TTS_IO_POLYPHASE 64
 #define TTS_ATT_KEY_SPLIT 1
 #define TTS_ATT_KEY_SPLIT_ALWAYS 2
 #define TTS_COMPUTE_F32 0
```

New measurement: 584,900, median of 6. 1.01x the previous value.
